# GMC-DRL/MetaBox

Hardware: AMD Instinct MI355X
Metric: env-steps/sec (instances x gens/s), RLEPSO bbob-easy d=10 (higher is better)
Workload: dtype f64

## Files before the change

### include/mbx.h

```cpp
#ifndef MBX_H
#define MBX_H

#include <stddef.h>
#include <stdint.h>

#ifdef __cplusplus
extern "C" {
#endif

#define MBX_OK            0
#define MBX_E_ARG        -1
#define MBX_E_HIP        -2
#define MBX_E_UNSUPPORTED -3
#define MBX_E_NOMEM      -4

#define MBX_KIND_PROTEIN 100

#define MBX_NOISE_NONE    0
#define MBX_NOISE_GAUSS   1
#define MBX_NOISE_UNIFORM 2
#define MBX_NOISE_CAUCHY  3

typedef struct mbx_problem_desc {
    int32_t func_id;
    int32_t kind;
    int32_t dim;
    int32_t n_peaks;
    int32_t noise_kind;
    int32_t reserved;
    double  bias, lb, ub;
    double  pen_coef;
    double  s[4];
    double  noise_a, noise_b;
    const double* dshift;
    const double* m1;
    const double* m2;
    const double* v0;
    const double* v1;
    const double* v2;
    const double* py;
    const double* pc;
    const double* pw;
} mbx_problem_desc;

typedef struct mbx_suite mbx_suite;
typedef struct mbx_batch mbx_batch;

int mbx_suite_create(const mbx_problem_desc* descs, int n_problems, const double* opt, mbx_suite** out);
int mbx_suite_destroy(mbx_suite* s);
int mbx_suite_size(const mbx_suite* s);
int mbx_suite_optimum(const mbx_suite* s, double* optimum_out );
int mbx_suite_close_pairs(const mbx_suite* s, int problem);

int mbx_eval(mbx_suite* s, int problem, const double* d_x, int n, double* d_f,
             int noisy, uint64_t seed, const double* d_noise_draws, void* stream);

#define MBX_ALGO_RLEPSO 1
#define MBX_ALGO_LDE    2
#define MBX_ALGO_DEDDQN 3
#define MBX_ALGO_RANDOM_SEARCH 4
#define MBX_ALGO_RLPSO  5
#define MBX_ALGO_GLEET  6
#define MBX_ALGO_QLPSO  7
#define MBX_ALGO_DE     8
#define MBX_ALGO_PSO    9
#define MBX_ALGO_CMAES  10
#define MBX_ALGO_GLPSO  11
#define MBX_ALGO_JDE21  13
#define MBX_ALGO_MADDE  15

typedef struct mbx_algo_cfg {
    int32_t algo;
    int32_t np;
    int32_t dim;
    int32_t max_fes;
    int32_t log_interval;
    int32_t n_logpoint;
    int32_t early_stop;
    int32_t n_group;
    uint32_t flags;
} mbx_algo_cfg;

#define MBX_F_FDR_FAST               1u
#define MBX_F_GENERIC_GEOMETRY       2u
#define MBX_F_ROLLOUT_PER_GENERATION 4u
int mbx_batch_flags(const mbx_batch* b);

int mbx_state_dim(const mbx_algo_cfg* cfg);
int mbx_action_dim(const mbx_algo_cfg* cfg);
int64_t mbx_tape_stride(const mbx_algo_cfg* cfg);

int mbx_batch_create(mbx_suite* s, const mbx_algo_cfg* cfg, const int32_t* problem_idx,
                     const uint64_t* seeds, int n_instances, mbx_batch** out);
int mbx_batch_destroy(mbx_batch* b);

int mbx_set_tape(mbx_batch* b, const double* d_tape);

int mbx_reset(mbx_batch* b, double* d_state_out, void* stream);

int mbx_step(mbx_batch* b, const void* d_actions, double* d_state_out, double* d_reward_out,
             uint8_t* d_done_out, void* stream);

int mbx_results(mbx_batch* b, double* d_cost_curves , double* d_fes ,
                double* d_return , int32_t* d_steps , int32_t* d_cost_len ,
                void* stream);

int mbx_batch_rebind(mbx_batch* b, const int32_t* problem_idx , const uint64_t* seeds );

int mbx_read_public(mbx_batch* b, int instance, double* host_out , void* stream);

int64_t mbx_instance_state_doubles(const mbx_batch* b);
int mbx_debug_read_state(mbx_batch* b, int instance, double* host_out);
int mbx_debug_write_state(mbx_batch* b, int instance, const double* host_in);

#define MBX_POLICY_RLEPSO 0
#define MBX_POLICY_RLPSO  1
typedef struct mbx_gauss_mlp {
    const float* d_weights;
    int32_t in_dim, h1, h2, out_dim;
    float min_sigma, max_sigma;
    int32_t variant;
} mbx_gauss_mlp;

int mbx_gauss_policy(mbx_batch* b, const mbx_gauss_mlp* net, const double* d_state, float* d_actions, float* d_mu_sigma,
                      void* stream);

typedef struct mbx_lstm_policy {
    const float* d_weights;
    int32_t in_dim, hidden, out_dim;
} mbx_lstm_policy;
int mbx_lde_policy(mbx_batch* b, const mbx_lstm_policy* net, const double* d_state, float* d_h, float* d_c, float* d_actions,
                   float* d_mu_sigma, void* stream);

typedef struct mbx_qnet {
    const float* d_weights;
    int32_t in_dim, width, depth, n_act;
} mbx_qnet;
int mbx_ddqn_qnet(mbx_batch* b, const mbx_qnet* net, const double* d_state, int32_t* d_actions, float* d_q, void* stream);

int mbx_rlepso_policy_table_rows(const mbx_batch* b);
int mbx_rlepso_policy_table(mbx_batch* b, const mbx_gauss_mlp* net, float* d_table, void* stream);
int mbx_rlepso_act_step(mbx_batch* b, const float* d_table, float* d_actions_out, double* d_state_out,
                        double* d_reward_out, uint8_t* d_done_out, void* stream);

int mbx_rlepso_rollout_resident(const mbx_batch* b);
int mbx_rlepso_rollout(mbx_batch* b, const float* d_table, int n_gens, float* d_traj_actions, double* d_traj_state,
                       double* d_traj_reward, uint8_t* d_traj_done, double* d_state_out, double* d_reward_out,
                       uint8_t* d_done_out, void* stream);

int mbx_lde_rollout_resident(const mbx_batch* b);
int mbx_lde_rollout(mbx_batch* b, const mbx_lstm_policy* net, const double* d_state_in, float* d_h, float* d_c, int n_gens,
                    float* d_traj_actions, double* d_traj_state, double* d_traj_reward, uint8_t* d_traj_done, double* d_state_out,
                    double* d_reward_out, uint8_t* d_done_out, void* stream);

int mbx_rlpso_rollout(mbx_batch* b, const mbx_gauss_mlp* net, int n_steps, float* d_actions_out, double* d_state_out,
                      double* d_reward_out, uint8_t* d_done_out, void* stream);

typedef struct mbx_gleet_actor {
    const float* d_weights;
    int32_t n_floats;
    float min_sigma, max_sigma;
} mbx_gleet_actor;
int mbx_gleet_policy(mbx_batch* b, const mbx_gleet_actor* net, const double* d_state, float* d_actions, float* d_mu_sigma, void* stream);

int mbx_qlpso_rollout(mbx_batch* b, const double* d_q_table, int n_steps, int32_t* d_actions_out, double* d_state_out,
                      double* d_reward_out, uint8_t* d_done_out, void* stream);

int mbx_debug_math(int op, const double* d_x, const double* d_y, double* d_out, int n, void* stream);

int mbx_debug_rlepso_draws(uint64_t seed, int gen, int episode, int np, int dim, double* d_out, void* stream);

int mbx_batch_launch_info(const mbx_batch* b, int32_t out[4]);

int mbx_debug_clock_probe(uint64_t* d_out, int n_samples, int sleep_units, void* stream);
int mbx_debug_clock_mark(uint64_t* d_out2, void* stream);
int mbx_debug_clock_slots(mbx_batch* b, uint64_t* d_slots2);

const char* mbx_last_error(void);
const char* mbx_version(void);

#ifdef __cplusplus
}
#endif
#endif
```

### metabox_amd/_abi.py

```python
import ctypes as C
import os

import numpy as np

_HERE = os.path.dirname(os.path.abspath(__file__))
LIB_PATH = os.environ.get('MBX_LIB') or os.path.join(_HERE, 'csrc', 'libmbx.so')

c_double_p = C.POINTER(C.c_double)


class ProblemDesc(C.Structure):
    _fields_ = [('func_id', C.c_int32), ('kind', C.c_int32), ('dim', C.c_int32), ('n_peaks', C.c_int32),
                ('noise_kind', C.c_int32), ('reserved', C.c_int32),
                ('bias', C.c_double), ('lb', C.c_double), ('ub', C.c_double), ('pen_coef', C.c_double),
                ('s', C.c_double * 4), ('noise_a', C.c_double), ('noise_b', C.c_double),
                ('dshift', c_double_p), ('m1', c_double_p), ('m2', c_double_p),
                ('v0', c_double_p), ('v1', c_double_p), ('v2', c_double_p),
                ('py', c_double_p), ('pc', c_double_p), ('pw', c_double_p)]


class AlgoCfg(C.Structure):
    _fields_ = [('algo', C.c_int32), ('np', C.c_int32), ('dim', C.c_int32), ('max_fes', C.c_int32),
                ('log_interval', C.c_int32), ('n_logpoint', C.c_int32), ('early_stop', C.c_int32),
                ('n_group', C.c_int32), ('flags', C.c_uint32)]


F_FDR_FAST, F_GENERIC_GEOMETRY, F_ROLLOUT_PER_GENERATION = 1, 2, 4


class GaussMlp(C.Structure):
    _fields_ = [('d_weights', C.c_void_p), ('in_dim', C.c_int32), ('h1', C.c_int32), ('h2', C.c_int32), ('out_dim', C.c_int32),
                ('min_sigma', C.c_float), ('max_sigma', C.c_float), ('variant', C.c_int32)]


class LstmPolicy(C.Structure):
    _fields_ = [('d_weights', C.c_void_p), ('in_dim', C.c_int32), ('hidden', C.c_int32), ('out_dim', C.c_int32)]


class QNet(C.Structure):
    _fields_ = [('d_weights', C.c_void_p), ('in_dim', C.c_int32), ('width', C.c_int32), ('depth', C.c_int32), ('n_act', C.c_int32)]


class GleetActor(C.Structure):
    _fields_ = [('d_weights', C.c_void_p), ('n_floats', C.c_int32), ('min_sigma', C.c_float), ('max_sigma', C.c_float)]


ALGO_RLEPSO, ALGO_LDE, ALGO_DEDDQN, ALGO_RANDOM_SEARCH, ALGO_RLPSO, ALGO_GLEET, ALGO_QLPSO, ALGO_DE, ALGO_PSO, ALGO_CMAES = 1, 2, 3, 4, 5, 6, 7, 8, 9, 10
ALGO_GLPSO = 11
ALGO_JDE21 = 13
ALGO_MADDE = 15
POLICY_RLEPSO, POLICY_RLPSO = 0, 1
_ARRAY_FIELDS = ('dshift', 'm1', 'm2', 'v0', 'v1', 'v2', 'py', 'pc', 'pw')


def pack_desc(d):
    st = ProblemDesc()
    keep = []
    for k in ('func_id', 'kind', 'dim', 'n_peaks', 'noise_kind'):
        setattr(st, k, int(d[k]))
    for k in ('bias', 'lb', 'ub', 'pen_coef', 'noise_a', 'noise_b'):
        setattr(st, k, float(d[k]))
    for i in range(4):
        st.s[i] = float(d['s'][i])
    for k in _ARRAY_FIELDS:
        a = d.get(k)
        if a is None:
            setattr(st, k, c_double_p())
        else:
            a = np.ascontiguousarray(a, dtype=np.float64)
            keep.append(a)
            setattr(st, k, a.ctypes.data_as(c_double_p))
    return st, keep


def pack_descs(descs):
    arr = (ProblemDesc * len(descs))()
    keep = []
    for i, d in enumerate(descs):
        st, k = pack_desc(d)
        arr[i] = st
        keep.extend(k)
    return arr, keep


_lib = None


class MbxError(RuntimeError):
    pass


def load_lib():
    global _lib
    if _lib is not None:
        return _lib
    if not os.path.exists(LIB_PATH) and not os.environ.get('MBX_LIB'):
        import shutil
        import subprocess
        if shutil.which('hipcc') or os.path.exists('/opt/rocm/bin/hipcc'):
            subprocess.call(['make', '-C', os.path.join(_HERE, 'csrc'), '-s'])
    if not os.path.exists(LIB_PATH):
        raise MbxError(f'{LIB_PATH} is missing: build it with `python -c "import __graft_entry__ as g; g.build()"` '
                       f'(hipcc --offload-arch=gfx950). metabox_amd has no CPU fallback.')
    lib = C.CDLL(LIB_PATH)
    vp, i32, u64, i64 = C.c_void_p, C.c_int32, C.c_uint64, C.c_int64
    proto = {
        'mbx_suite_create': (C.c_int, [C.POINTER(ProblemDesc), C.c_int, c_double_p, C.POINTER(vp)]),
        'mbx_suite_destroy': (C.c_int, [vp]),
        'mbx_suite_size': (C.c_int, [vp]),
        'mbx_suite_optimum': (C.c_int, [vp, c_double_p]),
        'mbx_suite_close_pairs': (C.c_int, [vp, C.c_int]),
        'mbx_eval': (C.c_int, [vp, C.c_int, vp, C.c_int, vp, C.c_int, u64, vp, vp]),
        'mbx_state_dim': (C.c_int, [C.POINTER(AlgoCfg)]),
        'mbx_action_dim': (C.c_int, [C.POINTER(AlgoCfg)]),
        'mbx_tape_stride': (i64, [C.POINTER(AlgoCfg)]),
        'mbx_batch_create': (C.c_int, [vp, C.POINTER(AlgoCfg), C.POINTER(i32), C.POINTER(u64), C.c_int,
                                       C.POINTER(vp)]),
        'mbx_batch_destroy': (C.c_int, [vp]),
        'mbx_batch_flags': (C.c_int, [vp]),
        'mbx_set_tape': (C.c_int, [vp, vp]),
        'mbx_reset': (C.c_int, [vp, vp, vp]),
        'mbx_step': (C.c_int, [vp, vp, vp, vp, vp, vp]),
        'mbx_results': (C.c_int, [vp, vp, vp, vp, vp, vp, vp]),
        'mbx_gauss_policy': (C.c_int, [vp, C.POINTER(GaussMlp), vp, vp, vp, vp]),
        'mbx_lde_policy': (C.c_int, [vp, C.POINTER(LstmPolicy), vp, vp, vp, vp, vp, vp]),
        'mbx_ddqn_qnet': (C.c_int, [vp, C.POINTER(QNet), vp, vp, vp, vp]),
        'mbx_rlepso_policy_table_rows': (C.c_int, [vp]),
        'mbx_rlepso_policy_table': (C.c_int, [vp, C.POINTER(GaussMlp), vp, vp]),
        'mbx_rlepso_act_step': (C.c_int, [vp, vp, vp, vp, vp, vp, vp]),
        'mbx_rlepso_rollout_resident': (C.c_int, [vp]),
        'mbx_rlepso_rollout': (C.c_int, [vp, vp, C.c_int, vp, vp, vp, vp, vp, vp, vp, vp]),
        'mbx_lde_rollout_resident': (C.c_int, [vp]),
        'mbx_lde_rollout': (C.c_int, [vp, C.POINTER(LstmPolicy), vp, vp, vp, C.c_int, vp, vp, vp, vp, vp, vp, vp, vp]),
        'mbx_rlpso_rollout': (C.c_int, [vp, C.POINTER(GaussMlp), C.c_int, vp, vp, vp, vp, vp]),
        'mbx_qlpso_rollout': (C.c_int, [vp, vp, C.c_int, vp, vp, vp, vp, vp]),
        'mbx_gleet_policy': (C.c_int, [vp, C.POINTER(GleetActor), vp, vp, vp, vp]),
        'mbx_debug_math': (C.c_int, [C.c_int, vp, vp, vp, C.c_int, vp]),
        'mbx_debug_rlepso_draws': (C.c_int, [C.c_uint64, C.c_int, C.c_int, C.c_int, C.c_int, vp, vp]),
        'mbx_batch_launch_info': (C.c_int, [vp, C.POINTER(C.c_int32)]),
        'mbx_instance_state_doubles': (i64, [vp]),
        'mbx_debug_read_state': (C.c_int, [vp, C.c_int, c_double_p]),
        'mbx_debug_write_state': (C.c_int, [vp, C.c_int, c_double_p]),
        'mbx_debug_clock_probe': (C.c_int, [vp, C.c_int, C.c_int, vp]),
        'mbx_debug_clock_mark': (C.c_int, [vp, vp]),
        'mbx_debug_clock_slots': (C.c_int, [vp, vp]),
        'mbx_batch_rebind': (C.c_int, [vp, vp, vp]),
        'mbx_read_public': (C.c_int, [vp, C.c_int, c_double_p, vp]),
        'mbx_last_error': (C.c_char_p, []),
        'mbx_version': (C.c_char_p, []),
    }
    for name, (res, args) in proto.items():
        fn = getattr(lib, name)
        fn.restype = res
        fn.argtypes = args
    _lib = lib
    return lib


EXPORTED_SYMBOLS = ('mbx_suite_create', 'mbx_suite_destroy', 'mbx_suite_size', 'mbx_suite_optimum', 'mbx_suite_close_pairs', 'mbx_eval', 'mbx_state_dim', 'mbx_action_dim',
                    'mbx_tape_stride', 'mbx_batch_create', 'mbx_batch_destroy', 'mbx_batch_flags', 'mbx_set_tape', 'mbx_reset', 'mbx_step', 'mbx_results',
                    'mbx_gauss_policy', 'mbx_lde_policy', 'mbx_ddqn_qnet', 'mbx_rlepso_policy_table_rows', 'mbx_rlepso_policy_table', 'mbx_rlepso_act_step',
                    'mbx_rlepso_rollout_resident', 'mbx_rlepso_rollout', 'mbx_lde_rollout_resident', 'mbx_lde_rollout', 'mbx_rlpso_rollout',
                    'mbx_qlpso_rollout', 'mbx_gleet_policy', 'mbx_debug_math', 'mbx_debug_rlepso_draws', 'mbx_batch_launch_info', 'mbx_instance_state_doubles',
                    'mbx_debug_read_state', 'mbx_debug_write_state', 'mbx_debug_clock_probe', 'mbx_debug_clock_mark', 'mbx_debug_clock_slots',
                    'mbx_batch_rebind', 'mbx_read_public', 'mbx_last_error', 'mbx_version')


def check(rc):
    if rc != 0:
        msg = load_lib().mbx_last_error()
        raise MbxError(f'mbx error {rc}: {msg.decode() if msg else "?"}')
```

### metabox_amd/csrc/mbx.hip

```cpp
#include <hip/hip_runtime.h>

#include <cmath>
#include <cstdarg>
#include <cstdio>
#include <cstring>
#include <algorithm>
#include <memory>
#include <string>
#include <vector>

#include "mbx_device.hpp"
#include "mbx_rlepso.hpp"
#include "mbx_lde.hpp"
#ifndef MBX_LDE100_STEP_THREADS
#define MBX_LDE100_STEP_THREADS 512
#endif
#ifndef MBX_LDE50_STEP_THREADS
#define MBX_LDE50_STEP_THREADS 256
#endif
#include "mbx_ddqn.hpp"
#include "mbx_rs.hpp"
#include "mbx_policy.hpp"
#include "mbx_lstm_policy.hpp"
#include "mbx_lde_run.hpp"
#include "mbx_qnet.hpp"
#include "mbx_rlpso.hpp"
#include "mbx_gleet.hpp"
#include "mbx_qlpso.hpp"
#include "mbx_gleet_policy.hpp"
#include "mbx_classic.hpp"
#include "mbx_glpso.hpp"
#include "mbx_jde21.hpp"
#include "mbx_madde.hpp"
#ifndef MBX_SINGLE_TU
#define MBX_RUN_KERNELS_EXTERN
#endif
#include "mbx_run_kernels.hpp"

using namespace mbx;

static thread_local std::string g_err;

static int fail(int code, const char* fmt, ...)
{
    char buf[512];
    va_list ap;
    va_start(ap, fmt);
    vsnprintf(buf, sizeof(buf), fmt, ap);
    va_end(ap);
    g_err = buf;
    return code;
}

#define HIP_TRY(expr)                                                                             \
    do {                                                                                          \
        hipError_t _e = (expr);                                                                   \
        if (_e != hipSuccess) return fail(MBX_E_HIP, "%s failed: %s", #expr, hipGetErrorString(_e)); \
    } while (0)

struct mbx_suite {
    int n = 0, dim = 0;
    double* d_pool = nullptr;
    DevProblem* d_problems = nullptr;
    std::vector<DevProblem> h_problems;
    std::vector<double> optimum;
};

struct mbx_batch {
    mbx_suite* suite = nullptr;
    mbx_algo_cfg cfg{};
    int B = 0;
    int32_t* d_problem_idx = nullptr;
    std::vector<int32_t> h_problem_idx;
    uint64_t* d_seeds = nullptr;
    double* d_state = nullptr;
    int32_t* d_order = nullptr;
    double* d_pci = nullptr;
    unsigned long long* d_clk = nullptr;
    double* d_scratch = nullptr;
    float* d_lstm_pack = nullptr;
    bool fdr_fast = false;
    bool rl_run_kinds_ok = false;
    bool lde_run_kinds_ok = false;
    bool lde_run_kinds_two = false;
    bool rollout_per_generation = false;
    int64_t state_stride = 0;
    const double* d_tape = nullptr;
    size_t lds_bytes = 0;
    int64_t sc_off = 0;
    int64_t tape_stride = 0;
    int state_dim = 0, action_dim = 0;
    int threads = kThreads;
    int fixed_geometry = 0;
};

struct AlgoGeom { int64_t state_doubles, sc_off, tape_stride, lds_doubles; int state_dim, action_dim; };

static AlgoGeom geom_of(const mbx_algo_cfg& c)
{
    AlgoGeom g{};
    if (c.algo == MBX_ALGO_RLEPSO) {
        g.state_doubles = MBX_RLEPSO_STATE_DOUBLES(c.np, c.dim, c.n_logpoint);
        g.sc_off = MBX_RLEPSO_ST_SCALARS(c.np, c.dim);
        g.tape_stride = MBX_RLEPSO_TAPE_STRIDE(c.np, c.dim);
        g.lds_doubles = rl_lds_doubles(c.np, c.dim, (c.flags & MBX_F_GENERIC_GEOMETRY) || c.n_group != 5 || rl_maps_in_lds(c.np, c.dim));
        g.state_dim = 1; g.action_dim = 7 * c.n_group;
    } else if (c.algo == MBX_ALGO_LDE) {
        g.state_doubles = MBX_LDE_STATE_DOUBLES(c.np, c.dim, c.n_logpoint);
        g.sc_off = MBX_LDE_ST_SCALARS(c.np, c.dim);
        g.tape_stride = MBX_LDE_TAPE_STRIDE(c.np, c.dim);
        g.lds_doubles = lde_lds_doubles(c.np, c.dim, lde_maps_in_lds(c.np, c.dim) || (c.flags & MBX_F_GENERIC_GEOMETRY));
        g.state_dim = c.np + 2 * MBX_LDE_BINS; g.action_dim = 2 * c.np;
    } else if (c.algo == MBX_ALGO_DEDDQN) {
        g.state_doubles = MBX_DQ_STATE_DOUBLES(c.np, c.dim, c.n_logpoint);
        g.sc_off = MBX_DQ_ST_SCALARS(c.np, c.dim);
        g.tape_stride = MBX_DQ_TAPE_STRIDE(c.np, c.dim);
        g.lds_doubles = dq_lds_doubles(c.np, c.np, c.dim);
        g.state_dim = MBX_DQ_NFEAT; g.action_dim = 1;
    } else if (c.algo == MBX_ALGO_RANDOM_SEARCH) {
        g.state_doubles = MBX_RS_STATE_DOUBLES(c.np, c.dim, c.n_logpoint);
        g.sc_off = MBX_RS_ST_SCALARS(c.np, c.dim);
        g.tape_stride = MBX_RS_TAPE_STRIDE(c.np, c.dim);
        g.lds_doubles = rs_lds_doubles(c.np, c.dim);
        g.state_dim = 1; g.action_dim = 0;
    } else if (c.algo == MBX_ALGO_RLPSO) {
        g.state_doubles = MBX_RLPSO_STATE_DOUBLES(c.np, c.dim, c.n_logpoint);
        g.sc_off = MBX_RLPSO_ST_SCALARS(c.np, c.dim);
        g.tape_stride = MBX_RLPSO_TAPE_STRIDE(c.np, c.dim);
        g.lds_doubles = rp_lds_doubles(c.np, c.dim, 0);
        g.state_dim = 2 * c.dim; g.action_dim = 1;
    } else if (c.algo == MBX_ALGO_GLEET) {
        g.state_doubles = MBX_GLEET_STATE_DOUBLES(c.np, c.dim, c.n_logpoint);
        g.sc_off = MBX_GLEET_ST_SCALARS(c.np, c.dim);
        g.tape_stride = MBX_GLEET_TAPE_STRIDE(c.np, c.dim);
        g.lds_doubles = gl_lds_doubles(c.np, c.dim);
        g.state_dim = 27 * c.np; g.action_dim = c.np;
    } else if (c.algo == MBX_ALGO_QLPSO) {
        g.state_doubles = MBX_QLPSO_STATE_DOUBLES(c.np, c.dim, c.n_logpoint);
        g.sc_off = MBX_QLPSO_ST_SCALARS(c.np, c.dim);
        g.tape_stride = MBX_QLPSO_TAPE_STRIDE(c.np, c.dim);
        g.lds_doubles = ql_lds_doubles(c.np, c.np, c.dim);
        g.state_dim = 1; g.action_dim = 1;
    } else if (c.algo == MBX_ALGO_DE || c.algo == MBX_ALGO_PSO || c.algo == MBX_ALGO_CMAES) {
        g.state_doubles = c.algo == MBX_ALGO_DE ? MBX_DE_STATE_DOUBLES(c.np, c.dim, c.n_logpoint)
                        : c.algo == MBX_ALGO_PSO ? MBX_PSO_STATE_DOUBLES(c.np, c.dim, c.n_logpoint) : MBX_CMA_STATE_DOUBLES(c.np, c.dim, c.n_logpoint);
        g.sc_off = c.algo == MBX_ALGO_DE ? MBX_DE_ST_SCALARS(c.np, c.dim) : c.algo == MBX_ALGO_PSO ? MBX_PSO_ST_SCALARS(c.np, c.dim) : MBX_CMA_ST_SCALARS(c.np, c.dim);
        g.tape_stride = 0;
        g.lds_doubles = cl_lds_doubles(c.np, c.np, c.dim, 0, c.algo == MBX_ALGO_CMAES);
        g.state_dim = 1; g.action_dim = 0;
    } else if (c.algo == MBX_ALGO_GLPSO) {
        g.state_doubles = MBX_GLPSO_STATE_DOUBLES(c.np, c.dim, c.n_logpoint);
        g.sc_off = MBX_GLPSO_ST_SCALARS(c.np, c.dim);
        g.tape_stride = MBX_GLPSO_TAPE_STRIDE(c.np, c.dim);
        g.lds_doubles = gp_lds_doubles(c.np, c.dim);
        g.state_dim = 1; g.action_dim = 0;
    } else if (c.algo == MBX_ALGO_JDE21) {
        g.state_doubles = MBX_JDE21_STATE_DOUBLES(c.np, c.dim, c.n_logpoint);
        g.sc_off = MBX_JDE21_ST_SCALARS(c.np, c.dim);
        g.tape_stride = MBX_JDE21_TAPE_STRIDE(c.np, c.dim);
        g.lds_doubles = jd_lds_doubles(c.np, c.dim);
        g.state_dim = 1; g.action_dim = 0;
    } else if (c.algo == MBX_ALGO_MADDE) {
        g.state_doubles = MBX_MADDE_STATE_DOUBLES(c.np, c.dim, c.n_logpoint);
        g.sc_off = MBX_MADDE_ST_SCALARS(c.np, c.dim);
        g.tape_stride = MBX_MADDE_TAPE_STRIDE(c.np, c.dim);
        g.lds_doubles = md_lds_doubles(c.np, c.dim);
        g.state_dim = 1; g.action_dim = 0;
    }
    return g;
}

extern "C" int mbx_suite_destroy(mbx_suite* s);
extern "C" int mbx_batch_destroy(mbx_batch* b);

__global__ __launch_bounds__(kThreads) void k_eval(const DevProblem* problems, int problem, const double* __restrict__ x, int n,
                                                   int rows, double* __restrict__ f, int noisy, uint64_t seed,
                                                   const double* __restrict__ draws)
{
    extern __shared__ __attribute__((aligned(16))) double smem[];
    const DevProblem P = problems[problem];
    const int D = P.dim, tid = threadIdx.x;
    const int row0 = blockIdx.x * rows;
    const int m = min(rows, n - row0);
    const int64_t NE = align2((int64_t)rows * D), SC = align2(NE > 2 * kThreads ? NE : 2 * kThreads), DD = align2((int64_t)D * D);
    const int64_t DV = align2(D);
    double* X = smem;
    double* T = X + NE;
    double* Z = T + eval_t_doubles(rows, D);
    double* M1T = Z + SC;
    double* M2T = M1T + DD;
    double* VEC = M2T + DD;
    double* F = VEC + 4 * DV;
    const EvalLds L{X, Z, T, M1T, M2T, VEC, VEC + DV, VEC + 2 * DV, VEC + 3 * DV, F};
    stage_problem(P, L);
    for (int e = tid; e < m * D; e += kThreads) X[e] = x[(int64_t)row0 * D + e];
    __syncthreads();
    eval_rows(P, L, m);
    for (int i = tid; i < m; i += kThreads) {
        double v = F[i];
        if (noisy && P.noise_kind != MBX_NOISE_NONE) {
            double a, b, c;
            const int r = row0 + i;
            if (draws) { a = draws[r]; b = draws[n + r]; c = draws[2 * (int64_t)n + r]; }
            else {
                const Rng rng{(uint32_t)seed, (uint32_t)(seed >> 32), 0u, 0u};
                philox_noise(rng, (uint32_t)r, MBX_SITE_EVAL_A, MBX_SITE_EVAL_B, P.noise_kind, a, b, c);
            }
            v = apply_noise(P, v, a, b, c);
        }
        f[row0 + i] = v;
    }
}

static size_t eval_lds_bytes(int rows, int D)
{
    const int64_t NE = align2((int64_t)rows * D), SC = align2(NE > 2 * kThreads ? NE : 2 * kThreads), DD = align2((int64_t)D * D);
    return (size_t)(NE + eval_t_doubles(rows, D) + SC + 2 * DD + 4 * align2(D) + align2(rows)) * sizeof(double);
}

__global__ void k_init_state(double* state, int64_t stride, int64_t sc_off, int B)
{
    const int b = blockIdx.x * blockDim.x + threadIdx.x;
    if (b < B) state[(int64_t)b * stride + sc_off + MBX_SC_EPISODE] = -1.;
}

__global__ void k_set_optimum(DevProblem* problems, const double* opt, int n)
{
    const int i = blockIdx.x * blockDim.x + threadIdx.x;
    if (i < n) problems[i].optimum = opt[i];
}

__global__ void k_results(const double* state, int64_t stride, int64_t sc_off, int B, int nlog, double* cost, double* fes,
                          double* ret, int32_t* steps, int32_t* cost_len)
{
    const int b = blockIdx.x * blockDim.x + threadIdx.x;
    if (b >= B) return;
    const double* sc = state + (int64_t)b * stride + sc_off;
    const int len = (int)sc[MBX_SC_COST_LEN];
    if (cost)
        for (int k = 0; k <= nlog; ++k) cost[(int64_t)b * (nlog + 1) + k] = sc[MBX_NSCALAR + (k < len ? k : len - 1)];
    if (fes) fes[b] = sc[MBX_SC_FES];
    if (ret) ret[b] = sc[MBX_SC_RETURN];
    if (steps) steps[b] = (int32_t)sc[MBX_SC_GEN];
    if (cost_len) cost_len[b] = len;
}

static int max_lds_bytes()
{
    int v = 0, dev = 0;
    (void)hipGetDevice(&dev);
    if (hipDeviceGetAttribute(&v, hipDeviceAttributeMaxSharedMemoryPerBlock, dev) != hipSuccess || v <= 0) v = 64 * 1024;
    return v;
}

static int launch_eval(mbx_suite* s, int problem, const double* d_x, int n, double* d_f, int noisy, uint64_t seed,
                       const double* d_draws, hipStream_t st)
{
    if (n <= 0) return MBX_OK;
    const int D = s->dim;
    int rows = n < 128 ? n : 128;
    const int cap = max_lds_bytes();
    while (rows > 1 && eval_lds_bytes(rows, D) > (size_t)cap) rows /= 2;
    const size_t lds = eval_lds_bytes(rows, D);
    if (lds > (size_t)cap) return fail(MBX_E_UNSUPPORTED, "dim %d needs %zu B of LDS (> %d)", D, lds, cap);
    HIP_TRY(hipFuncSetAttribute((const void*)k_eval, hipFuncAttributeMaxDynamicSharedMemorySize, (int)lds));
    const int grid = (n + rows - 1) / rows;
    hipLaunchKernelGGL(k_eval, dim3(grid), dim3(kThreads), lds, st, s->d_problems, problem, d_x, n, rows, d_f, noisy, seed,
                       d_draws);
    HIP_TRY(hipGetLastError());
    return MBX_OK;
}

extern "C" int mbx_suite_create(const mbx_problem_desc* descs, int n_problems, const double* opt, mbx_suite** out)
{
    if (!descs || n_problems <= 0 || !out) return fail(MBX_E_ARG, "mbx_suite_create: bad arguments");
    const int D = descs[0].dim;
    if (D < 2 || D > 64) return fail(MBX_E_ARG, "dim %d outside [2, 64]", D);
    std::vector<double> pool;
    std::vector<DevProblem> hp(n_problems);
    struct Off { int64_t o[11]; };
    std::vector<Off> offs(n_problems);
    auto push = [&](const double* p, size_t n) -> int64_t {
        if (!p) return -1;
        while (pool.size() % 2) pool.push_back(0.);
        const int64_t o = (int64_t)pool.size();
        pool.insert(pool.end(), p, p + n);
        return o;
    };
    for (int i = 0; i < n_problems; ++i) {
        const mbx_problem_desc& d = descs[i];
        if (d.dim != D) return fail(MBX_E_ARG, "problem %d has dim %d, suite dim is %d", i, d.dim, D);
        const bool bbob = d.kind >= 1 && d.kind <= 24, protein = d.kind == MBX_KIND_PROTEIN;
        if (!bbob && !protein) return fail(MBX_E_UNSUPPORTED, "problem %d: objective kind %d is not implemented", i, d.kind);
        if (bbob && (!d.dshift || !d.m1)) return fail(MBX_E_ARG, "problem %d: dshift/m1 missing", i);
        if (protein && (!d.v0 || !d.py || !d.pc || !d.pw || d.n_peaks < 2 || d.n_peaks > 160))
            return fail(MBX_E_ARG, "problem %d: protein tables missing (v0, py, pc, pw) or n_atoms outside [2,160]", i);
        if ((d.kind == 21 || d.kind == 22) && (!d.py || !d.pc || !d.pw || d.n_peaks <= 0))
            return fail(MBX_E_ARG, "problem %d: Gallagher tables missing", i);
        DevProblem& p = hp[i];
        memset(&p, 0, sizeof(p));
        p.func_id = d.func_id; p.kind = d.kind; p.dim = d.dim; p.n_peaks = d.n_peaks; p.noise_kind = d.noise_kind;
        p.bias = d.bias; p.lb = d.lb; p.ub = d.ub; p.pen_coef = d.pen_coef;
        for (int k = 0; k < 4; ++k) p.s[k] = d.s[k];
        p.noise_a = d.noise_a; p.noise_b = d.noise_b; p.optimum = NAN;
        const size_t DD = (size_t)D * D, NA = (size_t)d.n_peaks;
        const size_t PK = protein ? 3 * NA * D : NA * D;
        const size_t PC = protein ? 3 * NA : NA * D;
        const size_t PW = protein ? 3 * NA * NA : NA;
        Off& o = offs[i];
        o.o[0] = push(d.dshift, D); o.o[1] = push(d.m1, DD); o.o[2] = push(d.m2, DD);
        o.o[3] = push(d.v0, D); o.o[4] = push(d.v1, D); o.o[5] = push(d.v2, D);
        o.o[6] = push(d.py, PK); o.o[7] = push(d.pc, PC); o.o[8] = push(d.pw, PW);
        o.o[9] = -1; o.o[10] = -1;
        if (d.kind == 21 || d.kind == 22) {
            std::vector<double> lw(NA);
            for (size_t k = 0; k < NA; ++k) lw[k] = std::log(d.pw[k]);
            o.o[10] = push(lw.data(), NA);
            std::vector<double> ry(NA * D);
            for (int k = 0; k < d.n_peaks; ++k)
                for (int r = 0; r < D; ++r) {
                    double acc = 0.;
                    for (int j = 0; j < D; ++j) acc = std::fma(d.m1[(size_t)r * D + j], d.py[(size_t)k * D + j], acc);
                    ry[(size_t)k * D + r] = acc;
                }
            o.o[9] = push(ry.data(), NA * D);
        }
        if (protein) {
            const int n = d.n_peaks, W = n - 1, n_pairs = ((n + 1) / 2) * W;
            const double *se = d.pw, *qm = d.pw + NA * NA, *rm = d.pw + 2 * NA * NA;
            for (int a = 0; a < n; ++a)
                for (int c = a + 1; c < n; ++c)
                    if (se[a * n + c] != se[c * n + a] || qm[a * n + c] != qm[c * n + a] || rm[a * n + c] != rm[c * n + a])
                        return fail(MBX_E_ARG, "problem %d: the protein tables sqrt(e) | q | r must be symmetric (atoms %d, %d)", i, a, c);
            std::vector<int> pi_(n_pairs), pj_(n_pairs), order;
            std::vector<double> d0(n_pairs, INFINITY);
            std::vector<double> bd(n, 0.);
            for (int m = 0; m < n; ++m) {
                double q2 = 0.;
                for (int c = 0; c < 3; ++c) {
                    double bsum = 0.;
                    for (int k = 0; k < D; ++k) bsum += std::fabs(d.v0[k] * d.py[(size_t)k * 3 * n + 3 * m + c]);
                    bsum *= std::fmax(std::fabs(d.ub), std::fabs(d.lb));
                    q2 += bsum * bsum;
                }
                bd[m] = std::sqrt(q2) * (1. + 1e-12);
            }
            for (int t = 0; t < n_pairs; ++t) {
                const int a = t / W, b = t - a * W, La = W - a;
                const bool lower = b >= La;
                pi_[t] = lower ? W - a : a; pj_[t] = pi_[t] + 1 + (lower ? b - La : b);
                if (lower && pi_[t] == a) { pi_[t] = -1; continue; }
                double q2 = 0.;
                for (int c = 0; c < 3; ++c) { const double dd = d.pc[3 * pi_[t] + c] - d.pc[3 * pj_[t] + c]; q2 += dd * dd; }
                d0[t] = std::sqrt(q2) - bd[pi_[t]] - bd[pj_[t]];
            }
            int n_close = 0;
            for (int t = 0; t < n_pairs; ++t) n_close += pi_[t] >= 0 && d0[t] <= 9.0 + 1e-6;
            hp[i].n_close = n_close;
            order.resize(n_pairs);
            for (int t = 0; t < n_pairs; ++t) order[t] = t;
            std::stable_sort(order.begin(), order.end(), [&](int x, int y) { return d0[x] < d0[y]; });
            std::vector<double> rec((size_t)n_pairs * 4, 0.);
            std::vector<double> ij((size_t)(n_pairs + 1) / 2, 0.);
            int32_t* ijw = reinterpret_cast<int32_t*>(ij.data());
            for (int t = 0; t < n_pairs; ++t) {
                const int pi = pi_[order[t]], pj = pj_[order[t]];
                if (pi < 0) { ijw[t] = -1; continue; }
                ijw[t] = pi | (pj << 16);
                rec[(size_t)t * 4] = se[pi * n + pj]; rec[(size_t)t * 4 + 1] = qm[pi * n + pj]; rec[(size_t)t * 4 + 2] = rm[pi * n + pj];
            }
            o.o[9] = push(rec.data(), rec.size());
            o.o[10] = push(ij.data(), ij.size());
        }
    }
    std::unique_ptr<mbx_suite, int (*)(mbx_suite*)> guard(new mbx_suite(), mbx_suite_destroy);
    mbx_suite* s = guard.get();
    s->n = n_problems; s->dim = D;
    HIP_TRY(hipMalloc(&s->d_pool, pool.size() * sizeof(double)));
    HIP_TRY(hipMemcpy(s->d_pool, pool.data(), pool.size() * sizeof(double), hipMemcpyHostToDevice));
    for (int i = 0; i < n_problems; ++i) {
        const double** ptrs[11] = {&hp[i].dshift, &hp[i].m1, &hp[i].m2, &hp[i].v0, &hp[i].v1,
                                   &hp[i].v2, &hp[i].py, &hp[i].pc, &hp[i].pw, &hp[i].pyr, &hp[i].plogw};
        for (int k = 0; k < 11; ++k) *ptrs[k] = offs[i].o[k] < 0 ? nullptr : s->d_pool + offs[i].o[k];
    }
    HIP_TRY(hipMalloc(&s->d_problems, n_problems * sizeof(DevProblem)));
    HIP_TRY(hipMemcpy(s->d_problems, hp.data(), n_problems * sizeof(DevProblem), hipMemcpyHostToDevice));
    s->h_problems = hp;
    s->optimum.assign(n_problems, NAN);
    if (opt) {
        double *d_x = nullptr, *d_f = nullptr;
        HIP_TRY(hipMalloc(&d_x, (size_t)n_problems * D * sizeof(double)));
        HIP_TRY(hipMalloc(&d_f, (size_t)n_problems * sizeof(double)));
        HIP_TRY(hipMemcpy(d_x, opt, (size_t)n_problems * D * sizeof(double), hipMemcpyHostToDevice));
        for (int i = 0; i < n_problems; ++i) {
            int rc = launch_eval(s, i, d_x + (size_t)i * D, 1, d_f + i, 0, 0, nullptr, nullptr);
            if (rc) return rc;
        }
        hipLaunchKernelGGL(k_set_optimum, dim3((n_problems + 63) / 64), dim3(64), 0, nullptr, s->d_problems, d_f, n_problems);
        HIP_TRY(hipDeviceSynchronize());
        HIP_TRY(hipMemcpy(s->optimum.data(), d_f, n_problems * sizeof(double), hipMemcpyDeviceToHost));
        for (int i = 0; i < n_problems; ++i) s->h_problems[i].optimum = s->optimum[i];
        (void)hipFree(d_x); (void)hipFree(d_f);
    }
    *out = guard.release();
    return MBX_OK;
}

extern "C" int mbx_suite_destroy(mbx_suite* s)
{
    if (!s) return MBX_OK;
    (void)hipFree(s->d_pool); (void)hipFree(s->d_problems);
    delete s;
    return MBX_OK;
}

extern "C" int mbx_suite_size(const mbx_suite* s) { return s ? s->n : fail(MBX_E_ARG, "null suite"); }

extern "C" int mbx_suite_optimum(const mbx_suite* s, double* optimum_out)
{
    if (!s || !optimum_out) return fail(MBX_E_ARG, "mbx_suite_optimum: bad arguments");
    memcpy(optimum_out, s->optimum.data(), s->n * sizeof(double));
    return MBX_OK;
}

extern "C" int mbx_suite_close_pairs(const mbx_suite* s, int problem)
{
    if (!s || problem < 0 || problem >= s->n) return fail(MBX_E_ARG, "mbx_suite_close_pairs: bad arguments");
    return s->h_problems[problem].kind == MBX_KIND_PROTEIN ? s->h_problems[problem].n_close : -1;
}

extern "C" int mbx_eval(mbx_suite* s, int problem, const double* d_x, int n, double* d_f, int noisy, uint64_t seed,
                        const double* d_noise_draws, void* stream)
{
    if (!s || problem < 0 || problem >= s->n || n < 0 || (n > 0 && (!d_x || !d_f)))
        return fail(MBX_E_ARG, "mbx_eval: bad arguments");
    return launch_eval(s, problem, d_x, n, d_f, noisy, seed, d_noise_draws, (hipStream_t)stream);
}

static int check_cfg(const mbx_algo_cfg* c)
{
    if (!c) return fail(MBX_E_ARG, "null cfg");
    if (!((c->algo >= MBX_ALGO_RLEPSO && c->algo <= MBX_ALGO_GLPSO) || c->algo == MBX_ALGO_JDE21 || c->algo == MBX_ALGO_MADDE))
        return fail(MBX_E_UNSUPPORTED, "algo %d is not implemented in this build", c->algo);
    if (c->algo == MBX_ALGO_JDE21 && c->np != MBX_JDE21_NP) return fail(MBX_E_ARG, "JDE21 runs np = %d (160 + 10 rows), not %d", MBX_JDE21_NP, c->np);
    if (c->algo == MBX_ALGO_MADDE) {
        if (c->dim < 2 || c->dim > MBX_MADDE_DIM_MAX) return fail(MBX_E_ARG, "MadDE runs dim in [2, %d], not %d", MBX_MADDE_DIM_MAX, c->dim);
        if (c->np != MBX_MADDE_NP(c->dim)) return fail(MBX_E_ARG, "MadDE runs np = 2 dim^2 = %d, not %d", MBX_MADDE_NP(c->dim), c->np);
    } else if (c->np < 4 || c->np > kThreads) return fail(MBX_E_ARG, "np %d outside [4, %d]", c->np, kThreads);
    if (c->dim < 2 || c->dim > 64) return fail(MBX_E_ARG, "dim %d outside [2, 64]", c->dim);
    if (c->algo == MBX_ALGO_RLEPSO && (c->n_group < 1 || c->n_group > 16 || c->np / c->n_group < 1))
        return fail(MBX_E_ARG, "bad n_group %d", c->n_group);
    if (c->max_fes <= 0 || c->log_interval <= 0 || c->n_logpoint <= 0) return fail(MBX_E_ARG, "bad budget/log settings");
    if (c->flags & ~(MBX_F_FDR_FAST | MBX_F_GENERIC_GEOMETRY | MBX_F_ROLLOUT_PER_GENERATION)) return fail(MBX_E_ARG, "unknown bits in cfg.flags 0x%x", c->flags);
    return MBX_OK;
}

extern "C" int mbx_state_dim(const mbx_algo_cfg* c)
{
    if (int rc = check_cfg(c)) return rc;
    return geom_of(*c).state_dim;
}

extern "C" int mbx_action_dim(const mbx_algo_cfg* c)
{
    if (int rc = check_cfg(c)) return rc;
    return geom_of(*c).action_dim;
}

extern "C" int64_t mbx_tape_stride(const mbx_algo_cfg* c)
{
    if (int rc = check_cfg(c)) return rc;
    return geom_of(*c).tape_stride;
}

static int upload_launch_order(mbx_batch* b, const int32_t* problem_idx)
{
    const mbx_suite* s = b->suite;
    const int n_instances = b->B;
    auto weight = [&](int pi) -> int {
        const int k = s->h_problems[pi].kind;
        if (b->cfg.algo == MBX_ALGO_LDE && s->dim >= 16 && k != MBX_KIND_PROTEIN) {
            switch (k) {
            case 21: case 22: return 155; case 17: case 18: return 121; case 16: case 23: return 110; case 15: case 3: case 4: return 100; case 2: case 10: case 11: return 92;
            case 14: case 12: return 81; case 7: return 78; case 19: case 24: case 20: return 77; case 8: case 9: case 6: return 66; default: return 62;
            }
        }
        if (s->dim >= 16 && k != MBX_KIND_PROTEIN) {
            switch (k) {
            case 21: return 3016; case 22: return 2378; case 16: return 2342; case 15: return 2285; case 18: return 2283; case 17: return 2255;
            case 3: return 2077; case 23: return 2049; case 4: return 1980; case 7: return 1885; case 12: return 1840; case 2: return 1787;
            case 11: return 1784; case 10: return 1783; case 24: return 1682; case 14: return 1656; case 19: return 1607; case 1: return 1588;
            case 6: return 1566; case 8: return 1533; case 9: return 1528; case 20: return 1526; case 13: return 1499; case 5: return 1334;
            default: return 1886;
            }
        }
        switch (k) {
        case MBX_KIND_PROTEIN: return 30000 + s->h_problems[pi].n_close;
        case 21: return 416; case 3: return 332; case 15: return 326; case 16: return 325; case 22: return 323; case 23: return 316;
        case 18: return 310; case 17: return 310; case 4: return 309; case 2: return 282; case 12: return 282; case 11: return 275;
        case 10: return 270; case 6: return 254; case 14: return 252; case 1: return 251; case 20: return 250; case 19: return 247;
        case 24: return 246; case 8: return 244; case 13: return 239; case 7: return 237; case 9: return 233; case 5: return 153;
        default: return 276;
        }
    };
    b->lde_run_kinds_ok = true;
    b->rl_run_kinds_ok = true;
    for (int i = 0; i < n_instances; ++i) b->rl_run_kinds_ok = b->rl_run_kinds_ok && rl_run_kind_ok(s->h_problems[problem_idx[i]].kind, s->h_problems[problem_idx[i]].noise_kind);
    b->lde_run_kinds_two = true;
    for (int i = 0; i < n_instances; ++i) {
        b->lde_run_kinds_ok = b->lde_run_kinds_ok && lde_run_kind_ok(s->h_problems[problem_idx[i]].kind, s->dim, false);
        b->lde_run_kinds_two = b->lde_run_kinds_two && lde_run_kind_ok(s->h_problems[problem_idx[i]].kind, s->dim, true);
    }
    std::vector<int32_t> order(n_instances);
    for (int i = 0; i < n_instances; ++i) order[i] = i;
    std::stable_sort(order.begin(), order.end(), [&](int a, int c) {
        const int wa = weight(problem_idx[a]), wc = weight(problem_idx[c]);
        return wa != wc ? wa > wc : s->h_problems[problem_idx[a]].kind < s->h_problems[problem_idx[c]].kind;
    });
    if (!b->d_order) HIP_TRY(hipMalloc(&b->d_order, n_instances * sizeof(int32_t)));
    HIP_TRY(hipMemcpy(b->d_order, order.data(), n_instances * sizeof(int32_t), hipMemcpyHostToDevice));
    return MBX_OK;
}

static uint32_t env_flags()
{
    auto on = [](const char* name) { const char* v = getenv(name); return v && v[0] == '1'; };
    return (on("MBX_FDR_FAST") ? MBX_F_FDR_FAST : 0u) | (on("MBX_GENERIC_GEOMETRY") ? MBX_F_GENERIC_GEOMETRY : 0u) |
           (on("MBX_ROLLOUT_PER_GENERATION") ? MBX_F_ROLLOUT_PER_GENERATION : 0u);
}

extern "C" int mbx_batch_create(mbx_suite* s, const mbx_algo_cfg* cfg_in, const int32_t* problem_idx, const uint64_t* seeds,
                                int n_instances, mbx_batch** out)
{
    if (!s || !problem_idx || !seeds || n_instances <= 0 || !out) return fail(MBX_E_ARG, "mbx_batch_create: bad arguments");
    if (int rc = check_cfg(cfg_in)) return rc;
    mbx_algo_cfg effective = *cfg_in;
    effective.flags |= env_flags();
    const mbx_algo_cfg* cfg = &effective;
    if (cfg->dim != s->dim) return fail(MBX_E_ARG, "cfg.dim %d != suite dim %d", cfg->dim, s->dim);
    for (int i = 0; i < n_instances; ++i)
        if (problem_idx[i] < 0 || problem_idx[i] >= s->n) return fail(MBX_E_ARG, "problem_idx[%d]=%d out of range", i, problem_idx[i]);
    const AlgoGeom g = geom_of(*cfg);
    const size_t lds = (size_t)g.lds_doubles * sizeof(double);
    if (lds > (size_t)max_lds_bytes())
        return fail(MBX_E_UNSUPPORTED, "np=%d dim=%d needs %zu B of LDS per workgroup (> %d)", cfg->np, cfg->dim, lds, max_lds_bytes());
    std::unique_ptr<mbx_batch, int (*)(mbx_batch*)> guard(new mbx_batch(), mbx_batch_destroy);
    mbx_batch* b = guard.get();
    b->suite = s; b->cfg = *cfg; b->B = n_instances; b->lds_bytes = lds;
    if (cfg->algo == MBX_ALGO_LDE && (size_t)lde_lds_doubles(cfg->np, cfg->dim, true) * sizeof(double) > 40 * 1024 && cfg->dim >= 16) b->threads = 512;
    if (cfg->algo == MBX_ALGO_RLEPSO && (size_t)rl_lds_doubles(cfg->np, cfg->dim, true) * sizeof(double) > 80 * 1024 && cfg->dim >= 16) b->threads = cfg->dim >= 32 ? 1024 : 512;
    {
        const bool generic = (cfg->flags & MBX_F_GENERIC_GEOMETRY) != 0;
        if (cfg->algo == MBX_ALGO_RLEPSO && cfg->n_group == 5 && !generic) {
            if (b->threads == kThreads && cfg->np == 100 && cfg->dim == 10) b->fixed_geometry = 1;
            if (b->threads == 1024 && cfg->np == 128 && cfg->dim == 40) b->fixed_geometry = 2;
            if (b->threads == 512 && cfg->np == 100 && cfg->dim == 30) b->fixed_geometry = 7;
            if (b->threads == kThreads && cfg->np == 100 && cfg->dim == 12) b->fixed_geometry = 8;
            if (b->threads == 1024 && cfg->np == 100 && cfg->dim == 40) b->fixed_geometry = 10;
        }
        if (cfg->algo != MBX_ALGO_RLEPSO || b->fixed_geometry == 7 || b->fixed_geometry == 8 || b->fixed_geometry == 10) b->cfg.flags &= ~MBX_F_FDR_FAST;
        b->fdr_fast = (b->cfg.flags & MBX_F_FDR_FAST) != 0;
        if (cfg->algo == MBX_ALGO_LDE && b->threads == 512 && cfg->np == 50 && cfg->dim == 30 && !generic) b->fixed_geometry = 3;
        if (cfg->algo == MBX_ALGO_LDE && b->threads == 512 && cfg->np == 100 && cfg->dim == 30 && !generic) b->fixed_geometry = 6;
        if (cfg->algo == MBX_ALGO_LDE && b->threads == kThreads && cfg->np == 50 && cfg->dim == 10 && !generic) b->fixed_geometry = 9;
        if (cfg->algo == MBX_ALGO_DEDDQN && cfg->np == 100 && cfg->dim == 12 && !generic) b->fixed_geometry = 4;
        if (cfg->algo == MBX_ALGO_GLEET && cfg->np == 100 && cfg->dim == 10 && !generic) b->fixed_geometry = 5;
        b->rollout_per_generation = (cfg->flags & MBX_F_ROLLOUT_PER_GENERATION) != 0;
    }
#ifdef MBX_LDS_PAD_EXPERIMENT
    if (const char* e = getenv("MBX_LDS_PAD")) b->lds_bytes += (size_t)atoi(e);
#endif
    b->state_stride = (g.state_doubles + 1) & ~(int64_t)1;
    b->sc_off = g.sc_off; b->tape_stride = g.tape_stride; b->state_dim = g.state_dim; b->action_dim = g.action_dim;
    HIP_TRY(hipMalloc(&b->d_problem_idx, n_instances * sizeof(int32_t)));
    HIP_TRY(hipMalloc(&b->d_seeds, n_instances * sizeof(uint64_t)));
    HIP_TRY(hipMalloc(&b->d_state, (size_t)n_instances * b->state_stride * sizeof(double)));
    HIP_TRY(hipMemcpy(b->d_problem_idx, problem_idx, n_instances * sizeof(int32_t), hipMemcpyHostToDevice));
    b->h_problem_idx.assign(problem_idx, problem_idx + n_instances);
    HIP_TRY(hipMemcpy(b->d_seeds, seeds, n_instances * sizeof(uint64_t), hipMemcpyHostToDevice));
    HIP_TRY(hipMemset(b->d_state, 0, (size_t)n_instances * b->state_stride * sizeof(double)));
    if (int rc = upload_launch_order(b, problem_idx)) return rc;
    hipLaunchKernelGGL(k_init_state, dim3((n_instances + 255) / 256), dim3(256), 0, nullptr, b->d_state, b->state_stride,
                       g.sc_off, n_instances);
    HIP_TRY(hipDeviceSynchronize());
    if (cfg->algo == MBX_ALGO_RLEPSO) {
        {
        std::vector<double> pci(cfg->np);
        for (int i = 0; i < cfg->np; ++i) pci[i] = 0.05 + 0.45 * std::exp(10. * i / (cfg->np - 1)) / (std::exp(10.) - 1);
        HIP_TRY(hipMalloc(&b->d_pci, cfg->np * sizeof(double)));
        HIP_TRY(hipMemcpy(b->d_pci, pci.data(), cfg->np * sizeof(double), hipMemcpyHostToDevice));
        HIP_TRY(hipMalloc(&b->d_scratch, (size_t)n_instances * sizeof(double)));
    }
#define MBX_RL_LDS(...) HIP_TRY(hipFuncSetAttribute((const void*)(__VA_ARGS__), hipFuncAttributeMaxDynamicSharedMemorySize, (int)lds))
        MBX_RL_LDS(k_rlepso_reset<kThreads>); MBX_RL_LDS(k_rlepso_reset<512>); MBX_RL_LDS(k_rlepso_reset<1024>); MBX_RL_LDS(k_rlepso_reset<512, 100, 30>);
        MBX_RL_LDS(k_rlepso_step<kThreads, 0, 0, 0, true>); MBX_RL_LDS(k_rlepso_step<512, 0, 0, 0, true>); MBX_RL_LDS(k_rlepso_step<1024, 0, 0, 0, true>);
        MBX_RL_LDS(k_rlepso_step<kThreads, 0, 0, 0, false>); MBX_RL_LDS(k_rlepso_step<512, 0, 0, 0, false>); MBX_RL_LDS(k_rlepso_step<1024, 0, 0, 0, false>);
        MBX_RL_LDS(k_rlepso_step<kThreads, 100, 10, 5, true>); MBX_RL_LDS(k_rlepso_step<kThreads, 100, 10, 5, false>);
        MBX_RL_LDS(k_rlepso_step<1024, 128, 40, 5, true>); MBX_RL_LDS(k_rlepso_step<1024, 128, 40, 5, false>);
        MBX_RL_LDS(k_rlepso_step<512, 100, 30, 5, true>);
        MBX_RL_LDS(k_rlepso_run<MBX_RUN10_THREADS, 100, 10, 5, true>); MBX_RL_LDS(k_rlepso_run<MBX_RUN10_THREADS, 100, 10, 5, false>);
        MBX_RL_LDS(k_rlepso_run<1024, 128, 40, 5, true>); MBX_RL_LDS(k_rlepso_run<1024, 128, 40, 5, false>);
        MBX_RL_LDS(k_rlepso_run<512, 100, 30, 5, true>); MBX_RL_LDS(k_rlepso_run<256, 100, 12, 5, true>); MBX_RL_LDS(k_rlepso_run<1024, 100, 40, 5, true>);
#undef MBX_RL_LDS
    } else if (cfg->algo == MBX_ALGO_LDE) {
        {
            HIP_TRY(hipMalloc(&b->d_scratch, (size_t)n_instances * (sizeof(double) + (size_t)g.action_dim * sizeof(float))));
            HIP_TRY(hipMalloc(&b->d_lstm_pack, (size_t)lde_run_pack_floats(g.state_dim, 64, g.action_dim) * sizeof(float)));
            HIP_TRY(hipFuncSetAttribute((const void*)k_lde_run<100, 30>, hipFuncAttributeMaxDynamicSharedMemorySize, (int)(lde_run_lds_doubles(100, 30, 50, false) * sizeof(double))));
            HIP_TRY(hipFuncSetAttribute((const void*)k_lde_run<50, 30>, hipFuncAttributeMaxDynamicSharedMemorySize, (int)(lde_run_lds_doubles(50, 30, 50, false) * sizeof(double))));
            HIP_TRY(hipFuncSetAttribute((const void*)k_lde_run<50, 30, 50, true>, hipFuncAttributeMaxDynamicSharedMemorySize, (int)(lde_run_lds_doubles(50, 30, 50, true) * sizeof(double))));
            HIP_TRY(hipFuncSetAttribute((const void*)k_lde_run<50, 10>, hipFuncAttributeMaxDynamicSharedMemorySize, (int)(lde_run_lds_doubles(50, 10, 50, true) * sizeof(double))));
        }
        HIP_TRY(hipFuncSetAttribute((const void*)k_lde_reset<kThreads>, hipFuncAttributeMaxDynamicSharedMemorySize, (int)lds));
        HIP_TRY(hipFuncSetAttribute((const void*)k_lde_step<kThreads>, hipFuncAttributeMaxDynamicSharedMemorySize, (int)lds));
        HIP_TRY(hipFuncSetAttribute((const void*)k_lde_reset<512>, hipFuncAttributeMaxDynamicSharedMemorySize, (int)lds));
        HIP_TRY(hipFuncSetAttribute((const void*)k_lde_step<512>, hipFuncAttributeMaxDynamicSharedMemorySize, (int)lds));
        HIP_TRY(hipFuncSetAttribute((const void*)k_lde_step<MBX_LDE50_STEP_THREADS, 50, 30>, hipFuncAttributeMaxDynamicSharedMemorySize, (int)lds));
        HIP_TRY(hipFuncSetAttribute((const void*)k_lde_step<MBX_LDE100_STEP_THREADS, 100, 30>, hipFuncAttributeMaxDynamicSharedMemorySize, (int)lds));
        HIP_TRY(hipFuncSetAttribute((const void*)k_lde_reset<512, 100, 30>, hipFuncAttributeMaxDynamicSharedMemorySize, (int)lds));
        HIP_TRY(hipFuncSetAttribute((const void*)k_lde_reset<512, 50, 30>, hipFuncAttributeMaxDynamicSharedMemorySize, (int)lds));
    } else if (cfg->algo == MBX_ALGO_DEDDQN) {
        HIP_TRY(hipFuncSetAttribute((const void*)k_dq_reset, hipFuncAttributeMaxDynamicSharedMemorySize, (int)lds));
        HIP_TRY(hipFuncSetAttribute((const void*)k_dq_step<>, hipFuncAttributeMaxDynamicSharedMemorySize, (int)lds));
        HIP_TRY(hipFuncSetAttribute((const void*)k_dq_step<100, 12>, hipFuncAttributeMaxDynamicSharedMemorySize, (int)lds));
    } else if (cfg->algo == MBX_ALGO_DE || cfg->algo == MBX_ALGO_PSO || cfg->algo == MBX_ALGO_CMAES) {
        HIP_TRY(hipFuncSetAttribute((const void*)k_classic_reset, hipFuncAttributeMaxDynamicSharedMemorySize, (int)lds));
        HIP_TRY(hipFuncSetAttribute((const void*)k_de_sweep, hipFuncAttributeMaxDynamicSharedMemorySize, (int)lds));
        HIP_TRY(hipFuncSetAttribute((const void*)k_pso_sweep, hipFuncAttributeMaxDynamicSharedMemorySize, (int)lds));
        HIP_TRY(hipFuncSetAttribute((const void*)k_cmaes_generation, hipFuncAttributeMaxDynamicSharedMemorySize, (int)lds));
    } else if (cfg->algo == MBX_ALGO_GLPSO) {
        HIP_TRY(hipFuncSetAttribute((const void*)k_glpso_reset, hipFuncAttributeMaxDynamicSharedMemorySize, (int)lds));
        HIP_TRY(hipFuncSetAttribute((const void*)k_glpso_generation, hipFuncAttributeMaxDynamicSharedMemorySize, (int)lds));
    } else if (cfg->algo == MBX_ALGO_JDE21) {
        HIP_TRY(hipFuncSetAttribute((const void*)k_jde21_reset, hipFuncAttributeMaxDynamicSharedMemorySize, (int)lds));
        HIP_TRY(hipFuncSetAttribute((const void*)k_jde21_generation<2>, hipFuncAttributeMaxDynamicSharedMemorySize, (int)lds));
        HIP_TRY(hipFuncSetAttribute((const void*)k_jde21_generation<3>, hipFuncAttributeMaxDynamicSharedMemorySize, (int)lds));
    } else if (cfg->algo == MBX_ALGO_MADDE) {
        HIP_TRY(hipFuncSetAttribute((const void*)k_madde_reset, hipFuncAttributeMaxDynamicSharedMemorySize, (int)lds));
        HIP_TRY(hipFuncSetAttribute((const void*)k_madde_generation, hipFuncAttributeMaxDynamicSharedMemorySize, (int)lds));
    } else if (cfg->algo == MBX_ALGO_QLPSO) {
        HIP_TRY(hipFuncSetAttribute((const void*)k_qlpso_reset, hipFuncAttributeMaxDynamicSharedMemorySize, (int)lds));
        HIP_TRY(hipFuncSetAttribute((const void*)k_qlpso_step<false>, hipFuncAttributeMaxDynamicSharedMemorySize, (int)lds));
        HIP_TRY(hipFuncSetAttribute((const void*)k_qlpso_step<true>, hipFuncAttributeMaxDynamicSharedMemorySize, (int)lds));
    } else if (cfg->algo == MBX_ALGO_GLEET) {
        HIP_TRY(hipFuncSetAttribute((const void*)k_gleet_reset, hipFuncAttributeMaxDynamicSharedMemorySize, (int)lds));
        HIP_TRY(hipFuncSetAttribute((const void*)k_gleet_step<>, hipFuncAttributeMaxDynamicSharedMemorySize, (int)lds));
        HIP_TRY(hipFuncSetAttribute((const void*)k_gleet_step<100, 10>, hipFuncAttributeMaxDynamicSharedMemorySize, (int)lds));
    } else if (cfg->algo == MBX_ALGO_RLPSO) {
        HIP_TRY(hipFuncSetAttribute((const void*)k_rlpso_reset, hipFuncAttributeMaxDynamicSharedMemorySize, (int)lds));
        HIP_TRY(hipFuncSetAttribute((const void*)k_rlpso_step<false>, hipFuncAttributeMaxDynamicSharedMemorySize, (int)lds));
        HIP_TRY(hipFuncSetAttribute((const void*)k_rlpso_step<true>, hipFuncAttributeMaxDynamicSharedMemorySize, (int)lds));
    } else {
        HIP_TRY(hipFuncSetAttribute((const void*)k_rs_population, hipFuncAttributeMaxDynamicSharedMemorySize, (int)lds));
    }
    *out = guard.release();
    return MBX_OK;
}

extern "C" int mbx_batch_destroy(mbx_batch* b)
{
    if (!b) return MBX_OK;
    (void)hipFree(b->d_problem_idx); (void)hipFree(b->d_seeds); (void)hipFree(b->d_state); (void)hipFree(b->d_order); (void)hipFree(b->d_pci); (void)hipFree(b->d_scratch); (void)hipFree(b->d_lstm_pack);
    delete b;
    return MBX_OK;
}

extern "C" int mbx_batch_rebind(mbx_batch* b, const int32_t* problem_idx, const uint64_t* seeds)
{
    if (!b || !problem_idx || !seeds) return fail(MBX_E_ARG, "mbx_batch_rebind: bad arguments");
    for (int i = 0; i < b->B; ++i)
        if (problem_idx[i] < 0 || problem_idx[i] >= b->suite->n) return fail(MBX_E_ARG, "problem_idx[%d]=%d out of range", i, problem_idx[i]);
    HIP_TRY(hipDeviceSynchronize());
    HIP_TRY(hipMemcpy(b->d_problem_idx, problem_idx, b->B * sizeof(int32_t), hipMemcpyHostToDevice));
    b->h_problem_idx.assign(problem_idx, problem_idx + b->B);
    HIP_TRY(hipMemcpy(b->d_seeds, seeds, b->B * sizeof(uint64_t), hipMemcpyHostToDevice));
    if (int rc = upload_launch_order(b, problem_idx)) return rc;
    hipLaunchKernelGGL(k_init_state, dim3((b->B + 255) / 256), dim3(256), 0, nullptr, b->d_state, b->state_stride, b->sc_off, b->B);
    HIP_TRY(hipDeviceSynchronize());
    return MBX_OK;
}

extern "C" int mbx_read_public(mbx_batch* b, int instance, double* host_out, void* stream)
{
    if (!b || instance < 0 || instance >= b->B || !host_out) return fail(MBX_E_ARG, "mbx_read_public: bad arguments");
    const size_t n = (size_t)(MBX_NSCALAR + b->cfg.n_logpoint + 1) * sizeof(double);
    HIP_TRY(hipMemcpyAsync(host_out, b->d_state + (int64_t)instance * b->state_stride + b->sc_off, n, hipMemcpyDeviceToHost, (hipStream_t)stream));
    HIP_TRY(hipStreamSynchronize((hipStream_t)stream));
    return MBX_OK;
}

extern "C" int mbx_set_tape(mbx_batch* b, const double* d_tape)
{
    if (!b) return fail(MBX_E_ARG, "null batch");
    b->d_tape = d_tape;
    return MBX_OK;
}

static BatchParams make_params(const mbx_batch* b)
{
    BatchParams p;
    p.problems = b->suite->d_problems; p.problem_idx = b->d_problem_idx; p.seeds = b->d_seeds;
    p.state = b->d_state; p.state_stride = b->state_stride;
    p.tape = b->d_tape; p.tape_stride = b->tape_stride; p.order = b->d_order; p.pci = b->d_pci;
    p.NP = b->cfg.np; p.D = b->cfg.dim; p.max_fes = b->cfg.max_fes; p.log_interval = b->cfg.log_interval;
    p.n_logpoint = b->cfg.n_logpoint; p.early_stop = b->cfg.early_stop; p.n_group = b->cfg.n_group; p.B = b->B;
    p.sc_off = b->sc_off;
    p.clk = b->d_clk;
    return p;
}

static void launch_rlepso_step(mbx_batch* b, hipStream_t stream, const float* d_actions, double* d_state_out, double* d_reward_out,
                               uint8_t* d_done_out, const float* d_table, int table_rows, float* d_actions_out)
{
#define MBX_RLEPSO_LAUNCH(...)                                                                                                   \
    hipLaunchKernelGGL((k_rlepso_step<__VA_ARGS__>), dim3(b->B), dim3(b->threads), b->lds_bytes, stream, make_params(b), d_actions, \
                       d_state_out, d_reward_out, d_done_out, d_table, table_rows, d_actions_out)
    const bool fast = b->fdr_fast;
    if (b->fixed_geometry == 1) { if (fast) MBX_RLEPSO_LAUNCH(kThreads, 100, 10, 5, false); else MBX_RLEPSO_LAUNCH(kThreads, 100, 10, 5, true); }
    else if (b->fixed_geometry == 2) { if (fast) MBX_RLEPSO_LAUNCH(1024, 128, 40, 5, false); else MBX_RLEPSO_LAUNCH(1024, 128, 40, 5, true); }
    else if (b->fixed_geometry == 7) MBX_RLEPSO_LAUNCH(512, 100, 30, 5, true);
    else if (b->threads == 1024) { if (fast) MBX_RLEPSO_LAUNCH(1024, 0, 0, 0, false); else MBX_RLEPSO_LAUNCH(1024, 0, 0, 0, true); }
    else if (b->threads == 512) { if (fast) MBX_RLEPSO_LAUNCH(512, 0, 0, 0, false); else MBX_RLEPSO_LAUNCH(512, 0, 0, 0, true); }
    else { if (fast) MBX_RLEPSO_LAUNCH(kThreads, 0, 0, 0, false); else MBX_RLEPSO_LAUNCH(kThreads, 0, 0, 0, true); }
#undef MBX_RLEPSO_LAUNCH
}

extern "C" int mbx_reset(mbx_batch* b, double* d_state_out, void* stream)
{
    if (!b) return fail(MBX_E_ARG, "null batch");
    if (b->cfg.algo == MBX_ALGO_RANDOM_SEARCH)
        hipLaunchKernelGGL(k_rs_population, dim3(b->B), dim3(kThreads), b->lds_bytes, (hipStream_t)stream, make_params(b), 1, d_state_out,
                           (double*)nullptr, (uint8_t*)nullptr);
    else if (b->cfg.algo == MBX_ALGO_RLEPSO && b->fixed_geometry == 7)
        hipLaunchKernelGGL((k_rlepso_reset<512, 100, 30>), dim3(b->B), dim3(512), b->lds_bytes, (hipStream_t)stream, make_params(b), d_state_out);
    else if (b->cfg.algo == MBX_ALGO_RLEPSO && b->threads == 1024)
        hipLaunchKernelGGL(k_rlepso_reset<1024>, dim3(b->B), dim3(1024), b->lds_bytes, (hipStream_t)stream, make_params(b), d_state_out);
    else if (b->cfg.algo == MBX_ALGO_RLEPSO && b->threads == 512)
        hipLaunchKernelGGL(k_rlepso_reset<512>, dim3(b->B), dim3(512), b->lds_bytes, (hipStream_t)stream, make_params(b), d_state_out);
    else if (b->cfg.algo == MBX_ALGO_RLEPSO)
        hipLaunchKernelGGL(k_rlepso_reset<kThreads>, dim3(b->B), dim3(kThreads), b->lds_bytes, (hipStream_t)stream, make_params(b), d_state_out);
    else if (b->cfg.algo == MBX_ALGO_RLPSO)
        hipLaunchKernelGGL(k_rlpso_reset, dim3(b->B), dim3(kThreads), b->lds_bytes, (hipStream_t)stream, make_params(b), d_state_out);
    else if (b->cfg.algo == MBX_ALGO_DE || b->cfg.algo == MBX_ALGO_PSO || b->cfg.algo == MBX_ALGO_CMAES)
        hipLaunchKernelGGL(k_classic_reset, dim3(b->B), dim3(kThreads), (size_t)cl_lds_doubles(b->cfg.np, b->cfg.np, b->cfg.dim, 0, 0) * sizeof(double),
                           (hipStream_t)stream, make_params(b), (int)b->cfg.algo, d_state_out);
    else if (b->cfg.algo == MBX_ALGO_GLPSO)
        hipLaunchKernelGGL(k_glpso_reset, dim3(b->B), dim3(kThreads), b->lds_bytes, (hipStream_t)stream, make_params(b), d_state_out);
    else if (b->cfg.algo == MBX_ALGO_JDE21)
        hipLaunchKernelGGL(k_jde21_reset, dim3(b->B), dim3(kThreads), b->lds_bytes, (hipStream_t)stream, make_params(b), d_state_out);
    else if (b->cfg.algo == MBX_ALGO_MADDE)
        hipLaunchKernelGGL(k_madde_reset, dim3(b->B), dim3(kThreads), b->lds_bytes, (hipStream_t)stream, make_params(b), d_state_out);
    else if (b->cfg.algo == MBX_ALGO_QLPSO)
        hipLaunchKernelGGL(k_qlpso_reset, dim3(b->B), dim3(kThreads), b->lds_bytes, (hipStream_t)stream, make_params(b), d_state_out);
    else if (b->cfg.algo == MBX_ALGO_GLEET)
        hipLaunchKernelGGL(k_gleet_reset, dim3(b->B), dim3(kThreads), b->lds_bytes, (hipStream_t)stream, make_params(b), d_state_out);
    else {
        if (!d_state_out) return fail(MBX_E_ARG, "mbx_reset: this algorithm needs d_state_out");
        if (b->cfg.algo == MBX_ALGO_LDE && b->fixed_geometry == 6)
            hipLaunchKernelGGL((k_lde_reset<512, 100, 30>), dim3(b->B), dim3(512), b->lds_bytes, (hipStream_t)stream, make_params(b), d_state_out);
        else if (b->cfg.algo == MBX_ALGO_LDE && b->fixed_geometry == 3)
            hipLaunchKernelGGL((k_lde_reset<512, 50, 30>), dim3(b->B), dim3(512), b->lds_bytes, (hipStream_t)stream, make_params(b), d_state_out);
        else if (b->cfg.algo == MBX_ALGO_LDE && b->threads == 512)
            hipLaunchKernelGGL(k_lde_reset<512>, dim3(b->B), dim3(512), b->lds_bytes, (hipStream_t)stream, make_params(b), d_state_out);
        else if (b->cfg.algo == MBX_ALGO_LDE)
            hipLaunchKernelGGL(k_lde_reset<kThreads>, dim3(b->B), dim3(kThreads), b->lds_bytes, (hipStream_t)stream, make_params(b), d_state_out);
        else
            hipLaunchKernelGGL(k_dq_reset, dim3(b->B), dim3(kThreads), b->lds_bytes, (hipStream_t)stream, make_params(b), d_state_out);
    }
    HIP_TRY(hipGetLastError());
    return MBX_OK;
}

extern "C" int mbx_step(mbx_batch* b, const void* d_actions, double* d_state_out, double* d_reward_out, uint8_t* d_done_out,
                        void* stream)
{
    const bool no_agent = b && (b->cfg.algo == MBX_ALGO_RANDOM_SEARCH || b->cfg.algo == MBX_ALGO_DE || b->cfg.algo == MBX_ALGO_PSO ||
                                b->cfg.algo == MBX_ALGO_CMAES || b->cfg.algo == MBX_ALGO_GLPSO || b->cfg.algo == MBX_ALGO_JDE21 ||
                                b->cfg.algo == MBX_ALGO_MADDE);
    if (!b || (!d_actions && !no_agent)) return fail(MBX_E_ARG, "mbx_step: bad arguments");
    if (b->cfg.algo == MBX_ALGO_RANDOM_SEARCH)
        hipLaunchKernelGGL(k_rs_population, dim3(b->B), dim3(kThreads), b->lds_bytes, (hipStream_t)stream, make_params(b), 0, d_state_out,
                           d_reward_out, d_done_out);
    else if (b->cfg.algo == MBX_ALGO_RLEPSO)
        launch_rlepso_step(b, (hipStream_t)stream, (const float*)d_actions, d_state_out, d_reward_out, d_done_out, nullptr, 0, nullptr);
    else if (b->cfg.algo == MBX_ALGO_DE)
        hipLaunchKernelGGL(k_de_sweep, dim3(b->B), dim3(kThreads), (size_t)cl_lds_doubles(1, b->cfg.np, b->cfg.dim, 1, 0) * sizeof(double),
                           (hipStream_t)stream, make_params(b), d_state_out, d_reward_out, d_done_out);
    else if (b->cfg.algo == MBX_ALGO_PSO)
        hipLaunchKernelGGL(k_pso_sweep, dim3(b->B), dim3(kThreads), (size_t)cl_lds_doubles(1, b->cfg.np, b->cfg.dim, 0, 0) * sizeof(double),
                           (hipStream_t)stream, make_params(b), d_state_out, d_reward_out, d_done_out);
    else if (b->cfg.algo == MBX_ALGO_CMAES)
        hipLaunchKernelGGL(k_cmaes_generation, dim3(b->B), dim3(kThreads), (size_t)cl_lds_doubles(b->cfg.np, b->cfg.np, b->cfg.dim, 0, 1) * sizeof(double),
                           (hipStream_t)stream, make_params(b), d_state_out, d_reward_out, d_done_out);
    else if (b->cfg.algo == MBX_ALGO_GLPSO)
        hipLaunchKernelGGL(k_glpso_generation, dim3(b->B), dim3(kThreads), b->lds_bytes, (hipStream_t)stream, make_params(b), d_state_out,
                           d_reward_out, d_done_out);
    else if (b->cfg.algo == MBX_ALGO_JDE21 && jd_waves((int64_t)b->lds_bytes) == 3)
        hipLaunchKernelGGL(k_jde21_generation<3>, dim3(b->B), dim3(kThreads), b->lds_bytes, (hipStream_t)stream, make_params(b), d_state_out,
                           d_reward_out, d_done_out);
    else if (b->cfg.algo == MBX_ALGO_JDE21)
        hipLaunchKernelGGL(k_jde21_generation<2>, dim3(b->B), dim3(kThreads), b->lds_bytes, (hipStream_t)stream, make_params(b), d_state_out,
                           d_reward_out, d_done_out);
    else if (b->cfg.algo == MBX_ALGO_MADDE)
        hipLaunchKernelGGL(k_madde_generation, dim3(b->B), dim3(kThreads), b->lds_bytes, (hipStream_t)stream, make_params(b), d_state_out,
                           d_reward_out, d_done_out);
    else if (b->cfg.algo == MBX_ALGO_QLPSO)
        hipLaunchKernelGGL(k_qlpso_step<false>, dim3(b->B), dim3(kThreads), (size_t)ql_lds_doubles(1, b->cfg.np, b->cfg.dim) * sizeof(double),
                           (hipStream_t)stream, make_params(b), (const int32_t*)d_actions, (const double*)nullptr, 1, d_state_out,
                           d_reward_out, d_done_out, (int32_t*)nullptr);
    else if (b->cfg.algo == MBX_ALGO_GLEET && b->fixed_geometry == 5)
        hipLaunchKernelGGL((k_gleet_step<100, 10>), dim3(b->B), dim3(kThreads), b->lds_bytes, (hipStream_t)stream, make_params(b),
                           (const float*)d_actions, d_state_out, d_reward_out, d_done_out);
    else if (b->cfg.algo == MBX_ALGO_GLEET)
        hipLaunchKernelGGL(k_gleet_step<>, dim3(b->B), dim3(kThreads), b->lds_bytes, (hipStream_t)stream, make_params(b),
                           (const float*)d_actions, d_state_out, d_reward_out, d_done_out);
    else if (b->cfg.algo == MBX_ALGO_RLPSO)
        hipLaunchKernelGGL(k_rlpso_step<false>, dim3(b->B), dim3(kThreads), (size_t)rp_lds_doubles(1, b->cfg.dim, 0) * sizeof(double),
                           (hipStream_t)stream, make_params(b), (const float*)d_actions, GaussMlp{}, 1, d_state_out, d_reward_out,
                           d_done_out, (float*)nullptr);
    else {
        if (!d_state_out) return fail(MBX_E_ARG, "mbx_step: this algorithm needs d_state_out");
        if (b->cfg.algo == MBX_ALGO_LDE && b->fixed_geometry == 3)
            hipLaunchKernelGGL((k_lde_step<MBX_LDE50_STEP_THREADS, 50, 30>), dim3(b->B), dim3(MBX_LDE50_STEP_THREADS), b->lds_bytes, (hipStream_t)stream, make_params(b),
                               (const float*)d_actions, d_state_out, d_reward_out, d_done_out);
        else if (b->cfg.algo == MBX_ALGO_LDE && b->fixed_geometry == 6)
            hipLaunchKernelGGL((k_lde_step<MBX_LDE100_STEP_THREADS, 100, 30>), dim3(b->B), dim3(MBX_LDE100_STEP_THREADS), b->lds_bytes, (hipStream_t)stream, make_params(b),
                               (const float*)d_actions, d_state_out, d_reward_out, d_done_out);
        else if (b->cfg.algo == MBX_ALGO_LDE && b->threads == 512)
            hipLaunchKernelGGL(k_lde_step<512>, dim3(b->B), dim3(512), b->lds_bytes, (hipStream_t)stream, make_params(b),
                               (const float*)d_actions, d_state_out, d_reward_out, d_done_out);
        else if (b->cfg.algo == MBX_ALGO_LDE)
            hipLaunchKernelGGL(k_lde_step<kThreads>, dim3(b->B), dim3(kThreads), b->lds_bytes, (hipStream_t)stream, make_params(b),
                               (const float*)d_actions, d_state_out, d_reward_out, d_done_out);
        else if (b->fixed_geometry == 4)
            hipLaunchKernelGGL((k_dq_step<100, 12>), dim3(b->B), dim3(kDqStepThreads), (size_t)dq_lds_doubles(1, b->cfg.np, b->cfg.dim) * sizeof(double), (hipStream_t)stream, make_params(b),
                               (const int32_t*)d_actions, d_state_out, d_reward_out, d_done_out);
        else
            hipLaunchKernelGGL(k_dq_step<>, dim3(b->B), dim3(kDqStepThreads), (size_t)dq_lds_doubles(1, b->cfg.np, b->cfg.dim) * sizeof(double), (hipStream_t)stream, make_params(b),
                               (const int32_t*)d_actions, d_state_out, d_reward_out, d_done_out);
    }
    HIP_TRY(hipGetLastError());
    return MBX_OK;
}

static int check_gauss_mlp(const mbx_batch* b, const mbx_gauss_mlp* net, const char* who, size_t* lds)
{
    if (!b || !net || !net->d_weights) return fail(MBX_E_ARG, "%s: bad arguments", who);
    if (b->cfg.algo != MBX_ALGO_RLEPSO && b->cfg.algo != MBX_ALGO_RLPSO)
        return fail(MBX_E_UNSUPPORTED, "%s: the batch is neither an RLEPSO nor an RL-PSO batch", who);
    if (net->variant != (b->cfg.algo == MBX_ALGO_RLPSO ? MBX_POLICY_RLPSO : MBX_POLICY_RLEPSO))
        return fail(MBX_E_ARG, "%s: net.variant does not match the batch's algorithm", who);
    if (net->in_dim != b->state_dim || net->out_dim != b->action_dim || net->h1 < 1 || net->h2 < 1)
        return fail(MBX_E_ARG, "%s: network dimensions do not match the batch (state_dim -> h1 -> h2 -> action_dim)", who);
    *lds = gauss_mlp_lds_bytes(net->in_dim, net->h1, net->h2, net->out_dim);
    if (*lds > 64 * 1024) return fail(MBX_E_UNSUPPORTED, "%s: the weights do not fit the 64 KB LDS budget of this kernel", who);
    return MBX_OK;
}

static int policy_blocks(int rows)
{
    const int blocks = (rows + 2 * kPolicyWaves - 1) / (2 * kPolicyWaves);
    return blocks < 1 ? 1 : (blocks > 2048 ? 2048 : blocks);
}

extern "C" int mbx_gauss_policy(mbx_batch* b, const mbx_gauss_mlp* net, const double* d_state, float* d_actions, float* d_mu_sigma,
                                 void* stream)
{
    size_t lds = 0;
    if (const int rc = check_gauss_mlp(b, net, "mbx_gauss_policy", &lds)) return rc;
    if (!d_state || !d_actions) return fail(MBX_E_ARG, "mbx_gauss_policy: bad arguments");
    const GaussMlp g{net->d_weights, net->in_dim, net->h1, net->h2, net->out_dim, net->min_sigma, net->max_sigma, net->variant};
    hipLaunchKernelGGL(k_gauss_mlp_policy, dim3(policy_blocks(b->B)), dim3(kThreads), lds, (hipStream_t)stream, make_params(b), g,
                       d_state, d_actions, d_mu_sigma, 0);
    HIP_TRY(hipGetLastError());
    return MBX_OK;
}

static int lde_policy_launch(mbx_batch* b, const mbx_lstm_policy* net, const double* d_state, float* d_h, float* d_c, float* d_actions,
                             float* d_mu_sigma, void* stream, int skip_done)
{
    if (!b || !net || !net->d_weights || !d_state || !d_h || !d_c) return fail(MBX_E_ARG, "mbx_lde_policy: bad arguments");
    if (b->cfg.algo != MBX_ALGO_LDE) return fail(MBX_E_UNSUPPORTED, "mbx_lde_policy: the batch is not an LDE batch");
    if (net->in_dim != b->state_dim || net->out_dim != b->action_dim || net->hidden < 1 || net->hidden > 64 || net->out_dim > 512)
        return fail(MBX_E_ARG, "mbx_lde_policy: network %d -> %d -> %d does not fit the batch (state %d, action %d; hidden <= 64)",
                    net->in_dim, net->hidden, net->out_dim, b->state_dim, b->action_dim);
    const LstmPolicy g{net->d_weights, net->in_dim, net->hidden, net->out_dim};
    {
        const size_t lds = lstm_policy_lds_bytes(net->in_dim, net->hidden);
        if (lds > (size_t)max_lds_bytes()) return fail(MBX_E_UNSUPPORTED, "mbx_lde_policy: %zu B of LDS needed", lds);
#define MBX_LSTM_LAUNCH(...)                                                                                                                          \
        do {                                                                                                                                          \
            HIP_TRY(hipFuncSetAttribute((const void*)k_lstm_policy<__VA_ARGS__>, hipFuncAttributeMaxDynamicSharedMemorySize, (int)lds));              \
            hipLaunchKernelGGL((k_lstm_policy<__VA_ARGS__>), dim3((b->B + kLstmTile - 1) / kLstmTile), dim3(kThreads), lds, (hipStream_t)stream,      \
                               make_params(b), g, d_state, d_h, d_c, d_actions, d_mu_sigma, skip_done);                                               \
        } while (0)
        if (net->in_dim == 60 && net->hidden == 50 && net->out_dim == 100) MBX_LSTM_LAUNCH(kLstmTile, 60, 50, 100);
        else if (net->in_dim == 110 && net->hidden == 50 && net->out_dim == 200) MBX_LSTM_LAUNCH(kLstmTile, 110, 50, 200);
        else MBX_LSTM_LAUNCH(kLstmTile);
#undef MBX_LSTM_LAUNCH
    }
    HIP_TRY(hipGetLastError());
    return MBX_OK;
}

extern "C" int mbx_lde_policy(mbx_batch* b, const mbx_lstm_policy* net, const double* d_state, float* d_h, float* d_c, float* d_actions,
                              float* d_mu_sigma, void* stream)
{
    return lde_policy_launch(b, net, d_state, d_h, d_c, d_actions, d_mu_sigma, stream, 0);
}

extern "C" int mbx_ddqn_qnet(mbx_batch* b, const mbx_qnet* net, const double* d_state, int32_t* d_actions, float* d_q, void* stream)
{
    if (!b || !net || !net->d_weights || !d_state || !d_actions) return fail(MBX_E_ARG, "mbx_ddqn_qnet: bad arguments");
    if (b->cfg.algo != MBX_ALGO_DEDDQN) return fail(MBX_E_UNSUPPORTED, "mbx_ddqn_qnet: the batch is not a DE-DDQN batch");
    if (net->in_dim != b->state_dim) return fail(MBX_E_ARG, "mbx_ddqn_qnet: the network reads %d features, the batch writes %d", net->in_dim, b->state_dim);
    if (net->in_dim != 99 || net->width != 100 || net->depth != 4 || net->n_act != 4)
        return fail(MBX_E_UNSUPPORTED, "mbx_ddqn_qnet: only the reference architecture 99 -> 100 x 4 -> 4 is built (got %d -> %d x %d -> %d)",
                    net->in_dim, net->width, net->depth, net->n_act);
    const QNet g{net->d_weights, net->in_dim, net->width, net->depth, net->n_act};
    hipLaunchKernelGGL((k_qnet_argmax<99, 100, 4>), dim3((b->B + kQTile - 1) / kQTile), dim3(kQThreads), 0, (hipStream_t)stream, g, d_state, d_actions,
                       d_q, b->B);
    HIP_TRY(hipGetLastError());
    return MBX_OK;
}

extern "C" int mbx_rlepso_policy_table_rows(const mbx_batch* b)
{
    if (!b || b->cfg.algo != MBX_ALGO_RLEPSO) return fail(MBX_E_ARG, "mbx_rlepso_policy_table_rows: not an RLEPSO batch");
    return b->cfg.max_fes + 2 * b->cfg.np + 1;
}

extern "C" int mbx_rlepso_policy_table(mbx_batch* b, const mbx_gauss_mlp* net, float* d_table, void* stream)
{
    size_t lds = 0;
    if (const int rc = check_gauss_mlp(b, net, "mbx_rlepso_policy_table", &lds)) return rc;
    if (!d_table || net->in_dim != 1 || b->cfg.algo != MBX_ALGO_RLEPSO) return fail(MBX_E_ARG, "mbx_rlepso_policy_table: bad arguments");
    const int rows = mbx_rlepso_policy_table_rows(b);
    const GaussMlp g{net->d_weights, net->in_dim, net->h1, net->h2, net->out_dim, net->min_sigma, net->max_sigma, net->variant};
    hipLaunchKernelGGL(k_gauss_mlp_policy, dim3(policy_blocks(rows)), dim3(kThreads), lds, (hipStream_t)stream, make_params(b), g,
                       (const double*)nullptr, (float*)nullptr, d_table, rows);
    HIP_TRY(hipGetLastError());
    return MBX_OK;
}

extern "C" int mbx_rlepso_act_step(mbx_batch* b, const float* d_table, float* d_actions_out, double* d_state_out,
                                   double* d_reward_out, uint8_t* d_done_out, void* stream)
{
    if (!b || !d_table) return fail(MBX_E_ARG, "mbx_rlepso_act_step: bad arguments");
    if (b->cfg.algo != MBX_ALGO_RLEPSO) return fail(MBX_E_UNSUPPORTED, "mbx_rlepso_act_step: the batch is not an RLEPSO batch");
    if (b->d_tape) return fail(MBX_E_ARG, "mbx_rlepso_act_step: a replay tape carries no policy draws; use mbx_step with recorded actions");
    launch_rlepso_step(b, (hipStream_t)stream, nullptr, d_state_out, d_reward_out, d_done_out, d_table, mbx_rlepso_policy_table_rows(b), d_actions_out);
    HIP_TRY(hipGetLastError());
    return MBX_OK;
}

extern "C" int mbx_batch_flags(const mbx_batch* b)
{
    if (!b) return fail(MBX_E_ARG, "mbx_batch_flags: null batch");
    return (int)b->cfg.flags;
}

extern "C" int mbx_rlepso_rollout_resident(const mbx_batch* b)
{
    if (!b) return fail(MBX_E_ARG, "mbx_rlepso_rollout_resident: null batch");
    if (b->cfg.algo != MBX_ALGO_RLEPSO) return 0;
    return (b->fixed_geometry == 1 || b->fixed_geometry == 2 || b->fixed_geometry == 7 || b->fixed_geometry == 8 || b->fixed_geometry == 10) && !b->rollout_per_generation ? 1 : 0;
}

__global__ void k_sum_rewards(double* __restrict__ acc, const double* __restrict__ r, int n, int first)
{
    const int i = blockIdx.x * blockDim.x + threadIdx.x;
    if (i < n) acc[i] = first ? r[i] : acc[i] + r[i];
}

static int launch_rlepso_run(mbx_batch* b, const float* d_table, int rows, int n_gens, const RunOut& out, hipStream_t stream)
{
#define MBX_RUN_LAUNCH(T, ...) hipLaunchKernelGGL((k_rlepso_run<T, __VA_ARGS__>), dim3(b->B), dim3(T), b->lds_bytes, stream, make_params(b), d_table, rows, n_gens, out)
    if (b->fixed_geometry == 1) { if (b->fdr_fast) MBX_RUN_LAUNCH(MBX_RUN10_THREADS, 100, 10, 5, false); else MBX_RUN_LAUNCH(MBX_RUN10_THREADS, 100, 10, 5, true); }
    else if (b->fixed_geometry == 2) { if (b->fdr_fast) MBX_RUN_LAUNCH(1024, 128, 40, 5, false); else MBX_RUN_LAUNCH(1024, 128, 40, 5, true); }
    else if (b->fixed_geometry == 7) MBX_RUN_LAUNCH(512, 100, 30, 5, true);
    else if (b->fixed_geometry == 8) MBX_RUN_LAUNCH(256, 100, 12, 5, true);
    else if (b->fixed_geometry == 10) MBX_RUN_LAUNCH(1024, 100, 40, 5, true);
    else return fail(MBX_E_UNSUPPORTED, "k_rlepso_run: no instantiation for this geometry");
#undef MBX_RUN_LAUNCH
    HIP_TRY(hipGetLastError());
    return MBX_OK;
}

extern "C" int mbx_rlepso_rollout(mbx_batch* b, const float* d_table, int n_gens, float* d_traj_actions, double* d_traj_state,
                                  double* d_traj_reward, uint8_t* d_traj_done, double* d_state_out, double* d_reward_out,
                                  uint8_t* d_done_out, void* stream)
{
    if (!b || !d_table) return fail(MBX_E_ARG, "mbx_rlepso_rollout: bad arguments");
    if (b->cfg.algo != MBX_ALGO_RLEPSO) return fail(MBX_E_UNSUPPORTED, "mbx_rlepso_rollout: the batch is not an RLEPSO batch");
    if (n_gens < 1) return fail(MBX_E_ARG, "mbx_rlepso_rollout: n_gens must be >= 1");
    if (b->d_tape) return fail(MBX_E_ARG, "mbx_rlepso_rollout: a replay tape holds one generation and no policy draws; use mbx_step with recorded actions");
    const int rows = mbx_rlepso_policy_table_rows(b);
    if (mbx_rlepso_rollout_resident(b) == 1)
        return launch_rlepso_run(b, d_table, rows, n_gens, RunOut{d_traj_actions, d_traj_state, d_traj_reward, d_traj_done, d_state_out, d_reward_out, d_done_out},
                                 (hipStream_t)stream);
    const int64_t B = b->B, A = b->action_dim;
    for (int g = 0; g < n_gens; ++g) {
        double* r = d_traj_reward ? d_traj_reward + g * B : (d_reward_out ? b->d_scratch : nullptr);
        double* st = d_traj_state ? d_traj_state + g * B : d_state_out;
        uint8_t* dn = d_traj_done ? d_traj_done + g * B : d_done_out;
        launch_rlepso_step(b, (hipStream_t)stream, nullptr, st, r, dn, d_table, rows, d_traj_actions ? d_traj_actions + g * B * A : nullptr);
        if (d_reward_out)
            hipLaunchKernelGGL(k_sum_rewards, dim3((b->B + 255) / 256), dim3(256), 0, (hipStream_t)stream, d_reward_out, r, b->B, g == 0);
    }
    if (d_traj_state && d_state_out)
        HIP_TRY(hipMemcpyAsync(d_state_out, d_traj_state + (n_gens - 1) * B, B * sizeof(double), hipMemcpyDeviceToDevice, (hipStream_t)stream));
    if (d_traj_done && d_done_out)
        HIP_TRY(hipMemcpyAsync(d_done_out, d_traj_done + (n_gens - 1) * B, B, hipMemcpyDeviceToDevice, (hipStream_t)stream));
    HIP_TRY(hipGetLastError());
    return MBX_OK;
}

extern "C" int mbx_lde_rollout_resident(const mbx_batch* b)
{
    if (!b) return fail(MBX_E_ARG, "mbx_lde_rollout_resident: null batch");
    if (b->cfg.algo != MBX_ALGO_LDE) return 0;
    if (b->rollout_per_generation) return 0;
    if (b->fixed_geometry == 9 || b->fixed_geometry == 3) return (b->lde_run_kinds_ok || b->lde_run_kinds_two) ? 1 : 0;
    return b->fixed_geometry == 6 && b->lde_run_kinds_ok ? 1 : 0;
}

extern "C" int mbx_lde_rollout(mbx_batch* b, const mbx_lstm_policy* net, const double* d_state_in, float* d_h, float* d_c, int n_gens,
                               float* d_traj_actions, double* d_traj_state, double* d_traj_reward, uint8_t* d_traj_done,
                               double* d_state_out, double* d_reward_out, uint8_t* d_done_out, void* stream)
{
    if (!b || !net || !net->d_weights || !d_state_in || !d_h || !d_c || !d_state_out) return fail(MBX_E_ARG, "mbx_lde_rollout: bad arguments");
    if (b->cfg.algo != MBX_ALGO_LDE) return fail(MBX_E_UNSUPPORTED, "mbx_lde_rollout: the batch is not an LDE batch");
    if (n_gens < 1) return fail(MBX_E_ARG, "mbx_lde_rollout: n_gens must be >= 1");
    if (b->d_tape) return fail(MBX_E_ARG, "mbx_lde_rollout: a replay tape holds one generation and no policy draws; use mbx_step with recorded actions");
    if (net->in_dim != b->state_dim || net->out_dim != b->action_dim || net->hidden < 1 || net->hidden > 64)
        return fail(MBX_E_ARG, "mbx_lde_rollout: network %d -> %d -> %d does not fit the batch (state %d, action %d; hidden <= 64)",
                    net->in_dim, net->hidden, net->out_dim, b->state_dim, b->action_dim);
    const int64_t B = b->B, A = b->action_dim, NF = b->state_dim;
    if (mbx_lde_rollout_resident(b) == 1 && net->hidden == 50) {
        LdeRunArgs ka{};
        ka.bp = make_params(b);
        {
            const LstmPolicy src{net->d_weights, net->in_dim, net->hidden, net->out_dim};
            hipLaunchKernelGGL(k_lde_repack<0>, dim3(64), dim3(256), 0, (hipStream_t)stream, src, b->d_lstm_pack);
        }
        ka.net = LstmPolicy{b->d_lstm_pack, net->in_dim, net->hidden, net->out_dim};
        ka.state_in = d_state_in; ka.hbuf = d_h; ka.cbuf = d_c; ka.n_gens = n_gens;
        ka.out = LdeRunOut{d_traj_actions, d_traj_state, d_traj_reward, d_traj_done, d_state_out, d_reward_out, d_done_out};
        if (b->fixed_geometry == 6)
            hipLaunchKernelGGL((k_lde_run<100, 30>), dim3(b->B), dim3(lde_run_threads(100)), (size_t)lde_run_lds_doubles(100, 30, 50, false) * sizeof(double),
                               (hipStream_t)stream, ka);
        else if (b->fixed_geometry == 9)
            hipLaunchKernelGGL((k_lde_run<50, 10>), dim3(b->B), dim3(lde_run_threads(50)), (size_t)lde_run_lds_doubles(50, 10, 50, true) * sizeof(double),
                               (hipStream_t)stream, ka);
        else if (b->lde_run_kinds_ok)
            hipLaunchKernelGGL((k_lde_run<50, 30>), dim3(b->B), dim3(lde_run_threads(50)), (size_t)lde_run_lds_doubles(50, 30, 50, false) * sizeof(double),
                               (hipStream_t)stream, ka);
        else
            hipLaunchKernelGGL((k_lde_run<50, 30, 50, true>), dim3(b->B), dim3(lde_run_threads(50)), (size_t)lde_run_lds_doubles(50, 30, 50, true) * sizeof(double),
                               (hipStream_t)stream, ka);
        HIP_TRY(hipGetLastError());
        return MBX_OK;
    }
    if (d_state_in != d_state_out)
        HIP_TRY(hipMemcpyAsync(d_state_out, d_state_in, (size_t)B * NF * sizeof(double), hipMemcpyDeviceToDevice, (hipStream_t)stream));
    double* r_scratch = b->d_scratch;
    float* a_scratch = (float*)(b->d_scratch + B);
    for (int g = 0; g < n_gens; ++g) {
        float* acts = d_traj_actions ? d_traj_actions + g * B * A : a_scratch;
        if (const int rc = lde_policy_launch(b, net, d_state_out, d_h, d_c, acts, nullptr, stream, 1)) return rc;
        double* r = d_traj_reward ? d_traj_reward + g * B : (d_reward_out ? r_scratch : nullptr);
        uint8_t* dn = d_traj_done ? d_traj_done + g * B : d_done_out;
        if (const int rc = mbx_step(b, acts, d_state_out, r, dn, stream)) return rc;
        if (d_traj_state)
            HIP_TRY(hipMemcpyAsync(d_traj_state + g * B * NF, d_state_out, (size_t)B * NF * sizeof(double), hipMemcpyDeviceToDevice, (hipStream_t)stream));
        if (d_reward_out)
            hipLaunchKernelGGL(k_sum_rewards, dim3((b->B + 255) / 256), dim3(256), 0, (hipStream_t)stream, d_reward_out, r, b->B, g == 0);
    }
    if (d_traj_done && d_done_out)
        HIP_TRY(hipMemcpyAsync(d_done_out, d_traj_done + (n_gens - 1) * B, B, hipMemcpyDeviceToDevice, (hipStream_t)stream));
    HIP_TRY(hipGetLastError());
    return MBX_OK;
}

extern "C" int mbx_rlpso_rollout(mbx_batch* b, const mbx_gauss_mlp* net, int n_steps, float* d_actions_out, double* d_state_out,
                                 double* d_reward_out, uint8_t* d_done_out, void* stream)
{
    size_t lds = 0;
    if (const int rc = check_gauss_mlp(b, net, "mbx_rlpso_rollout", &lds)) return rc;
    if (b->cfg.algo != MBX_ALGO_RLPSO) return fail(MBX_E_UNSUPPORTED, "mbx_rlpso_rollout: the batch is not an RL-PSO batch");
    if (n_steps < 1) return fail(MBX_E_ARG, "mbx_rlpso_rollout: n_steps must be >= 1");
    if (b->d_tape) return fail(MBX_E_ARG, "mbx_rlpso_rollout: a replay tape holds one step; use mbx_step with recorded actions");
    if ((size_t)(net->in_dim + 2 * net->h1 + 2 * net->h2 + 2) * sizeof(float) > (size_t)kRpActDoubles * sizeof(double))
        return fail(MBX_E_UNSUPPORTED, "mbx_rlpso_rollout: hidden layers too wide for the in-kernel actor");
    const GaussMlp g{net->d_weights, net->in_dim, net->h1, net->h2, net->out_dim, net->min_sigma, net->max_sigma, net->variant};
    const size_t step_lds = (size_t)rp_lds_doubles(1, b->cfg.dim, 2 * gauss_mlp_net_floats(net->in_dim, net->h1, net->h2, 1)) * sizeof(double);
    if (step_lds > 64 * 1024) return fail(MBX_E_UNSUPPORTED, "mbx_rlpso_rollout: the actor does not fit the LDS budget of the step kernel");
    if (n_steps == 1)
        hipLaunchKernelGGL(k_rlpso_step<false>, dim3(b->B), dim3(kThreads), step_lds, (hipStream_t)stream, make_params(b),
                           (const float*)nullptr, g, 1, d_state_out, d_reward_out, d_done_out, d_actions_out);
    else
        hipLaunchKernelGGL(k_rlpso_step<true>, dim3(b->B), dim3(kThreads), step_lds, (hipStream_t)stream, make_params(b),
                           (const float*)nullptr, g, n_steps, d_state_out, d_reward_out, d_done_out, d_actions_out);
    HIP_TRY(hipGetLastError());
    return MBX_OK;
}

extern "C" int mbx_gleet_policy(mbx_batch* b, const mbx_gleet_actor* net, const double* d_state, float* d_actions, float* d_mu_sigma,
                                void* stream)
{
    if (!b || !net || !net->d_weights || !d_state || !d_actions) return fail(MBX_E_ARG, "mbx_gleet_policy: bad arguments");
    if (b->cfg.algo != MBX_ALGO_GLEET) return fail(MBX_E_UNSUPPORTED, "mbx_gleet_policy: the batch is not a GLEET batch");
    if (net->n_floats != GpOff::total) return fail(MBX_E_ARG, "mbx_gleet_policy: expected %d weights, got %d", GpOff::total, net->n_floats);
    if (b->cfg.np > kGpThreads) return fail(MBX_E_UNSUPPORTED, "mbx_gleet_policy: np %d > %d", b->cfg.np, kGpThreads);
    const GleetActor g{net->d_weights, net->min_sigma, net->max_sigma};
    hipLaunchKernelGGL(k_gleet_policy, dim3(b->B), dim3(kGpThreads), gleet_policy_lds_bytes(b->cfg.np), (hipStream_t)stream, make_params(b),
                       g, d_state, d_actions, d_mu_sigma);
    HIP_TRY(hipGetLastError());
    return MBX_OK;
}

extern "C" int mbx_qlpso_rollout(mbx_batch* b, const double* d_q_table, int n_steps, int32_t* d_actions_out, double* d_state_out,
                                 double* d_reward_out, uint8_t* d_done_out, void* stream)
{
    if (!b || !d_q_table) return fail(MBX_E_ARG, "mbx_qlpso_rollout: bad arguments");
    if (b->cfg.algo != MBX_ALGO_QLPSO) return fail(MBX_E_UNSUPPORTED, "mbx_qlpso_rollout: the batch is not a QLPSO batch");
    if (n_steps < 1) return fail(MBX_E_ARG, "mbx_qlpso_rollout: n_steps must be >= 1");
    if (b->d_tape && n_steps != 1) return fail(MBX_E_ARG, "mbx_qlpso_rollout: a replay tape holds one step");
    const size_t lds = (size_t)ql_lds_doubles(1, b->cfg.np, b->cfg.dim) * sizeof(double);
    if (n_steps == 1)
        hipLaunchKernelGGL(k_qlpso_step<false>, dim3(b->B), dim3(kThreads), lds, (hipStream_t)stream, make_params(b), (const int32_t*)nullptr,
                           d_q_table, 1, d_state_out, d_reward_out, d_done_out, d_actions_out);
    else
        hipLaunchKernelGGL(k_qlpso_step<true>, dim3(b->B), dim3(kThreads), lds, (hipStream_t)stream, make_params(b), (const int32_t*)nullptr,
                           d_q_table, n_steps, d_state_out, d_reward_out, d_done_out, d_actions_out);
    HIP_TRY(hipGetLastError());
    return MBX_OK;
}

extern "C" int mbx_results(mbx_batch* b, double* d_cost_curves, double* d_fes, double* d_return, int32_t* d_steps,
                           int32_t* d_cost_len, void* stream)
{
    if (!b) return fail(MBX_E_ARG, "null batch");
    hipLaunchKernelGGL(k_results, dim3((b->B + 255) / 256), dim3(256), 0, (hipStream_t)stream, b->d_state, b->state_stride,
                       b->sc_off, b->B, b->cfg.n_logpoint, d_cost_curves, d_fes, d_return,
                       d_steps, d_cost_len);
    HIP_TRY(hipGetLastError());
    return MBX_OK;
}

__global__ void k_debug_math(int op, const double* __restrict__ x, const double* __restrict__ y, double* __restrict__ out, int n)
{
    const int i = blockIdx.x * blockDim.x + threadIdx.x;
    if (i >= n) return;
    const double a = x[i], b = y ? y[i] : 0.;
    double r;
    switch (op) {
    case 0: r = m_log(a); break;
    case 1: r = m_exp(a); break;
    case 2: r = m_sin(a); break;
    case 3: r = m_cos(a); break;
    case 4: r = m_pow(a, b); break;
    case 5: r = osc1(a); break;
    default: r = asy1(a, b); break;
    }
    out[i] = r;
}

__global__ void k_debug_rlepso_draws(uint64_t seed, uint32_t gen, uint32_t episode, int NP, int D, double* __restrict__ out)
{
    const int it = blockIdx.x * blockDim.x + threadIdx.x;
    if (2 * it >= NP * D) return;
    const Rng rng{(uint32_t)seed, (uint32_t)(seed >> 32), gen, episode};
    const U4 wa = rng.draw((uint32_t)it, MBX_SITE_ELEM_A), wt = rng.draw((uint32_t)it, MBX_SITE_TOURN);
    double* o = out + (int64_t)it * 8;
    o[0] = u32d(wa.x); o[1] = u32d(wa.z); o[2] = (double)__umulhi(wt.x, (uint32_t)NP); o[3] = (double)__umulhi(wt.y, (uint32_t)NP);
    if (2 * it + 1 < NP * D) { o[4] = u32d(wa.y); o[5] = u32d(wa.w); o[6] = (double)__umulhi(wt.z, (uint32_t)NP); o[7] = (double)__umulhi(wt.w, (uint32_t)NP); }
}

extern "C" int mbx_debug_rlepso_draws(uint64_t seed, int gen, int episode, int np, int dim, double* d_out, void* stream)
{
    if (np < 1 || dim < 1 || !d_out) return fail(MBX_E_ARG, "mbx_debug_rlepso_draws: bad arguments");
    const int pairs = (np * dim + 1) / 2;
    hipLaunchKernelGGL(k_debug_rlepso_draws, dim3((pairs + 255) / 256), dim3(256), 0, (hipStream_t)stream, seed, (uint32_t)gen, (uint32_t)episode, np, dim, d_out);
    HIP_TRY(hipGetLastError());
    return MBX_OK;
}

__global__ void k_clock_probe(uint64_t* __restrict__ out, int n, int sleep_units)
{
    if (threadIdx.x != 0) return;
    for (int i = 0; i < n; ++i) {
        const uint64_t t = __builtin_amdgcn_s_memtime(), r = __builtin_amdgcn_s_memrealtime();
        out[2 * i] = t; out[2 * i + 1] = r;
        for (int k = 0; k < sleep_units; k += 127) __builtin_amdgcn_s_sleep(127);
    }
}

__global__ void k_clock_mark(uint64_t* __restrict__ out)
{
    if (threadIdx.x == 0) { out[0] = __builtin_amdgcn_s_memtime(); out[1] = __builtin_amdgcn_s_memrealtime(); }
}

extern "C" int mbx_debug_clock_probe(uint64_t* d_out, int n_samples, int sleep_units, void* stream)
{
    if (!d_out || n_samples < 2 || sleep_units < 1) return fail(MBX_E_ARG, "mbx_debug_clock_probe: bad arguments");
    hipLaunchKernelGGL(k_clock_probe, dim3(1), dim3(64), 0, (hipStream_t)stream, d_out, n_samples, sleep_units);
    HIP_TRY(hipGetLastError());
    return MBX_OK;
}

extern "C" int mbx_debug_clock_mark(uint64_t* d_out2, void* stream)
{
    if (!d_out2) return fail(MBX_E_ARG, "mbx_debug_clock_mark: bad arguments");
    hipLaunchKernelGGL(k_clock_mark, dim3(1), dim3(64), 0, (hipStream_t)stream, d_out2);
    HIP_TRY(hipGetLastError());
    return MBX_OK;
}

extern "C" int mbx_debug_clock_slots(mbx_batch* b, uint64_t* d_slots2)
{
    if (!b) return fail(MBX_E_ARG, "mbx_debug_clock_slots: null batch");
    b->d_clk = (unsigned long long*)d_slots2;
    return MBX_OK;
}

extern "C" int mbx_batch_launch_info(const mbx_batch* b, int32_t out[4])
{
    if (!b || !out) return fail(MBX_E_ARG, "mbx_batch_launch_info: bad arguments");
    out[0] = b->threads; out[1] = (int32_t)b->lds_bytes; out[2] = b->fixed_geometry; out[3] = (int32_t)b->state_stride;
    if (b->cfg.algo == MBX_ALGO_LDE && b->fixed_geometry == 3) out[0] = MBX_LDE50_STEP_THREADS;
    if (b->cfg.algo == MBX_ALGO_DEDDQN) {
        out[0] = kDqStepThreads; out[1] = (int32_t)(dq_lds_doubles(1, b->cfg.np, b->cfg.dim) * sizeof(double));
    }
    return MBX_OK;
}

extern "C" int mbx_debug_math(int op, const double* d_x, const double* d_y, double* d_out, int n, void* stream)
{
    if (op < 0 || op > 6 || !d_x || !d_out || n < 0 || ((op == 4 || op == 6) && !d_y)) return fail(MBX_E_ARG, "mbx_debug_math: bad arguments");
    if (n) hipLaunchKernelGGL(k_debug_math, dim3((n + 255) / 256), dim3(256), 0, (hipStream_t)stream, op, d_x, d_y, d_out, n);
    HIP_TRY(hipGetLastError());
    return MBX_OK;
}

extern "C" int64_t mbx_instance_state_doubles(const mbx_batch* b)
{
    if (!b) return fail(MBX_E_ARG, "null batch");
    return geom_of(b->cfg).state_doubles;
}

extern "C" int mbx_debug_read_state(mbx_batch* b, int instance, double* host_out)
{
    if (!b || instance < 0 || instance >= b->B || !host_out) return fail(MBX_E_ARG, "mbx_debug_read_state: bad arguments");
    HIP_TRY(hipDeviceSynchronize());
    const int64_t n = mbx_instance_state_doubles(b);
    HIP_TRY(hipMemcpy(host_out, b->d_state + (int64_t)instance * b->state_stride, n * sizeof(double), hipMemcpyDeviceToHost));
    double* sc = host_out + b->sc_off;
    const int len = (int)sc[MBX_SC_COST_LEN];
    for (int k = len; k <= b->cfg.n_logpoint && len > 0; ++k) sc[MBX_NSCALAR + k] = sc[MBX_NSCALAR + len - 1];
    return MBX_OK;
}

extern "C" int mbx_debug_write_state(mbx_batch* b, int instance, const double* host_in)
{
    if (!b || instance < 0 || instance >= b->B || !host_in) return fail(MBX_E_ARG, "mbx_debug_write_state: bad arguments");
    if (b->cfg.algo == MBX_ALGO_RLEPSO) {
        const DevProblem& P = b->suite->h_problems[b->h_problem_idx[instance]];
        const double* pb = host_in + MBX_RLEPSO_ST_PBPOS(b->cfg.np, b->cfg.dim);
        for (int e = 0; e < b->cfg.np * b->cfg.dim; ++e)
            if (!(pb[e] >= P.lb && pb[e] <= P.ub))
                return fail(MBX_E_ARG, "mbx_debug_write_state: pbest position %d (%g) lies outside the problem's box [%g, %g]", e, pb[e], P.lb, P.ub);
    }
    HIP_TRY(hipDeviceSynchronize());
    const int64_t n = mbx_instance_state_doubles(b);
    HIP_TRY(hipMemcpy(b->d_state + (int64_t)instance * b->state_stride, host_in, n * sizeof(double), hipMemcpyHostToDevice));
    return MBX_OK;
}

extern "C" const char* mbx_last_error(void) { return g_err.c_str(); }
extern "C" const char* mbx_version(void) { return "metabox_amd libmbx 0.4 (gfx950; Philox stream layout 2: include/mbx_layout.h section 3; linear maps as fma chains)"; }

#ifdef MBX_PHASE_TIMING
extern "C" int mbx_debug_phase_cycles(unsigned long long* out, int n, int reset)
{
    std::vector<unsigned long long> h(8192 * 16);
    if (hipMemcpyFromSymbol(h.data(), HIP_SYMBOL(mbx::g_phase_cycles), h.size() * 8) != hipSuccess) return -1;
    for (int i = 0; i < n && i < 16; ++i) { out[i] = 0; for (int b = 0; b < 8192; ++b) out[i] += h[b * 16 + i]; }
// ... 8 lines not shown
```

### metabox_amd/csrc/mbx_rlepso.hpp

```cpp
#pragma once
#include "mbx_device.hpp"

namespace mbx {

struct BatchParams {
    const DevProblem* problems;
    const int32_t* problem_idx;
    const uint64_t* seeds;
    double* state;
    int64_t state_stride;
    const double* tape;
    int64_t tape_stride;
    const int32_t* order;
    const double* pci;
    int32_t NP, D, max_fes, log_interval, n_logpoint, early_stop, n_group, B;
    int64_t sc_off;
    unsigned long long* clk;
};

template <class PT>
__device__ __forceinline__ bool log_and_terminate(const BatchParams& bp, const PT& P, double fes, double gbest, int& log_index,
                                                  int& cost_len, double* __restrict__ cost)
{
    if (fes >= (double)log_index * bp.log_interval) { log_index += 1; cost[cost_len++] = gbest; }
    bool done = fes >= bp.max_fes;
    if (!isnan(P.optimum) && bp.early_stop) done = done || gbest <= 1e-8;
    if (done) {
        if (cost_len >= bp.n_logpoint + 1) cost[cost_len - 1] = gbest;
        else cost[cost_len++] = gbest;
    }
    return done;
}

struct RlLds {
    double *PB, *X, *Z, *T, *M1T, *M2T, *DSH, *V0, *V1, *V2, *PBC, *NC, *PNI, *CMUT, *R1, *R2, *GB, *COEF, *RED;
    int *IMPR, *MASK, *RANK;
    uint8_t* KB;
    uint16_t* FL;
    int* FLN;
    double* NCS;
    int zd;
    __device__ __forceinline__ EvalLds eval() const { return EvalLds{X, Z, T, M1T, M2T, DSH, V0, V1, V2, NC, zd}; }
};

__host__ __device__ inline int64_t align2(int64_t n) { return (n + 1) & ~(int64_t)1; }

__host__ __device__ inline int64_t rl_aux_doubles(int NP, int D) { const int64_t NE = (int64_t)NP * D; return ((NE + 15) / 16 * 16 + 16 + 2 * NE + 7) / 8; }

__host__ __device__ inline int64_t rl_z_doubles(int NP, int D)
{
    const int64_t NE = align2((int64_t)NP * D);
    int64_t need = 3 * align2(NP) + 96 + rl_aux_doubles(NP, D);
    if (need < 2 * kThreads) need = 2 * kThreads;
    if (D == 12 && need < 4 * 4 * 100) need = 4 * 4 * 100;
    return align2(NE > need ? NE : need);
}

#ifndef MBX_RUN_KC40
#define MBX_RUN_KC40 8
#endif
#ifndef MBX_RUN_KC30
#define MBX_RUN_KC30 0
#endif
__host__ __device__ constexpr int rl_run_matvec_chunk(int D) { return D == 40 ? MBX_RUN_KC40 : D == 30 ? MBX_RUN_KC30 : 0; }

__host__ __device__ constexpr bool rl_maps_in_lds(int NP, int D) { return !(NP == 100 && D == 30); }

__host__ __device__ inline int64_t rl_lds_doubles(int NP, int D, bool maps = true)
{
    const int64_t NE = align2((int64_t)NP * D), SC = rl_z_doubles(NP, D), DD = maps ? align2((int64_t)D * D) : 0,
                  P = align2(NP), TS = eval_t_doubles(NP, D);
    return TS + NE + SC + 2 * DD + 4 * P + 5 * align2(D) + 16 + 3 * align2((P + 1) / 2);
}

__device__ __forceinline__ RlLds rl_carve(double* base, int NP, int D, bool maps = true)
{
    const int64_t NE = align2((int64_t)NP * D), SC = rl_z_doubles(NP, D), DD = maps ? align2((int64_t)D * D) : 0,
                  P = align2(NP), TS = eval_t_doubles(NP, D);
    RlLds L;
    double* p = base;
    L.PB = p; L.T = p; p += TS;
    L.X = p; p += NE;
    L.Z = p; L.zd = (int)SC;
    L.R1 = p; L.R2 = p + P; L.COEF = p + 2 * P;
    L.NCS = p + 2 * P + 96;
    L.KB = (uint8_t*)(p + 3 * P + 96);
    L.FLN = (int*)(L.KB + ((int64_t)NP * D + 15) / 16 * 16);
    L.FL = (uint16_t*)(L.FLN + 4);
    p += SC;
    L.M1T = p; p += DD;
    L.M2T = p; p += DD;
    L.DSH = p; p += align2(D);
    L.V0 = p; p += align2(D);
    L.V1 = p; p += align2(D);
    L.V2 = p; p += align2(D);
    L.PBC = p; p += P;
    L.NC = p; p += P;
    L.PNI = p; p += P;
    L.CMUT = p; p += P;
    L.GB = p; p += align2(D);
    L.RED = p; p += 16;
    L.IMPR = (int*)p; p += align2((P + 1) / 2);
    L.MASK = (int*)p; p += align2((P + 1) / 2);
    L.RANK = (int*)p;
    return L;
}

__device__ __forceinline__ void rl_commit(const RlLds& L, int NP, int D, bool stagnation, double& gbest, int& gbest_idx,
                                          double* __restrict__ gPB, double* __restrict__ gCC)
{
    const int tid = threadIdx.x;
    for (int i = tid; i < NP; i += MBX_NT) {
        const double nc = L.NC[i];
        if (stagnation) L.PNI[i] = nc < gCC[i] ? 0. : L.PNI[i] + 1;
        const int impr = nc < L.PBC[i];
        if (impr) L.PBC[i] = nc;
        L.IMPR[i] = impr;
        gCC[i] = nc;
    }
    double cbv; int cb;
    block_argmin(L.NC, NP, L.RED, cbv, cb);
    const bool better = cbv < gbest;
    if (better) { gbest = cbv; gbest_idx = cb; }
    const int NE = NP * D;
    const FastDiv fd(D);
    for (int e = tid; e < NE; e += MBX_NT) {
        const int i = fd.div(e);
        if (L.IMPR[i]) gPB[e] = L.X[e];
    }
    if (better && tid < D) L.GB[tid] = L.X[cb * D + tid];
    __syncthreads();
}

struct MoveCtx {
    const RlLds& L; const double* pci; const double* tape; const Rng& rng; double* gPos; double* gVel;
    const int* ORDER; const int* NLESS; const int* RANK; int NP, D, G; double lb, ub, vmax; const FastDiv& fg;
};

struct GaussMlp {
    const float* w;
    int32_t in_dim, h1, h2, out_dim;
    float min_sigma, max_sigma;
    int32_t variant;
};

__host__ __device__ inline int gauss_mlp_net_floats(int in, int h1, int h2, int A) { return in * h1 + h1 + h1 * h2 + h2 + h2 * A + A; }

__device__ __forceinline__ void gauss_head(const GaussMlp& net, float am, float as, float& mu, float& sigma)
{
    mu = (tanhf(am) + 1.f) / 2.f;
    if (net.variant == MBX_POLICY_RLPSO) sigma = fminf(fmaxf((tanhf(as) + 1.f) / 2.f, net.min_sigma), net.max_sigma);
    else sigma = (tanhf(as) + 1.f) / 2.f * (net.max_sigma - net.min_sigma) + net.min_sigma;
}

__device__ __forceinline__ float sample_action(const Rng& rng, int j, float mu, float sigma, int variant)
{
    const U4 w = rng.draw((uint32_t)j, MBX_SITE_POLICY);
    const float u1 = (float)((w.x >> 8) + 1u) * 5.9604644775390625e-8f;
    const float u2 = (float)(w.y >> 8) * 5.9604644775390625e-8f;
    const float r = __builtin_sqrtf(-1.3862943611198906f * __builtin_amdgcn_logf(u1));
    const float a = mu + sigma * (r * __builtin_amdgcn_cosf(u2));
    if (variant == MBX_POLICY_RLPSO) return fabsf(a - 0.5f) >= 0.5f ? (a + 3.f * sigma - mu) * ((1.f / 6.f) * sigma) : a;
    return fminf(fmaxf(a, 0.f), 1.f);
}

#ifdef MBX_PHASE_TIMING
__device__ unsigned long long g_phase_cycles[8192 * 16];
#define MBX_PHASE_BEGIN unsigned long long ph_t = clock64();
#define MBX_PHASE(k) do { if (threadIdx.x == 0) { const unsigned long long t_ = clock64(); g_phase_cycles[(blockIdx.x & 8191) * 16 + (k)] += t_ - ph_t; ph_t = t_; } } while (0)
#else
#define MBX_PHASE_BEGIN
#define MBX_PHASE(k)
#endif

#ifndef MBX_RL_WAVES
#define MBX_RL_WAVES __attribute__((amdgpu_waves_per_eu(THREADS == 256 ? 5 : 4)))
#endif
#ifndef MBX_FDR_UNROLL
#define MBX_FDR_UNROLL 4
#endif
#ifndef MBX_FDR_OWN_AT
#define MBX_FDR_OWN_AT 64
#endif

__device__ __forceinline__ void fdr_take(double lhs, double rhs, double& ab, double& bb, int& kb, double a, double b, int k)
{
#ifdef MBX_FDR_BRANCH
    if (__builtin_amdgcn_ballot_w64(lhs < rhs) == 0ull) return;
#endif
#ifdef MBX_FDR_SELECT
    if (lhs < rhs) { ab = a; bb = b; kb = k; }
#else
    unsigned long long saved;
    asm("s_mov_b64 %[sv], exec\n\t"
                 "v_cmpx_lt_f64_e32 %[l], %[r]\n\t"
                 "v_mov_b64 %[ab], %[a]\n\t"
                 "v_mov_b64 %[bb], %[b]\n\t"
                 "v_mov_b32 %[kb], %[k]\n\t"
                 "s_mov_b64 exec, %[sv]"
                 : [ab] "+v"(ab), [bb] "+v"(bb), [kb] "+v"(kb), [sv] "=&s"(saved)
                 : [l] "v"(lhs), [r] "v"(rhs), [a] "v"(a), [b] "v"(b), [k] "s"(k)
                 : "vcc");
#endif
}

__device__ __forceinline__ void fdr_take_neg(double dif, double& ab, double& bb, int& kb, double a, double b, int k)
{
    unsigned long long saved;
    asm("s_mov_b64 %[sv], exec\n\t"
        "v_cmpx_gt_f64_e32 0, %[d]\n\t"
        "v_mov_b64 %[ab], %[a]\n\t"
        "v_mov_b64 %[bb], %[b]\n\t"
        "v_mov_b32 %[kb], %[k]\n\t"
        "s_mov_b64 exec, %[sv]"
        : [ab] "+v"(ab), [bb] "+v"(bb), [kb] "+v"(kb), [sv] "=&s"(saved)
        : [d] "v"(dif), [a] "v"(a), [b] "v"(b), [k] "s"(k)
        : "vcc");
}
__device__ __forceinline__ void fdr_take_neg2(double dif0, double dif1, double& ab0, double& bb0, int& kb0, double& ab1, double& bb1, int& kb1,
                                              double a, double b0, double b1, int k)
{
    unsigned long long saved;
    asm("s_mov_b64 %[sv], exec\n\t"
        "v_cmpx_gt_f64_e32 0, %[d0]\n\t"
        "v_mov_b64 %[ab0], %[a]\n\t"
        "v_mov_b64 %[bb0], %[b0]\n\t"
        "v_mov_b32 %[kb0], %[k]\n\t"
        "s_mov_b64 exec, %[sv]\n\t"
        "v_cmpx_gt_f64_e32 0, %[d1]\n\t"
        "v_mov_b64 %[ab1], %[a]\n\t"
        "v_mov_b64 %[bb1], %[b1]\n\t"
        "v_mov_b32 %[kb1], %[k]\n\t"
        "s_mov_b64 exec, %[sv]"
        : [ab0] "+v"(ab0), [bb0] "+v"(bb0), [kb0] "+v"(kb0), [ab1] "+v"(ab1), [bb1] "+v"(bb1), [kb1] "+v"(kb1), [sv] "=&s"(saved)
        : [d0] "v"(dif0), [d1] "v"(dif1), [a] "v"(a), [b0] "v"(b0), [b1] "v"(b1), [k] "s"(k)
        : "vcc");
}
__device__ __forceinline__ float f64_hi_as_f32(double v) { return __int_as_float(__double2hiint(v)); }
__device__ __forceinline__ float fdr_min3_abs(float m, float x, float y)
{
    float r;
    asm("v_min3_f32 %[r], %[m], |%[x]|, |%[y]|" : [r] "=v"(r) : [m] "v"(m), [x] "v"(x), [y] "v"(y));
    return r;
}
__device__ __forceinline__ void rl_mark_copies(const RlLds& L, int NP, int D, int r)
{
    if (r > 0 && r < NP && L.NC[r] == L.NC[r - 1]) {
        bool same = true;
        for (int d = 0; d < D && same; ++d) same = L.PB[r * D + d] == L.PB[(r - 1) * D + d];
        if (same) L.NCS[r] = 1e300;
    }
}

__device__ __forceinline__ int fdr_settle(const RlLds& L, const int* __restrict__ ORDER, int D, int rk, int d, int nless, int kw, unsigned long long* cnt = nullptr)
{
    const int lane = threadIdx.x & 63;
    const double fi = L.NC[rk];
    const double pp = L.PB[rk * D + d];
    const double aw = L.NC[kw] - fi, bw = fabs(L.PB[kw * D + d] - pp) + 1e-5;
    int first_copy = 0x7fffffff;
    bool others = false;
    for (int k0 = 0; k0 < nless; k0 += 64) {
        const int k = k0 + lane;
        bool band = false, copy = false;
        if (k < nless && k != kw) {
            const double a = L.NC[k] - fi, b = fabs(L.PB[k * D + d] - pp) + 1e-5, pr = aw * b;
            band = __builtin_fma(a, bw, -pr) <= pr * -0x1p-49;
            copy = band && a == aw && b == bw;
        }
        const unsigned long long mc = __builtin_amdgcn_ballot_w64(copy), mo = __builtin_amdgcn_ballot_w64(band && !copy);
        if (mc != 0ull && first_copy == 0x7fffffff) first_copy = k0 + (int)__builtin_ctzll(mc);
        others = others || mo != 0ull;
    }
    int kbest = kw < first_copy ? kw : first_copy;
#ifdef MBX_FDR_COUNT
    if (cnt && lane == 0) atomicAdd(cnt + (others ? 5 : first_copy != 0x7fffffff ? 4 : 6), 1ull);
#endif
    if (others) {
        double qb = aw / bw;
        int ib = ORDER[kbest];
        for (int k0 = 0; k0 < nless; k0 += 64) {
            const int k = k0 + lane;
            bool cont = false;
            double qk = 0.;
            int ik = 0;
            if (k < nless && k != kw) {
                const double a = L.NC[k] - fi, b = fabs(L.PB[k * D + d] - pp) + 1e-5, pr = aw * b;
                cont = __builtin_fma(a, bw, -pr) <= pr * -0x1p-49 && !(a == aw && b == bw);
                if (cont) { qk = a / b; ik = ORDER[k]; }
            }
            unsigned long long m = __builtin_amdgcn_ballot_w64(cont);
            while (m != 0ull) {
                const int l = (int)__builtin_ctzll(m);
                m &= m - 1ull;
                const double ql = __hiloint2double(__builtin_amdgcn_readlane(__double2hiint(qk), l), __builtin_amdgcn_readlane(__double2loint(qk), l));
                const int il = __builtin_amdgcn_readlane(ik, l);
                if (ql < qb || (ql == qb && il < ib)) { qb = ql; ib = il; kbest = k0 + l; }
            }
        }
    }
    return kbest;
}

template <int W, int UN = MBX_FDR_UNROLL, bool TIE = true>
// ... 209 lines not shown
                const int e = e0 + q;
                if (!(ucs[q] > pci)) {
                    int t1, t2;
                    if (c.tape) { t1 = (int)c.tape[MBX_RLEPSO_TAPE_TOURN(NP, D) + 2 * e]; t2 = (int)c.tape[MBX_RLEPSO_TAPE_TOURN(NP, D) + 2 * e + 1]; }
                    else {
                        const bool odd = W == 2 ? q == 1 : (e & 1);
                        t1 = (int)__umulhi(odd ? wt.z : wt.x, (uint32_t)NP); t2 = (int)__umulhi(odd ? wt.w : wt.y, (uint32_t)NP);
                    }
                    xrs[q] = c.RANK[L.PBC[t2] < L.PBC[t1] ? t2 : t1];
                }
            }
        }
    }
#pragma unroll
    for (int q = 0; q < W; ++q) {
        const int e = e0 + q, d = d0 + q;
        const double pp = L.PB[es0 + q], uc = ucs[q];
        const int xr = xrs[q], kb = L.KB[es0 + q];
        const double ex = L.PB[xr * D + d];
        const double v_fdr = uf[q] * (L.PB[kb * D + d] - pp);
        const double v_pbest = r1 * (pp - cur[q]);
        const double v_gbest = r2 * (L.GB[d] - cur[q]);
        const double v_cl = uc * (ex - cur[q]);
        double nv = cw * vel[q] + c1 * v_cl + c2 * v_fdr + c3 * v_gbest + c4 * v_pbest;
        nv = fmin(fmax(nv, -c.vmax), c.vmax);
        double np_ = cur[q] + nv;
        np_ = fmin(fmax(np_, c.lb), c.ub);
        L.X[e] = np_;
        if (RES) { cur[q] = np_; vel[q] = nv; }
        else { c.gPos[e] = np_; c.gVel[e] = nv; }
    }
}

template <int THREADS, int NPC = 0, int DC = 0>
__global__ __launch_bounds__(THREADS) void k_rlepso_reset(BatchParams bp, double* __restrict__ state_out)
{
    extern __shared__ __attribute__((aligned(16))) double smem[];
    const int b = bp.order[blockIdx.x], tid = threadIdx.x;
    const int NP = NPC ? NPC : bp.NP, D = DC ? DC : bp.D, NE = NP * D;
    constexpr bool MAPS = rl_maps_in_lds(NPC, DC);
    constexpr int MD = MAPS ? 0 : DC;
    const DevProblem P = bp.problems[bp.problem_idx[b]];
    const RlLds L = rl_carve(smem, NP, D, MAPS);
    double* S = bp.state + (int64_t)b * bp.state_stride;
    double* sc = S + MBX_RLEPSO_ST_SCALARS(NP, D);
    const double* tape = bp.tape ? bp.tape + (int64_t)b * bp.tape_stride : nullptr;

    const int episode = (int)sc[MBX_SC_EPISODE] + 1;
    const uint64_t seed = bp.seeds[b];
    const Rng rng{(uint32_t)seed, (uint32_t)(seed >> 32), 0u, (uint32_t)episode};
    const double lb = P.lb, ub = P.ub, vmax = 0.1 * (ub - lb);

    stage_problem<0, MAPS>(P, L.eval());
    for (int e = tid; e < NE; e += MBX_NT) {
        double up, uv;
        if (tape) { up = tape[MBX_RLEPSO_TAPE_REPOS(NP, D) + e]; uv = tape[MBX_RLEPSO_TAPE_REVEL(NP, D) + e]; }
        else { const U4 w = rng.draw((uint32_t)e, MBX_SITE_ELEM_R); up = u53(w.x, w.y); uv = u53(w.z, w.w); }
        const double x = lb + (ub - lb) * up;
        L.X[e] = x;
        S[MBX_RLEPSO_ST_POS(NP, D) + e] = x;
        S[MBX_RLEPSO_ST_PBPOS(NP, D) + e] = x;
        S[MBX_RLEPSO_ST_VEL(NP, D) + e] = -vmax + (vmax - (-vmax)) * uv;
    }
    __syncthreads();
    population_costs<0, MD>(P, L.eval(), NP, rng, tape ? tape + MBX_RLEPSO_TAPE_NOISE1(NP, D) : nullptr, MBX_SITE_NOISE1_A, MBX_SITE_NOISE1_B);
    double gb; int gi;
    block_argmin(L.NC, NP, L.RED, gb, gi);
    for (int i = tid; i < NP; i += MBX_NT) {
        const double c = L.NC[i];
        S[MBX_RLEPSO_ST_CCOST(NP, D) + i] = c;
        S[MBX_RLEPSO_ST_PBEST(NP, D) + i] = c;
        S[MBX_RLEPSO_ST_PNI(NP, D) + i] = 0.;
    }
    if (tid < D) S[MBX_RLEPSO_ST_GBPOS(NP, D) + tid] = L.X[gi * D + tid];
    if (tid == 0) {
        sc[MBX_SC_GBEST] = gb; sc[MBX_SC_FES] = NP; sc[MBX_SC_LOG_INDEX] = 1; sc[MBX_SC_COST_LEN] = 1;
        sc[MBX_SC_DONE] = 0; sc[MBX_SC_RETURN] = 0; sc[MBX_SC_GEN] = 0; sc[MBX_SC_EPISODE] = episode;
        sc[MBX_SC_GBEST_IDX] = gi; sc[MBX_SC_REINIT] = 0;
        sc[MBX_NSCALAR] = gb;
        if (state_out) state_out[b] = (double)NP / bp.max_fes;
    }
}

template <int THREADS, int NPC = 0, int DC = 0, int GC = 0, bool TIE = true>
__global__ __launch_bounds__(THREADS) MBX_RL_WAVES void k_rlepso_step(BatchParams bp, const float* __restrict__ actions,
                                                          double* __restrict__ state_out, double* __restrict__ reward_out,
                                                          uint8_t* __restrict__ done_out, const float* __restrict__ policy_table,
                                                          int table_rows, float* __restrict__ actions_out)
{
    extern __shared__ __attribute__((aligned(16))) double smem[];
    const int b = bp.order[blockIdx.x], tid = threadIdx.x;
    const int NP = NPC ? NPC : bp.NP, D = DC ? DC : bp.D, NE = NP * D, G = GC ? GC : bp.n_group;
    double* S = bp.state + (int64_t)b * bp.state_stride;
    double* sc = S + MBX_RLEPSO_ST_SCALARS(NP, D);

    if (sc[MBX_SC_DONE] != 0.) {
        if (tid == 0) {
            if (state_out) state_out[b] = sc[MBX_SC_FES] / bp.max_fes;
            if (reward_out) reward_out[b] = 0.;
            if (done_out) done_out[b] = 1;
        }
        return;
    }
    MBX_PHASE_BEGIN
    ConstProblem& P = *(ConstProblem*)(bp.problems + bp.problem_idx[b]);
    const RlLds L = rl_carve(smem, NP, D, rl_maps_in_lds(NPC, DC));
    const double* tape = bp.tape ? bp.tape + (int64_t)b * bp.tape_stride : nullptr;
    const float* act = actions + (int64_t)b * (7 * G);

    const int gen = (int)sc[MBX_SC_GEN] + 1;
    const uint64_t seed = bp.seeds[b];
    const Rng rng{(uint32_t)seed, (uint32_t)(seed >> 32), (uint32_t)gen, (uint32_t)(int)sc[MBX_SC_EPISODE], true};
    const double lb = P.lb, ub = P.ub, vmax = 0.1 * (ub - lb);
    double gbest = sc[MBX_SC_GBEST];
    int gbest_idx = (int)sc[MBX_SC_GBEST_IDX];
    const double pre_gbest = gbest;
    double fes = sc[MBX_SC_FES];

    const double* gPB = S + MBX_RLEPSO_ST_PBPOS(NP, D);
    double* gPos = S + MBX_RLEPSO_ST_POS(NP, D);
    double* gVel = S + MBX_RLEPSO_ST_VEL(NP, D);
    float* ACT = (float*)L.R1;
    if (policy_table && tid < 7 * G) {
        const int A = 7 * G;
        int row = (int)fes;
        row = row < table_rows ? row : table_rows - 1;
        const float* ms = policy_table + (int64_t)row * 2 * A;
        const float a = sample_action(rng, tid, ms[tid], ms[A + tid], MBX_POLICY_RLEPSO);
        ACT[tid] = a;
        if (actions_out) actions_out[(int64_t)b * A + tid] = a;
    }
    for (int i = tid; i < NP; i += MBX_NT) {
        L.PBC[i] = S[MBX_RLEPSO_ST_PBEST(NP, D) + i];
        L.RANK[i] = 0; L.MASK[i] = 0;
        L.IMPR[i] = i;
        L.PNI[i] = S[MBX_RLEPSO_ST_PNI(NP, D) + i];
    }
    if (tid < D) L.GB[tid] = S[MBX_RLEPSO_ST_GBPOS(NP, D) + tid];
    if (tid == 0) *L.FLN = 0;
    stage_problem<eval_dc(DC), eval_md(DC) == 0>(P, L.eval());
    auto get_coe = [&](const float* a) {
        const float cm = a[0] * 0.01f;
        const float wv = a[1] * 0.8f + 0.1f;
        float den = a[3] + a[4];
        den = den + a[5]; den = den + a[6]; den = den + 1e-5f;
        float scale = 1.f / den;
        scale = scale * a[2]; scale = scale * 8.f;
        double* c = L.COEF + tid * 6;
        c[0] = (double)cm; c[1] = (double)wv;
        c[2] = (double)(scale * a[3]); c[3] = (double)(scale * a[4]);
        c[4] = (double)(scale * a[5]); c[5] = (double)(scale * a[6]);
    };
    if (!policy_table && tid < G) get_coe(act + tid * G);
    __syncthreads();
    if (policy_table && tid < G) get_coe(ACT + tid * G);
    MBX_PHASE(0);
    const int per_group = NP / G;
    const FastDiv fd(D), fg(per_group);
    int* ORDER = L.IMPR;
    int* NLESS = L.MASK;
    int* RANK = L.RANK;
    {
        const int parts = MBX_NT / NP > 0 ? MBX_NT / NP : 1;
        for (int w = tid; w < parts * NP; w += MBX_NT) {
            const int part = w / NP, i = w - part * NP;
            const int j0 = part * NP / parts, j1 = (part + 1) * NP / parts;
            const double fi = L.PBC[i];
            int nle = 0, nless = 0;
#ifndef MBX_ABLATE_RANK
#pragma unroll 4
            for (int j = j0; j < j1; ++j) {
                const double fj = L.PBC[j];
                nless += fj < fi;
                nle += fj <= fi;
            }
#else
            if (part == 0) { nle = i + 1; nless = i; }
#endif
            atomicAdd(&RANK[i], nle); atomicAdd(&NLESS[i], nless);
        }
    }
    __syncthreads();
    int equal_costs = 0;
    for (int i = tid; i < NP; i += MBX_NT) {
        const int g = fg.div(i);
        L.CMUT[i] = g < G ? L.COEF[g * 6] * L.PNI[i] : 0.;
        if (tape) { L.R1[i] = tape[MBX_RLEPSO_TAPE_RAND1(NP, D) + i]; L.R2[i] = tape[MBX_RLEPSO_TAPE_RAND2(NP, D) + i]; }
        else { const U4 w = rng.draw((uint32_t)i, MBX_SITE_PART); L.R1[i] = u53(w.x, w.y); L.R2[i] = u53(w.z, w.w); }
        const double fi = L.PBC[i];
        int rank = NLESS[i];
        if (RANK[i] - rank > 1) {
            equal_costs = 1;
            for (int j = 0; j < i; ++j) rank += L.PBC[j] == fi;
        }
        RANK[i] = rank;
        ORDER[rank] = i; L.NC[rank] = fi; L.NCS[rank] = fi;
    }
    equal_costs = __syncthreads_or(equal_costs);
    MBX_PHASE(1);
    for (int e = tid; e < NE; e += MBX_NT) { const int i = fd.div(e), d = e - i * D; L.PB[RANK[i] * D + d] = gPB[e]; }
    __syncthreads();
    if (equal_costs) {
        for (int r = tid; r < NP; r += MBX_NT) rl_mark_copies(L, NP, D, r);
        __syncthreads();
    }
    MBX_PHASE(2);

#ifndef MBX_ABLATE_FDR
    if ((D & 1) == 0) fdr_pass<2, MBX_FDR_UNROLL, TIE, THREADS>(L, ORDER, NLESS, NP, D, tid, ub - lb + 1e-5);
    else fdr_pass<1, MBX_FDR_UNROLL, TIE, THREADS>(L, ORDER, NLESS, NP, D, tid, ub - lb + 1e-5);
#else
    for (int e = tid; e < NE; e += MBX_NT) L.KB[e] = 0;
    __syncthreads();
#endif

    const MoveCtx mc{L, bp.pci, tape, rng, gPos, gVel, ORDER, NLESS, RANK, NP, D, G, lb, ub, vmax, fg};
    if ((D & 1) == 0) {
        const int HD = D >> 1, NI = NP * HD;
        const FastDiv fh(HD);
        for (int it = tid; it < NI; it += MBX_NT) {
            const int i = fh.div(it);
            const double2 c2 = *(const double2*)(gPos + 2 * it), v2 = *(const double2*)(gVel + 2 * it);
            double cur[2] = {c2.x, c2.y}, vel[2] = {v2.x, v2.y};
            rl_move<2>(mc, i, 2 * (it - i * HD), cur, vel);
        }
    } else {
        for (int e = tid; e < NE; e += MBX_NT) {
            const int i = fd.div(e);
            double cur[1] = {gPos[e]}, vel[1] = {gVel[e]};
            rl_move<1>(mc, i, e - i * D, cur, vel);
        }
    }
    __syncthreads();
    MBX_PHASE(3);

    population_costs<eval_dc(DC), eval_md(DC)>(P, L.eval(), NP, rng, tape ? tape + MBX_RLEPSO_TAPE_NOISE0(NP, D) : nullptr, MBX_SITE_NOISE0_A, MBX_SITE_NOISE0_B);
    MBX_PHASE(4);
    fes += NP;
    rl_commit(L, NP, D, true, gbest, gbest_idx, S + MBX_RLEPSO_ST_PBPOS(NP, D), S + MBX_RLEPSO_ST_CCOST(NP, D));
    MBX_PHASE(5);

    int mine = 0;
    for (int i = tid; i < NP; i += MBX_NT) {
        double u;
        if (tape) u = tape[MBX_RLEPSO_TAPE_REINIT(NP, D) + i];
        else { const U4 w = rng.draw((uint32_t)i, MBX_SITE_REINIT); u = u53(w.x, w.y); }
        const int m = u < L.CMUT[i] * 0.01 * L.PNI[i];
        L.MASK[i] = m;
        mine += m;
    }
    const int n_reinit = __syncthreads_count(mine);
    MBX_PHASE(6);
    if (n_reinit > 0) {
        for (int e = tid; e < NE; e += MBX_NT) {
            const int i = fd.div(e);
            if (L.MASK[i]) {
                double up, uv;
                if (tape) { up = tape[MBX_RLEPSO_TAPE_REPOS(NP, D) + e]; uv = tape[MBX_RLEPSO_TAPE_REVEL(NP, D) + e]; }
                else { const U4 w = rng.draw((uint32_t)e, MBX_SITE_ELEM_R); up = u53(w.x, w.y); uv = u53(w.z, w.w); }
                const double x = lb + (ub - lb) * up;
                L.X[e] = x;
                gPos[e] = x;
                gVel[e] = -vmax + (vmax - (-vmax)) * uv;
            }
        }
        __syncthreads();
        population_costs<eval_dc(DC), eval_md(DC)>(P, L.eval(), NP, rng, tape ? tape + MBX_RLEPSO_TAPE_NOISE1(NP, D) : nullptr, MBX_SITE_NOISE1_A, MBX_SITE_NOISE1_B);
        fes += n_reinit;
        rl_commit(L, NP, D, false, gbest, gbest_idx, S + MBX_RLEPSO_ST_PBPOS(NP, D), S + MBX_RLEPSO_ST_CCOST(NP, D));
    }

    MBX_PHASE(7);
    for (int i = tid; i < NP; i += MBX_NT) {
        S[MBX_RLEPSO_ST_PBEST(NP, D) + i] = L.PBC[i];
        S[MBX_RLEPSO_ST_PNI(NP, D) + i] = L.PNI[i];
    }
    if (gbest < pre_gbest && tid < D) S[MBX_RLEPSO_ST_GBPOS(NP, D) + tid] = L.GB[tid];

    if (tid == 0) {
        int log_index = (int)sc[MBX_SC_LOG_INDEX], cost_len = (int)sc[MBX_SC_COST_LEN];
        double* cost = sc + MBX_NSCALAR;
        const bool done = log_and_terminate(bp, P, fes, gbest, log_index, cost_len, cost);
        const double reward = gbest < pre_gbest ? 1. : -1.;
        sc[MBX_SC_GBEST] = gbest; sc[MBX_SC_FES] = fes; sc[MBX_SC_LOG_INDEX] = log_index; sc[MBX_SC_COST_LEN] = cost_len;
        sc[MBX_SC_DONE] = done ? 1. : 0.; sc[MBX_SC_RETURN] += reward; sc[MBX_SC_GEN] = gen;
        sc[MBX_SC_GBEST_IDX] = gbest_idx; sc[MBX_SC_REINIT] = n_reinit > 0 ? 1. : 0.;
        if (state_out) state_out[b] = fes / bp.max_fes;
        if (reward_out) reward_out[b] = reward;
        if (done_out) done_out[b] = done ? 1 : 0;
    }
    MBX_PHASE(8);
}

struct RunOut {
    float* traj_actions;
    double* traj_state;
    double* traj_reward;
    uint8_t* traj_done;
    double* state_out;
    double* reward_out;
    uint8_t* done_out;
};

#ifndef MBX_RUN_WAVES
#define MBX_RUN_WAVES MBX_RL_WAVES
#endif
template <int THREADS, int NPC, int DC, int GC, int KIND, int NOISE, bool TIE, class ARGS>
__device__ __forceinline__ void rl_run_body(ARGS ar)
{
    const int n_gens = ar().n_gens;
    static_assert(NPC > 0 && DC > 0 && GC > 0 && (DC & 1) == 0 && NPC <= THREADS, "k_rlepso_run: compile-time geometry, even D, NP <= THREADS");
    constexpr int NP = NPC, D = DC, G = GC, HD = D / 2, NI = NP * HD, IT = (NI + THREADS - 1) / THREADS, A = 7 * G;
    extern __shared__ __attribute__((aligned(16))) double smem[];
    const int b = ar().bp.order[blockIdx.x], tid0 = threadIdx.x, tid = tid0;
    double* S = ar().bp.state + (int64_t)b * ar().bp.state_stride;
    double* sc = S + MBX_RLEPSO_ST_SCALARS(NP, D);
    const int64_t B = ar().bp.B;

    if (sc[MBX_SC_DONE] != 0.) {
        const double st = sc[MBX_SC_FES] / ar().bp.max_fes;
        for (int g = tid; g < n_gens; g += THREADS) {
            if (ar().out.traj_state) ar().out.traj_state[g * B + b] = st;
            if (ar().out.traj_reward) ar().out.traj_reward[g * B + b] = 0.;
            if (ar().out.traj_done) ar().out.traj_done[g * B + b] = 1;
        }
        if (tid == 0) {
            if (ar().out.state_out) ar().out.state_out[b] = st;
            if (ar().out.reward_out) ar().out.reward_out[b] = 0.;
            if (ar().out.done_out) ar().out.done_out[b] = 1;
        }
        return;
    }
    unsigned long long clk_c0 = 0, clk_r0 = 0;
    const bool clocked = ar().bp.clk != nullptr && tid0 == 0;
    if (clocked) { clk_c0 = __builtin_amdgcn_s_memtime(); clk_r0 = __builtin_amdgcn_s_memrealtime(); }
    ConstProblem& P = *(ConstProblem*)(ar().bp.problems + ar().bp.problem_idx[b]);
    const RlLds L = rl_carve(smem, NP, D, rl_maps_in_lds(NPC, DC));
    int gen = (int)sc[MBX_SC_GEN];
    const uint64_t seed = ar().bp.seeds[b];
    const uint32_t episode = (uint32_t)(int)sc[MBX_SC_EPISODE];
    const double lb = P.lb, ub = P.ub, vmax = 0.1 * (ub - lb);
    double gbest = sc[MBX_SC_GBEST];
    int gbest_idx = (int)sc[MBX_SC_GBEST_IDX];
    double fes = sc[MBX_SC_FES];
    int log_index = (int)sc[MBX_SC_LOG_INDEX], cost_len = (int)sc[MBX_SC_COST_LEN];
    double* cost = sc + MBX_NSCALAR;
    double ret = 0.;
    int n_reinit = 0;

    double* gPos = S + MBX_RLEPSO_ST_POS(NP, D);
    double* gVel = S + MBX_RLEPSO_ST_VEL(NP, D);
    double* gPB = S + MBX_RLEPSO_ST_PBPOS(NP, D);
    double vel[IT][2], pbp[IT][2], cc = 0.;
#pragma unroll
    for (int j = 0; j < IT; ++j) {
        const int it = tid + j * THREADS;
        vel[j][0] = vel[j][1] = pbp[j][0] = pbp[j][1] = 0.;
        if (it < NI) {
            const double2 v2 = *(const double2*)(gVel + 2 * it), p2 = *(const double2*)(gPB + 2 * it);
            vel[j][0] = v2.x; vel[j][1] = v2.y; pbp[j][0] = p2.x; pbp[j][1] = p2.y;
            *(double2*)(L.X + 2 * it) = *(const double2*)(gPos + 2 * it);
        }
    }
    if (tid < NP) {
        L.PBC[tid] = S[MBX_RLEPSO_ST_PBEST(NP, D) + tid];
        L.PNI[tid] = S[MBX_RLEPSO_ST_PNI(NP, D) + tid];
        cc = S[MBX_RLEPSO_ST_CCOST(NP, D) + tid];
    }
    if (tid < D) L.GB[tid] = S[MBX_RLEPSO_ST_GBPOS(NP, D) + tid];
    stage_problem<eval_dc(DC), eval_md(DC) == 0, ConstProblem>(P, L.eval());
    constexpr int per_group = NP / G;
    const FastDiv fg(per_group), fh(HD);
    int* ORDER = L.IMPR;
    int* NLESS = L.MASK;
    int* RANK = L.RANK;
    float* ACT = (float*)L.R1;
    int* EQC = (int*)(L.RED + 14);

    auto commit = [&](bool stagnation, int tid) {
        if (tid < NP) {
            const double nc = L.NC[tid];
            if (stagnation) L.PNI[tid] = nc < cc ? 0. : L.PNI[tid] + 1;
            const int impr = nc < L.PBC[tid];
            if (impr) L.PBC[tid] = nc;
            L.IMPR[tid] = impr;
            cc = nc;
        }
        double cbv; int cb;
        block_argmin(L.NC, NP, L.RED, cbv, cb);
        const bool better = cbv < gbest;
        if (better) { gbest = cbv; gbest_idx = cb; }
#pragma unroll
        for (int j = 0; j < IT; ++j) {
            const int it = tid + j * THREADS;
            if (it < NI && L.IMPR[fh.div(it)]) { const double2 x2 = *(const double2*)(L.X + 2 * it); pbp[j][0] = x2.x; pbp[j][1] = x2.y; }
        }
        if (better && tid < D) L.GB[tid] = L.X[cb * D + tid];
        __syncthreads();
    };

    bool done = false;
    int g = 0;
    __syncthreads();
    for (; g < n_gens && !done; ++g) {
        int tid = tid0;
        asm volatile("" : "+v"(tid));
        gen += 1;
        const Rng rng{(uint32_t)seed, (uint32_t)(seed >> 32), (uint32_t)gen, episode, true};
        const double pre_gbest = gbest;
        if (tid < A) {
            int row = (int)fes;
            row = row < ar().table_rows ? row : ar().table_rows - 1;
            const float* ms = ar().policy_table + (int64_t)row * 2 * A;
            const float a = sample_action(rng, tid, ms[tid], ms[A + tid], MBX_POLICY_RLEPSO);
            ACT[tid] = a;
            if (ar().out.traj_actions) ar().out.traj_actions[((int64_t)g * B + b) * A + tid] = a;
        }
        if (tid < NP) { NLESS[tid] = 0; ORDER[tid] = tid; }
        if (tid == 0) { *EQC = 0; *L.FLN = 0; }
        __syncthreads();
        if (tid < G) {
            const float* a = ACT + tid * G;
            const float cm = a[0] * 0.01f;
            const float wv = a[1] * 0.8f + 0.1f;
            float den = a[3] + a[4];
            den = den + a[5]; den = den + a[6]; den = den + 1e-5f;
            float scale = 1.f / den;
            scale = scale * a[2]; scale = scale * 8.f;
            double* c = L.COEF + tid * 6;
            c[0] = (double)cm; c[1] = (double)wv;
            c[2] = (double)(scale * a[3]); c[3] = (double)(scale * a[4]);
            c[4] = (double)(scale * a[5]); c[5] = (double)(scale * a[6]);
        }
        {
            constexpr int parts = THREADS / NP > 0 ? THREADS / NP : 1;
            for (int w = tid; w < parts * NP; w += THREADS) {
                const int part = w / NP, i = w - part * NP;
                const int j0 = part * NP / parts, j1 = (part + 1) * NP / parts;
                const double fi = L.PBC[i];
                int nless = 0;
#ifndef MBX_ABLATE_RANK
#pragma unroll 5
                for (int j = j0; j < j1; ++j) nless += L.PBC[j] < fi;
#else
                if (part == 0) nless = i;
#endif
                atomicAdd(&NLESS[i], nless);
            }
        }
        __syncthreads();
        if (tid < NP) {
            const int i = tid, gi = fg.div(i);
            L.CMUT[i] = gi < G ? L.COEF[gi * 6] * L.PNI[i] : 0.;
            const U4 w = rng.draw((uint32_t)i, MBX_SITE_PART);
            L.R1[i] = u53(w.x, w.y); L.R2[i] = u53(w.z, w.w);
            const int rank = NLESS[i];
            RANK[i] = rank;
            ORDER[rank] = i; L.NC[rank] = L.PBC[i]; L.NCS[rank] = L.PBC[i];
        }
        __syncthreads();
        if (tid < NP && ORDER[RANK[tid]] != tid) *EQC = 1;
        auto stage_pbest = [&](int tid) {
#pragma unroll
            for (int j = 0; j < IT; ++j) {
                const int it = tid + j * THREADS;
                if (it < NI) { const int i = fh.div(it), d0 = 2 * (it - i * HD); *(double2*)(L.PB + RANK[i] * D + d0) = double2{pbp[j][0], pbp[j][1]}; }
            }
        };
        stage_pbest(tid);
        __syncthreads();
        if (*EQC) {
            int rank = 0;
            if (tid < NP) {
                const double fi = L.PBC[tid];
                rank = NLESS[tid];
                for (int j = 0; j < tid; ++j) rank += L.PBC[j] == fi;
            }
            __syncthreads();
            if (tid < NP) { RANK[tid] = rank; ORDER[rank] = tid; L.NC[rank] = L.PBC[tid]; L.NCS[rank] = L.PBC[tid]; }
            __syncthreads();
            stage_pbest(tid);
            __syncthreads();
            rl_mark_copies(L, NP, D, tid);
            __syncthreads();
        }
#ifdef MBX_ABLATE_FDR
        for (int e = tid; e < NP * D; e += THREADS) L.KB[e] = 0;
        __syncthreads();
#else
        fdr_pass<2, (DC == 40 ? 2 : MBX_FDR_UNROLL), TIE, THREADS>(L, ORDER, NLESS, NP, D, tid, ub - lb + 1e-5, ar().bp.clk);
#endif
        {
            const MoveCtx mc{L, ar().bp.pci, nullptr, rng, nullptr, nullptr, ORDER, NLESS, RANK, NP, D, G, lb, ub, vmax, fg};
#pragma unroll
            for (int j = 0; j < IT; ++j) {
                const int it = tid + j * THREADS;
                if (it < NI) {
                    const int i = fh.div(it);
                    const double2 c2 = *(const double2*)(L.X + 2 * it);
                    double cur[2] = {c2.x, c2.y};
                    rl_move<2, true>(mc, i, 2 * (it - i * HD), cur, vel[j]);
                }
            }
        }
        __syncthreads();
        population_costs<eval_dc(DC), eval_md(DC), ConstProblem, rl_run_matvec_chunk(DC), KIND, NOISE>(P, L.eval(), NP, rng, nullptr, MBX_SITE_NOISE0_A, MBX_SITE_NOISE0_B);
        fes += NP;
        commit(true, tid);
        int mine = 0;
        if (tid < NP) {
            const U4 w = rng.draw((uint32_t)tid, MBX_SITE_REINIT);
            const double u = u53(w.x, w.y);
            mine = u < L.CMUT[tid] * 0.01 * L.PNI[tid];
            L.MASK[tid] = mine;
        }
        n_reinit = __syncthreads_count(mine);
        if (n_reinit > 0) {
#pragma unroll
            for (int j = 0; j < IT; ++j) {
                const int it = tid + j * THREADS;
                if (it < NI && L.MASK[fh.div(it)]) {
#pragma unroll
                    for (int q = 0; q < 2; ++q) {
                        const int e = 2 * it + q;
                        const U4 w = rng.draw((uint32_t)e, MBX_SITE_ELEM_R);
                        const double up = u53(w.x, w.y), uv = u53(w.z, w.w);
                        L.X[e] = lb + (ub - lb) * up;
                        vel[j][q] = -vmax + (vmax - (-vmax)) * uv;
                    }
                }
            }
            __syncthreads();
            population_costs<eval_dc(DC), eval_md(DC), ConstProblem, rl_run_matvec_chunk(DC), KIND, NOISE>(P, L.eval(), NP, rng, nullptr, MBX_SITE_NOISE1_A, MBX_SITE_NOISE1_B);
            fes += n_reinit;
            commit(false, tid);
        }
        if (fes >= (double)log_index * ar().bp.log_interval) { log_index += 1; if (tid == 0) cost[cost_len] = gbest; cost_len += 1; }
        done = fes >= ar().bp.max_fes;
        if (!isnan(P.optimum) && ar().bp.early_stop) done = done || gbest <= 1e-8;
        if (done) {
            if (cost_len >= ar().bp.n_logpoint + 1) { if (tid == 0) cost[cost_len - 1] = gbest; }
            else { if (tid == 0) cost[cost_len] = gbest; cost_len += 1; }
        }
        const double reward = gbest < pre_gbest ? 1. : -1.;
        ret += reward;
        if (tid == 0) {
            if (ar().out.traj_state) ar().out.traj_state[g * B + b] = fes / ar().bp.max_fes;
            if (ar().out.traj_reward) ar().out.traj_reward[g * B + b] = reward;
            if (ar().out.traj_done) ar().out.traj_done[g * B + b] = done ? 1 : 0;
        }
    }
#pragma unroll
    for (int j = 0; j < IT; ++j) {
        const int it = tid + j * THREADS;
        if (it < NI) {
            *(double2*)(gPos + 2 * it) = *(const double2*)(L.X + 2 * it);
            *(double2*)(gVel + 2 * it) = double2{vel[j][0], vel[j][1]};
            *(double2*)(gPB + 2 * it) = double2{pbp[j][0], pbp[j][1]};
        }
    }
    if (tid < NP) {
        S[MBX_RLEPSO_ST_PBEST(NP, D) + tid] = L.PBC[tid];
        S[MBX_RLEPSO_ST_PNI(NP, D) + tid] = L.PNI[tid];
        S[MBX_RLEPSO_ST_CCOST(NP, D) + tid] = cc;
    }
    if (tid < D) S[MBX_RLEPSO_ST_GBPOS(NP, D) + tid] = L.GB[tid];
    const double st = fes / ar().bp.max_fes;
    for (int t = g + tid; t < n_gens; t += THREADS) {
        if (ar().out.traj_state) ar().out.traj_state[t * B + b] = st;
        if (ar().out.traj_reward) ar().out.traj_reward[t * B + b] = 0.;
        if (ar().out.traj_done) ar().out.traj_done[t * B + b] = 1;
    }
    if (tid == 0) {
        sc[MBX_SC_GBEST] = gbest; sc[MBX_SC_FES] = fes; sc[MBX_SC_LOG_INDEX] = log_index; sc[MBX_SC_COST_LEN] = cost_len;
        sc[MBX_SC_DONE] = done ? 1. : 0.; sc[MBX_SC_RETURN] += ret; sc[MBX_SC_GEN] = gen;
        sc[MBX_SC_GBEST_IDX] = gbest_idx; sc[MBX_SC_REINIT] = n_reinit > 0 ? 1. : 0.;
        if (ar().out.state_out) ar().out.state_out[b] = st;
        if (ar().out.reward_out) ar().out.reward_out[b] = ret;
        if (ar().out.done_out) ar().out.done_out[b] = done ? 1 : 0;
        if (clocked) {
            atomicAdd(ar().bp.clk, (unsigned long long)__builtin_amdgcn_s_memtime() - clk_c0);
            atomicAdd(ar().bp.clk + 1, (unsigned long long)__builtin_amdgcn_s_memrealtime() - clk_r0);
        }
    }
}


struct RlRunArgs {
    BatchParams bp;
    const float* policy_table;
    int32_t table_rows, n_gens;
    RunOut out;
};

template <int THREADS, int NPC, int DC, int GC, int KIND, int NOISE, bool TIE>
__device__ __noinline__ void rl_run_body_of_kind(uint32_t karg_lo_, uint32_t karg_hi_)
{
    const uint32_t lo = (uint32_t)__builtin_amdgcn_readfirstlane((int)karg_lo_), hi = (uint32_t)__builtin_amdgcn_readfirstlane((int)karg_hi_);
    typedef const RlRunArgs __attribute__((address_space(4))) CArgs;
    auto ar = [&]() -> CArgs& {
        uintptr_t p = (uintptr_t)(((uint64_t)hi << 32) | lo);
        asm volatile("" : "+s"(p));
        return *(CArgs*)p;
    };
    rl_run_body<THREADS, NPC, DC, GC, KIND, NOISE, TIE>(ar);
}

__host__ __device__ constexpr bool rl_run_per_kind(int DC) { return DC == 10 || DC == 40; }
__host__ __device__ constexpr bool rl_run_kind_ok(int kind, int noise_kind)
{
    return noise_kind == MBX_NOISE_NONE ? (kind >= 1 && kind <= 24)
                                        : (kind == 1 || kind == 7 || kind == 8 || kind == 10 || kind == 14 || kind == 17 || kind == 19 || kind == 21);
}

template <int THREADS, int NPC, int DC, int GC, bool TIE = true>
__global__ __launch_bounds__(THREADS) MBX_RUN_WAVES void k_rlepso_run(BatchParams bp, const float* __restrict__ policy_table, int table_rows,
                                                                     int n_gens, RunOut out)
{
    if constexpr (rl_run_per_kind(DC)) {
        static_assert(sizeof(RlRunArgs) == sizeof(BatchParams) + 8 + 8 + sizeof(RunOut), "RlRunArgs mirrors the kernel's parameter list");
        const uint64_t karg = (uint64_t)(uintptr_t)__builtin_amdgcn_kernarg_segment_ptr();
        const uint32_t klo = (uint32_t)karg, khi = (uint32_t)(karg >> 32);
        const DevProblem* pr = bp.problems + bp.problem_idx[bp.order[blockIdx.x]];
        const int kind = __builtin_amdgcn_readfirstlane(pr->kind);
        const bool noisy = __builtin_amdgcn_readfirstlane(pr->noise_kind) != MBX_NOISE_NONE;
#define MBX_RL_KIND(K) case K: rl_run_body_of_kind<THREADS, NPC, DC, GC, K, 0, TIE>(klo, khi); break;
#define MBX_RL_NOISY(K) case K: rl_run_body_of_kind<THREADS, NPC, DC, GC, K, 1, TIE>(klo, khi); break;
        if (noisy) {
            switch (kind) {
            MBX_RL_NOISY(1) MBX_RL_NOISY(7) MBX_RL_NOISY(8) MBX_RL_NOISY(10) MBX_RL_NOISY(14) MBX_RL_NOISY(17) MBX_RL_NOISY(19) MBX_RL_NOISY(21)
            default: rl_run_body_of_kind<THREADS, NPC, DC, GC, 0, -1, TIE>(klo, khi);
            }
        } else {
            switch (kind) {
            MBX_RL_KIND(1) MBX_RL_KIND(2) MBX_RL_KIND(3) MBX_RL_KIND(4) MBX_RL_KIND(5) MBX_RL_KIND(6) MBX_RL_KIND(7) MBX_RL_KIND(8)
            MBX_RL_KIND(9) MBX_RL_KIND(10) MBX_RL_KIND(11) MBX_RL_KIND(12) MBX_RL_KIND(13) MBX_RL_KIND(14) MBX_RL_KIND(15) MBX_RL_KIND(16)
            MBX_RL_KIND(17) MBX_RL_KIND(18) MBX_RL_KIND(19) MBX_RL_KIND(20) MBX_RL_KIND(21) MBX_RL_KIND(22) MBX_RL_KIND(23) MBX_RL_KIND(24)
            default: rl_run_body_of_kind<THREADS, NPC, DC, GC, 0, -1, TIE>(klo, khi);
            }
        }
#undef MBX_RL_NOISY
#undef MBX_RL_KIND
    } else {
        typedef const RlRunArgs __attribute__((address_space(4))) CArgs;
        rl_run_body<THREADS, NPC, DC, GC, 0, -1, TIE>([]() -> CArgs& {
            return *(CArgs*)(uintptr_t)__builtin_amdgcn_kernarg_segment_ptr();
        });
    }
}

}
```

### metabox_amd/csrc/mbx_run_kernels.hpp

```cpp
#pragma once
#ifndef MBX_RUN10_THREADS
#define MBX_RUN10_THREADS 256
#endif
#define MBX_RUN_RLEPSO_EXACT(X)                                                                          \
    X template __global__ void k_rlepso_run<MBX_RUN10_THREADS, 100, 10, 5, true>(BatchParams, const float*, int, int, RunOut); \
    X template __global__ void k_rlepso_run<512, 100, 30, 5, true>(BatchParams, const float*, int, int, RunOut);                \
    X template __global__ void k_rlepso_run<256, 100, 12, 5, true>(BatchParams, const float*, int, int, RunOut);
#define MBX_RUN_RLEPSO_C5(X) X template __global__ void k_rlepso_run<1024, 128, 40, 5, true>(BatchParams, const float*, int, int, RunOut);
#define MBX_RUN_RLEPSO_D40(X) X template __global__ void k_rlepso_run<1024, 100, 40, 5, true>(BatchParams, const float*, int, int, RunOut);
#define MBX_RUN_RLEPSO_FAST(X)                                                                           \
    X template __global__ void k_rlepso_run<MBX_RUN10_THREADS, 100, 10, 5, false>(BatchParams, const float*, int, int, RunOut); \
    X template __global__ void k_rlepso_run<1024, 128, 40, 5, false>(BatchParams, const float*, int, int, RunOut);
#ifdef MBX_RUN_KERNELS_EXTERN
namespace mbx {
MBX_RUN_RLEPSO_EXACT(extern)
MBX_RUN_RLEPSO_C5(extern)
MBX_RUN_RLEPSO_D40(extern)
MBX_RUN_RLEPSO_FAST(extern)
extern template __global__ void k_lde_run<100, 30>(LdeRunArgs);
extern template __global__ void k_lde_run<50, 30>(LdeRunArgs);
extern template __global__ void k_lde_run<50, 10>(LdeRunArgs);
extern template __global__ void k_lde_run<50, 30, 50, true>(LdeRunArgs);
}
#endif
```

### metabox_amd/suite.py

```python
import ctypes as C

import numpy as np
import torch

from . import _abi


def _require_gpu():
    if not torch.cuda.is_available():
        raise _abi.MbxError('metabox_amd needs a ROCm GPU (MI355X); there is no CPU fallback for the hot path.')


def _ptr(t):
    return C.c_void_p(t.data_ptr()) if t is not None else C.c_void_p()


def _stream():
    return C.c_void_p(torch.cuda.current_stream().cuda_stream)


class Suite:

    def __init__(self, problems):
        _require_gpu()
        self.lib = _abi.load_lib()
        self.problems = list(problems)
        self.dim = int(self.problems[0].dim)
        descs = [p.desc() for p in self.problems]
        arr, self._keep = _abi.pack_descs(descs)
        opts = [getattr(p, 'opt', None) for p in self.problems]
        opt_arr = None
        if all(o is not None for o in opts):
            opt_arr = np.ascontiguousarray(np.stack([np.asarray(o, dtype=np.float64) for o in opts]))
        h = C.c_void_p()
        _abi.check(self.lib.mbx_suite_create(arr, len(descs), opt_arr.ctypes.data_as(_abi.c_double_p) if opt_arr is not None
                                             else _abi.c_double_p(), C.byref(h)))
        self._h = h
        out = np.empty(len(descs))
        _abi.check(self.lib.mbx_suite_optimum(self._h, out.ctypes.data_as(_abi.c_double_p)))
        self._optimum = out
        for i, p in enumerate(self.problems):
            p._suite = self
            p._suite_index = i
            p._optimum = None if np.isnan(out[i]) else float(out[i])

    def __len__(self):
        return len(self.problems)

    def optimum(self, i):
        v = self._optimum[i]
        return None if np.isnan(v) else float(v)

    def eval_device(self, i, x_dev, noisy=False, seed=0, noise_draws=None):
        assert x_dev.is_cuda and x_dev.dtype == torch.float64 and x_dev.is_contiguous() and x_dev.shape[1] == self.dim
        n = x_dev.shape[0]
        f = torch.empty(n, dtype=torch.float64, device=x_dev.device)
        _abi.check(self.lib.mbx_eval(self._h, int(i), _ptr(x_dev), n, _ptr(f), int(bool(noisy)), int(seed),
                                     _ptr(noise_draws), _stream()))
        return f

    _eval_calls = 0

    def eval(self, i, x, noisy=False, seed=None, noise_draws=None):
        xd = torch.from_numpy(np.ascontiguousarray(x, dtype=np.float64)).cuda()
        if seed is None:
            Suite._eval_calls += 1
            seed = (int(np.random.randint(0, 2 ** 31 - 1)) << 20) + Suite._eval_calls
        nd = None
        if noise_draws is not None:
            nd = torch.from_numpy(np.ascontiguousarray(noise_draws, dtype=np.float64)).cuda()
        return self.eval_device(i, xd, noisy, seed, nd).cpu().numpy()

    def close(self):
        if getattr(self, '_h', None):
            self.lib.mbx_suite_destroy(self._h)
            self._h = None

    def __del__(self):
        try:
            self.close()
        except Exception:
            pass


class Batch:

    def __init__(self, suite, algo, problem_idx, seeds, np_, max_fes, log_interval, n_logpoint, early_stop=True, n_group=5, flags=0):
        _require_gpu()
        self.lib = suite.lib
        self.suite = suite
        self.cfg = _abi.AlgoCfg(int(algo), int(np_), suite.dim, int(max_fes), int(log_interval), int(n_logpoint),
                                int(bool(early_stop)), int(n_group), int(flags))
        pidx = np.ascontiguousarray(problem_idx, dtype=np.int32)
        sd = np.ascontiguousarray(seeds, dtype=np.uint64)
        assert pidx.shape == sd.shape and pidx.ndim == 1
        self.B = int(pidx.shape[0])
        h = C.c_void_p()
        _abi.check(self.lib.mbx_batch_create(suite._h, C.byref(self.cfg), pidx.ctypes.data_as(C.POINTER(C.c_int32)),
                                             sd.ctypes.data_as(C.POINTER(C.c_uint64)), self.B, C.byref(h)))
        self._h = h
        self.flags = int(self.lib.mbx_batch_flags(h))
        self.cfg.flags = self.flags
        self.state_dim = self.lib.mbx_state_dim(C.byref(self.cfg))
        self.action_dim = self.lib.mbx_action_dim(C.byref(self.cfg))
        self.tape_stride = int(self.lib.mbx_tape_stride(C.byref(self.cfg)))
        dev = torch.device('cuda', torch.cuda.current_device())
        self.device = dev
        self.state = torch.zeros(self.B, self.state_dim, dtype=torch.float64, device=dev)
        self.reward = torch.zeros(self.B, dtype=torch.float64, device=dev)
        self.done = torch.zeros(self.B, dtype=torch.uint8, device=dev)
        self._tape = None

    def set_tape(self, tape):
        if tape is not None:
            assert tape.is_cuda and tape.dtype == torch.float64 and tape.is_contiguous()
            assert tuple(tape.shape) == (self.B, self.tape_stride)
        self._tape = tape
        _abi.check(self.lib.mbx_set_tape(self._h, _ptr(tape)))

    def reset(self):
        _abi.check(self.lib.mbx_reset(self._h, _ptr(self.state), _stream()))
        return self.state

    def step(self, actions):
        if self.action_dim > 0:
            want = torch.int32 if self.cfg.algo in (_abi.ALGO_DEDDQN, _abi.ALGO_QLPSO) else torch.float32
            assert actions.is_cuda and actions.is_contiguous() and actions.dtype == want
            assert actions.numel() == self.B * self.action_dim
        else:
            actions = None
        _abi.check(self.lib.mbx_step(self._h, _ptr(actions), _ptr(self.state), _ptr(self.reward), _ptr(self.done), _stream()))
        return self.state, self.reward, self.done

    def _net(self, weights, h1, h2, min_sigma, max_sigma):
        assert weights.is_cuda and weights.dtype == torch.float32 and weights.is_contiguous()
        variant = _abi.POLICY_RLPSO if self.cfg.algo == _abi.ALGO_RLPSO else _abi.POLICY_RLEPSO
        return _abi.GaussMlp(weights.data_ptr(), self.state_dim, int(h1), int(h2), self.action_dim, float(min_sigma), float(max_sigma), variant)

    def rlpso_rollout(self, weights, h1, h2, min_sigma, max_sigma, n_steps, want_actions=False):
        acts = None
        if want_actions:
            if getattr(self, '_actions', None) is None:
                self._actions = torch.empty(self.B, self.action_dim, dtype=torch.float32, device=self.device)
            acts = self._actions
        net = self._net(weights, h1, h2, min_sigma, max_sigma)
        _abi.check(self.lib.mbx_rlpso_rollout(self._h, C.byref(net), int(n_steps), _ptr(acts), _ptr(self.state), _ptr(self.reward),
                                              _ptr(self.done), _stream()))
        return (self.state, self.reward, self.done, acts) if want_actions else (self.state, self.reward, self.done)

    def gleet_policy(self, weights, min_sigma, max_sigma, want_mu_sigma=False):
        assert weights.is_cuda and weights.dtype == torch.float32 and weights.is_contiguous()
        if getattr(self, '_actions', None) is None:
            self._actions = torch.empty(self.B, self.action_dim, dtype=torch.float32, device=self.device)
        ms = torch.empty(self.B, 2, self.action_dim, dtype=torch.float32, device=self.device) if want_mu_sigma else None
        net = _abi.GleetActor(weights.data_ptr(), int(weights.numel()), float(min_sigma), float(max_sigma))
        _abi.check(self.lib.mbx_gleet_policy(self._h, C.byref(net), _ptr(self.state), _ptr(self._actions), _ptr(ms), _stream()))
        return (self._actions, ms) if want_mu_sigma else self._actions

    def qlpso_rollout(self, q_table, n_steps, want_actions=False):
        assert q_table.is_cuda and q_table.dtype == torch.float64 and q_table.is_contiguous() and tuple(q_table.shape) == (4, 4)
        acts = None
        if want_actions:
            if getattr(self, '_iactions', None) is None:
                self._iactions = torch.empty(self.B, dtype=torch.int32, device=self.device)
            acts = self._iactions
        _abi.check(self.lib.mbx_qlpso_rollout(self._h, _ptr(q_table), int(n_steps), _ptr(acts), _ptr(self.state), _ptr(self.reward),
                                              _ptr(self.done), _stream()))
        return (self.state, self.reward, self.done, acts) if want_actions else (self.state, self.reward, self.done)

    def ddqn_qnet(self, weights, width=100, depth=4, n_act=4, want_q=False):
        assert weights.is_cuda and weights.dtype == torch.float32 and weights.is_contiguous()
        need = self.state_dim * width + width + (depth - 1) * (width * width + width) + width * n_act + n_act
        if weights.numel() != need:
            raise ValueError(f'packed Q-network has {weights.numel()} floats, {self.state_dim} -> {width} x {depth} -> {n_act} needs {need}')
        if getattr(self, '_iactions', None) is None:
            self._iactions = torch.empty(self.B, dtype=torch.int32, device=self.device)
        q = torch.empty(self.B, n_act, dtype=torch.float32, device=self.device) if want_q else None
        net = _abi.QNet(weights.data_ptr(), self.state_dim, int(width), int(depth), int(n_act))
        _abi.check(self.lib.mbx_ddqn_qnet(self._h, C.byref(net), _ptr(self.state), _ptr(self._iactions), _ptr(q), _stream()))
        return (self._iactions, q) if want_q else self._iactions

    def lde_policy(self, weights, hidden, h, c, want_mu_sigma=False, sample=True):
        assert weights.is_cuda and weights.dtype == torch.float32 and weights.is_contiguous()
        assert h.is_cuda and c.is_cuda and h.dtype == c.dtype == torch.float32 and h.is_contiguous() and c.is_contiguous()
        assert h.numel() == c.numel() == self.B * hidden
        need = (self.state_dim + hidden) * 4 * hidden + 4 * hidden + 2 * hidden * self.action_dim + 2 * self.action_dim
        if weights.numel() != need:
            raise ValueError(f'packed LSTM policy has {weights.numel()} floats, in {self.state_dim} / hidden {hidden} / out {self.action_dim} needs {need}')
        if getattr(self, '_actions', None) is None:
            self._actions = torch.empty(self.B, self.action_dim, dtype=torch.float32, device=self.device)
        ms = torch.empty(self.B, 2, self.action_dim, dtype=torch.float32, device=self.device) if want_mu_sigma else None
        net = _abi.LstmPolicy(weights.data_ptr(), self.state_dim, int(hidden), self.action_dim)
        _abi.check(self.lib.mbx_lde_policy(self._h, C.byref(net), _ptr(self.state), _ptr(h), _ptr(c), _ptr(self._actions) if sample else None,
                                           _ptr(ms), _stream()))
        acts = self._actions if sample else None
        return (acts, ms) if want_mu_sigma else acts

    def lde_rollout_is_resident(self):
        return int(self.lib.mbx_lde_rollout_resident(self._h)) == 1

    def lde_rollout(self, weights, hidden, h, c, n_gens, trajectory=False):
        assert weights.is_cuda and weights.dtype == torch.float32 and weights.is_contiguous()
        assert h.is_cuda and c.is_cuda and h.dtype == c.dtype == torch.float32 and h.is_contiguous() and c.is_contiguous()
        assert h.numel() == c.numel() == self.B * hidden
        need = (self.state_dim + hidden) * 4 * hidden + 4 * hidden + 2 * hidden * self.action_dim + 2 * self.action_dim
        if weights.numel() != need:
            raise ValueError(f'packed LSTM policy has {weights.numel()} floats, in {self.state_dim} / hidden {hidden} / out {self.action_dim} needs {need}')
        n_gens = int(n_gens)
        traj = None
        if trajectory:
            traj = {'actions': torch.zeros(n_gens, self.B, self.action_dim, dtype=torch.float32, device=self.device),
                    'state': torch.zeros(n_gens, self.B, self.state_dim, dtype=torch.float64, device=self.device),
                    'reward': torch.empty(n_gens, self.B, dtype=torch.float64, device=self.device),
                    'done': torch.empty(n_gens, self.B, dtype=torch.uint8, device=self.device)}
        t = traj or {}
        net = _abi.LstmPolicy(weights.data_ptr(), self.state_dim, int(hidden), self.action_dim)
        _abi.check(self.lib.mbx_lde_rollout(self._h, C.byref(net), _ptr(self.state), _ptr(h), _ptr(c), n_gens, _ptr(t.get('actions')),
                                            _ptr(t.get('state')), _ptr(t.get('reward')), _ptr(t.get('done')), _ptr(self.state), _ptr(self.reward),
                                            _ptr(self.done), _stream()))
        return (self.state, self.reward, self.done, traj) if trajectory else (self.state, self.reward, self.done)

    def gauss_policy(self, weights, h1, h2, min_sigma, max_sigma, want_mu_sigma=False):
        if getattr(self, '_actions', None) is None:
            self._actions = torch.empty(self.B, self.action_dim, dtype=torch.float32, device=self.device)
        ms = torch.empty(self.B, 2, self.action_dim, dtype=torch.float32, device=self.device) if want_mu_sigma else None
        net = self._net(weights, h1, h2, min_sigma, max_sigma)
        _abi.check(self.lib.mbx_gauss_policy(self._h, C.byref(net), _ptr(self.state), _ptr(self._actions), _ptr(ms), _stream()))
        return (self._actions, ms) if want_mu_sigma else self._actions

    def policy_table(self, weights, h1, h2, min_sigma, max_sigma):
        rows = int(self.lib.mbx_rlepso_policy_table_rows(self._h))
        table = torch.empty(rows, 2, self.action_dim, dtype=torch.float32, device=self.device)
        net = self._net(weights, h1, h2, min_sigma, max_sigma)
        _abi.check(self.lib.mbx_rlepso_policy_table(self._h, C.byref(net), _ptr(table), _stream()))
        return table

    def _check_table(self, table):
        assert table.is_cuda and table.dtype == torch.float32 and table.is_contiguous()
        rows = int(self.lib.mbx_rlepso_policy_table_rows(self._h))
        if tuple(table.shape) != (rows, 2, self.action_dim):
            raise ValueError(f'actor table has shape {tuple(table.shape)}, this batch needs ({rows}, 2, {self.action_dim}) '
                             f'(mbx_rlepso_policy_table_rows x (mu, sigma) x action_dim)')

    def rollout_is_resident(self):
        return int(self.lib.mbx_rlepso_rollout_resident(self._h)) == 1

    def act_step(self, table, want_actions=False):
        self._check_table(table)
        acts = None
        if want_actions:
            if getattr(self, '_actions', None) is None:
                self._actions = torch.empty(self.B, self.action_dim, dtype=torch.float32, device=self.device)
            acts = self._actions
        _abi.check(self.lib.mbx_rlepso_act_step(self._h, _ptr(table), _ptr(acts), _ptr(self.state), _ptr(self.reward), _ptr(self.done),
                                                _stream()))
        return (self.state, self.reward, self.done, acts) if want_actions else (self.state, self.reward, self.done)

    def rlepso_rollout(self, table, n_gens, trajectory=False):
        self._check_table(table)
        n_gens = int(n_gens)
        traj = None
        if trajectory:
            traj = {'actions': torch.zeros(n_gens, self.B, self.action_dim, dtype=torch.float32, device=self.device),
                    'state': torch.empty(n_gens, self.B, dtype=torch.float64, device=self.device),
                    'reward': torch.empty(n_gens, self.B, dtype=torch.float64, device=self.device),
                    'done': torch.empty(n_gens, self.B, dtype=torch.uint8, device=self.device)}
        t = traj or {}
        _abi.check(self.lib.mbx_rlepso_rollout(self._h, _ptr(table), n_gens, _ptr(t.get('actions')), _ptr(t.get('state')),
                                               _ptr(t.get('reward')), _ptr(t.get('done')), _ptr(self.state), _ptr(self.reward),
                                               _ptr(self.done), _stream()))
        return (self.state, self.reward, self.done, traj) if trajectory else (self.state, self.reward, self.done)

    def results(self):
        n = self.cfg.n_logpoint + 1
        cost = torch.empty(self.B, n, dtype=torch.float64, device=self.device)
        fes = torch.empty(self.B, dtype=torch.float64, device=self.device)
        ret = torch.empty(self.B, dtype=torch.float64, device=self.device)
        steps = torch.empty(self.B, dtype=torch.int32, device=self.device)
        clen = torch.empty(self.B, dtype=torch.int32, device=self.device)
        _abi.check(self.lib.mbx_results(self._h, _ptr(cost), _ptr(fes), _ptr(ret), _ptr(steps), _ptr(clen), _stream()))
        return {'cost': cost, 'fes': fes, 'return': ret, 'steps': steps, 'cost_len': clen}

    def rebind(self, problem_idx, seeds):
        pidx = np.ascontiguousarray(problem_idx, dtype=np.int32)
        sd = np.ascontiguousarray(seeds, dtype=np.uint64)
        assert pidx.shape == sd.shape == (self.B,)
        _abi.check(self.lib.mbx_batch_rebind(self._h, pidx.ctypes.data_as(C.c_void_p), sd.ctypes.data_as(C.c_void_p)))

    def read_public(self, instance=0):
        if getattr(self, '_pub', None) is None:
            self._pub = np.empty(16 + self.cfg.n_logpoint + 1)
        _abi.check(self.lib.mbx_read_public(self._h, int(instance), self._pub.ctypes.data_as(_abi.c_double_p), _stream()))
        return self._pub

    def read_state(self, instance):
        n = int(self.lib.mbx_instance_state_doubles(self._h))
        out = np.empty(n)
        _abi.check(self.lib.mbx_debug_read_state(self._h, int(instance), out.ctypes.data_as(_abi.c_double_p)))
        return out

    def write_state(self, instance, block):
        n = int(self.lib.mbx_instance_state_doubles(self._h))
        block = np.ascontiguousarray(block, dtype=np.float64)
        assert block.shape == (n,)
        _abi.check(self.lib.mbx_debug_write_state(self._h, int(instance), block.ctypes.data_as(_abi.c_double_p)))

    def launch_info(self):
        import ctypes as C
        out = (C.c_int32 * 4)()
        _abi.check(self.lib.mbx_batch_launch_info(self._h, out))
        return {'threads': out[0], 'lds_bytes': out[1], 'fixed_geometry': out[2], 'state_doubles': out[3]}

    def close(self):
        if getattr(self, '_h', None):
            self.lib.mbx_batch_destroy(self._h)
            self._h = None

    def __del__(self):
        try:
            self.close()
        except Exception:
            pass
```

Measured before the change: 35.81 million.

## Split rollout runs into head/tail units to balance the final wave across CUs

For the d=10 RLEPSO resident rollout, a fraction of instances is split into a head unit (early generations) and a tail unit (last generations). Each head publishes a per-instance epoch flag, and tails either run opportunistically in the first launch once the flag is seen or in a second launch. The aim is to fill idle compute slots during the tail wave where few long blocks would otherwise run alone. In exchange it adds a second kernel launch, atomic flag polling, extra state writes and reads between units, and a risk of redundant or serialized work. It is skipped during graph capture.

Result: slower. 35.41 million (-1.1%).

```diff
diff --git a/include/mbx.h b/include/mbx.h
--- a/include/mbx.h
+++ b/include/mbx.h
@@ -84,6 +84,7 @@
 #define MBX_F_FDR_FAST               1u
 #define MBX_F_GENERIC_GEOMETRY       2u
 #define MBX_F_ROLLOUT_PER_GENERATION 4u
+#define MBX_F_ROLLOUT_NO_SPLIT       8u
 int mbx_batch_flags(const mbx_batch* b);
 
 int mbx_state_dim(const mbx_algo_cfg* cfg);
@@ -176,6 +177,10 @@
 int mbx_debug_clock_mark(uint64_t* d_out2, void* stream);
 int mbx_debug_clock_slots(mbx_batch* b, uint64_t* d_slots2);
 
+int mbx_batch_run_plan(const mbx_batch* b, int n_gens, int32_t out[6]);
+int mbx_debug_run_split(mbx_batch* b, int S, int tail_max, int tail_min, int defer_all);
+int mbx_debug_run_plan(int n_instances, int n_gens, int slots, const int32_t* forced3, int32_t plan_out[4], int32_t* units_out);
+
 const char* mbx_last_error(void);
 const char* mbx_version(void);
 
diff --git a/metabox_amd/_abi.py b/metabox_amd/_abi.py
--- a/metabox_amd/_abi.py
+++ b/metabox_amd/_abi.py
@@ -25,7 +25,7 @@
                 ('n_group', C.c_int32), ('flags', C.c_uint32)]
 
 
-F_FDR_FAST, F_GENERIC_GEOMETRY, F_ROLLOUT_PER_GENERATION = 1, 2, 4
+F_FDR_FAST, F_GENERIC_GEOMETRY, F_ROLLOUT_PER_GENERATION, F_ROLLOUT_NO_SPLIT = 1, 2, 4, 8
 
 
 class GaussMlp(C.Structure):
@@ -144,6 +144,9 @@
         'mbx_debug_clock_probe': (C.c_int, [vp, C.c_int, C.c_int, vp]),
         'mbx_debug_clock_mark': (C.c_int, [vp, vp]),
         'mbx_debug_clock_slots': (C.c_int, [vp, vp]),
+        'mbx_batch_run_plan': (C.c_int, [vp, C.c_int, C.POINTER(C.c_int32)]),
+        'mbx_debug_run_split': (C.c_int, [vp, C.c_int, C.c_int, C.c_int, C.c_int]),
+        'mbx_debug_run_plan': (C.c_int, [C.c_int, C.c_int, C.c_int, C.POINTER(C.c_int32), C.POINTER(C.c_int32), C.POINTER(C.c_int32)]),
         'mbx_batch_rebind': (C.c_int, [vp, vp, vp]),
         'mbx_read_public': (C.c_int, [vp, C.c_int, c_double_p, vp]),
         'mbx_last_error': (C.c_char_p, []),
@@ -163,7 +166,7 @@
                     'mbx_rlepso_rollout_resident', 'mbx_rlepso_rollout', 'mbx_lde_rollout_resident', 'mbx_lde_rollout', 'mbx_rlpso_rollout',
                     'mbx_qlpso_rollout', 'mbx_gleet_policy', 'mbx_debug_math', 'mbx_debug_rlepso_draws', 'mbx_batch_launch_info', 'mbx_instance_state_doubles',
                     'mbx_debug_read_state', 'mbx_debug_write_state', 'mbx_debug_clock_probe', 'mbx_debug_clock_mark', 'mbx_debug_clock_slots',
-                    'mbx_batch_rebind', 'mbx_read_public', 'mbx_last_error', 'mbx_version')
+                    'mbx_batch_run_plan', 'mbx_debug_run_split', 'mbx_debug_run_plan', 'mbx_batch_rebind', 'mbx_read_public', 'mbx_last_error', 'mbx_version')
 
 
 def check(rc):
diff --git a/metabox_amd/csrc/mbx.hip b/metabox_amd/csrc/mbx.hip
--- a/metabox_amd/csrc/mbx.hip
+++ b/metabox_amd/csrc/mbx.hip
@@ -84,6 +84,12 @@
     bool lde_run_kinds_ok = false;
     bool lde_run_kinds_two = false;
     bool rollout_per_generation = false;
+    bool rollout_no_split = false;
+    uint32_t* d_split = nullptr;
+    uint32_t epoch = 0;
+    int run_slots = 0;
+    bool plan_forced = false;
+    int forced_S = 0, forced_tail_max = 0, forced_tail_min = 0, forced_defer = 0;
     int64_t state_stride = 0;
     const double* d_tape = nullptr;
     size_t lds_bytes = 0;
@@ -451,7 +457,7 @@
     if (c->algo == MBX_ALGO_RLEPSO && (c->n_group < 1 || c->n_group > 16 || c->np / c->n_group < 1))
         return fail(MBX_E_ARG, "bad n_group %d", c->n_group);
     if (c->max_fes <= 0 || c->log_interval <= 0 || c->n_logpoint <= 0) return fail(MBX_E_ARG, "bad budget/log settings");
-    if (c->flags & ~(MBX_F_FDR_FAST | MBX_F_GENERIC_GEOMETRY | MBX_F_ROLLOUT_PER_GENERATION)) return fail(MBX_E_ARG, "unknown bits in cfg.flags 0x%x", c->flags);
+    if (c->flags & ~(MBX_F_FDR_FAST | MBX_F_GENERIC_GEOMETRY | MBX_F_ROLLOUT_PER_GENERATION | MBX_F_ROLLOUT_NO_SPLIT)) return fail(MBX_E_ARG, "unknown bits in cfg.flags 0x%x", c->flags);
     return MBX_OK;
 }
 
@@ -526,7 +532,7 @@
 {
     auto on = [](const char* name) { const char* v = getenv(name); return v && v[0] == '1'; };
     return (on("MBX_FDR_FAST") ? MBX_F_FDR_FAST : 0u) | (on("MBX_GENERIC_GEOMETRY") ? MBX_F_GENERIC_GEOMETRY : 0u) |
-           (on("MBX_ROLLOUT_PER_GENERATION") ? MBX_F_ROLLOUT_PER_GENERATION : 0u);
+           (on("MBX_ROLLOUT_PER_GENERATION") ? MBX_F_ROLLOUT_PER_GENERATION : 0u) | (on("MBX_ROLLOUT_NO_SPLIT") ? MBX_F_ROLLOUT_NO_SPLIT : 0u);
 }
 
 extern "C" int mbx_batch_create(mbx_suite* s, const mbx_algo_cfg* cfg_in, const int32_t* problem_idx, const uint64_t* seeds,
@@ -566,6 +572,7 @@
         if (cfg->algo == MBX_ALGO_DEDDQN && cfg->np == 100 && cfg->dim == 12 && !generic) b->fixed_geometry = 4;
         if (cfg->algo == MBX_ALGO_GLEET && cfg->np == 100 && cfg->dim == 10 && !generic) b->fixed_geometry = 5;
         b->rollout_per_generation = (cfg->flags & MBX_F_ROLLOUT_PER_GENERATION) != 0;
+        b->rollout_no_split = (cfg->flags & MBX_F_ROLLOUT_NO_SPLIT) != 0;
     }
 #ifdef MBX_LDS_PAD_EXPERIMENT
     if (const char* e = getenv("MBX_LDS_PAD")) b->lds_bytes += (size_t)atoi(e);
@@ -602,6 +609,17 @@
         MBX_RL_LDS(k_rlepso_run<1024, 128, 40, 5, true>); MBX_RL_LDS(k_rlepso_run<1024, 128, 40, 5, false>);
         MBX_RL_LDS(k_rlepso_run<512, 100, 30, 5, true>); MBX_RL_LDS(k_rlepso_run<256, 100, 12, 5, true>); MBX_RL_LDS(k_rlepso_run<1024, 100, 40, 5, true>);
 #undef MBX_RL_LDS
+        if (b->fixed_geometry == 1) {
+            HIP_TRY(hipMalloc(&b->d_split, (size_t)2 * n_instances * sizeof(uint32_t)));
+            HIP_TRY(hipMemset(b->d_split, 0, (size_t)2 * n_instances * sizeof(uint32_t)));
+            int dev = 0, per_cu = 0;
+            hipDeviceProp_t prop;
+            HIP_TRY(hipGetDevice(&dev));
+            HIP_TRY(hipGetDeviceProperties(&prop, dev));
+            if (b->fdr_fast) HIP_TRY(hipOccupancyMaxActiveBlocksPerMultiprocessor(&per_cu, (const void*)k_rlepso_run<MBX_RUN10_THREADS, 100, 10, 5, false>, MBX_RUN10_THREADS, lds));
+            else HIP_TRY(hipOccupancyMaxActiveBlocksPerMultiprocessor(&per_cu, (const void*)k_rlepso_run<MBX_RUN10_THREADS, 100, 10, 5, true>, MBX_RUN10_THREADS, lds));
+            b->run_slots = prop.multiProcessorCount * per_cu;
+        }
     } else if (cfg->algo == MBX_ALGO_LDE) {
         {
             HIP_TRY(hipMalloc(&b->d_scratch, (size_t)n_instances * (sizeof(double) + (size_t)g.action_dim * sizeof(float))));
@@ -661,6 +679,7 @@
 {
     if (!b) return MBX_OK;
     (void)hipFree(b->d_problem_idx); (void)hipFree(b->d_seeds); (void)hipFree(b->d_state); (void)hipFree(b->d_order); (void)hipFree(b->d_pci); (void)hipFree(b->d_scratch); (void)hipFree(b->d_lstm_pack);
+    (void)hipFree(b->d_split);
     delete b;
     return MBX_OK;
 }
@@ -973,17 +992,66 @@
     if (i < n) acc[i] = first ? r[i] : acc[i] + r[i];
 }
 
+static RunPlan rlepso_run_plan(const mbx_batch* b, int n_gens, bool capturing)
+{
+    if (b->fixed_geometry != 1 || b->rollout_no_split || !b->d_split || capturing) return RunPlan{0, 1, 0, 0};
+    if (b->plan_forced) return run_plan_make(b->B, n_gens, b->forced_S, b->forced_tail_max, b->forced_tail_min);
+    return run_plan_default(b->B, n_gens, b->run_slots);
+}
+
 static int launch_rlepso_run(mbx_batch* b, const float* d_table, int rows, int n_gens, const RunOut& out, hipStream_t stream)
 {
-#define MBX_RUN_LAUNCH(T, ...) hipLaunchKernelGGL((k_rlepso_run<T, __VA_ARGS__>), dim3(b->B), dim3(T), b->lds_bytes, stream, make_params(b), d_table, rows, n_gens, out)
-    if (b->fixed_geometry == 1) { if (b->fdr_fast) MBX_RUN_LAUNCH(MBX_RUN10_THREADS, 100, 10, 5, false); else MBX_RUN_LAUNCH(MBX_RUN10_THREADS, 100, 10, 5, true); }
-    else if (b->fixed_geometry == 2) { if (b->fdr_fast) MBX_RUN_LAUNCH(1024, 128, 40, 5, false); else MBX_RUN_LAUNCH(1024, 128, 40, 5, true); }
-    else if (b->fixed_geometry == 7) MBX_RUN_LAUNCH(512, 100, 30, 5, true);
-    else if (b->fixed_geometry == 8) MBX_RUN_LAUNCH(256, 100, 12, 5, true);
-    else if (b->fixed_geometry == 10) MBX_RUN_LAUNCH(1024, 100, 40, 5, true);
-    else return fail(MBX_E_UNSUPPORTED, "k_rlepso_run: no instantiation for this geometry");
+    hipStreamCaptureStatus cap = hipStreamCaptureStatusNone;
+    if (hipStreamIsCapturing(stream, &cap) != hipSuccess) { (void)hipGetLastError(); cap = hipStreamCaptureStatusActive; }
+    RunSplit sp{};
+    sp.plan = rlepso_run_plan(b, n_gens, cap != hipStreamCaptureStatusNone);
+    if (sp.plan.S > 0) {
+        b->epoch += 1;
+        if (b->epoch == 0) b->epoch = 1;
+        sp.flag = b->d_split; sp.tail_done = b->d_split + b->B; sp.epoch = b->epoch;
+    }
+    for (int phase = 0; phase < (sp.plan.S > 0 ? 2 : 1); ++phase) {
+        const int grid = phase == 0 ? run_plan_grid(b->B, sp.plan) : sp.plan.S;
+        sp.phase = phase | (phase == 0 && b->plan_forced && b->forced_defer ? 2 : 0);
+#define MBX_RUN_LAUNCH(T, ...) hipLaunchKernelGGL((k_rlepso_run<T, __VA_ARGS__>), dim3(grid), dim3(T), b->lds_bytes, stream, make_params(b), d_table, rows, n_gens, out, sp)
+        if (b->fixed_geometry == 1) { if (b->fdr_fast) MBX_RUN_LAUNCH(MBX_RUN10_THREADS, 100, 10, 5, false); else MBX_RUN_LAUNCH(MBX_RUN10_THREADS, 100, 10, 5, true); }
+        else if (b->fixed_geometry == 2) { if (b->fdr_fast) MBX_RUN_LAUNCH(1024, 128, 40, 5, false); else MBX_RUN_LAUNCH(1024, 128, 40, 5, true); }
+        else if (b->fixed_geometry == 7) MBX_RUN_LAUNCH(512, 100, 30, 5, true);
+        else if (b->fixed_geometry == 8) MBX_RUN_LAUNCH(256, 100, 12, 5, true);
+        else if (b->fixed_geometry == 10) MBX_RUN_LAUNCH(1024, 100, 40, 5, true);
+        else return fail(MBX_E_UNSUPPORTED, "k_rlepso_run: no instantiation for this geometry");
 #undef MBX_RUN_LAUNCH
-    HIP_TRY(hipGetLastError());
+    }
+    HIP_TRY(hipGetLastError());
+    return MBX_OK;
+}
+
+extern "C" int mbx_debug_run_split(mbx_batch* b, int S, int tail_max, int tail_min, int defer_all)
+{
+    if (!b) return fail(MBX_E_ARG, "mbx_debug_run_split: null batch");
+    b->plan_forced = S >= 0;
+    b->forced_S = S; b->forced_tail_max = tail_max; b->forced_tail_min = tail_min; b->forced_defer = defer_all;
+    return MBX_OK;
+}
+
+extern "C" int mbx_batch_run_plan(const mbx_batch* b, int n_gens, int32_t out[6])
+{
+    if (!b || !out || n_gens < 1) return fail(MBX_E_ARG, "mbx_batch_run_plan: bad arguments");
+    const RunPlan p = b->cfg.algo == MBX_ALGO_RLEPSO ? rlepso_run_plan(b, n_gens, false) : RunPlan{0, 1, 0, 0};
+    out[0] = p.S; out[1] = p.stripe; out[2] = p.tail_max; out[3] = p.tail_min; out[4] = run_plan_grid(b->B, p); out[5] = b->run_slots;
+    return MBX_OK;
+}
+
+extern "C" int mbx_debug_run_plan(int n_instances, int n_gens, int slots, const int32_t* forced3, int32_t plan_out[4], int32_t* units_out)
+{
+    if (n_instances < 1 || n_gens < 1 || !plan_out) return fail(MBX_E_ARG, "mbx_debug_run_plan: bad arguments");
+    const RunPlan p = forced3 ? run_plan_make(n_instances, n_gens, forced3[0], forced3[1], forced3[2]) : run_plan_default(n_instances, n_gens, slots);
+    plan_out[0] = p.S; plan_out[1] = p.stripe; plan_out[2] = p.tail_max; plan_out[3] = p.tail_min;
+    if (units_out)
+        for (int idx = 0; idx < run_plan_grid(n_instances, p); ++idx) {
+            const RunUnit u = run_plan_decode(idx, n_instances, n_gens, p);
+            units_out[4 * idx] = u.pos; units_out[4 * idx + 1] = u.g0; units_out[4 * idx + 2] = u.g1; units_out[4 * idx + 3] = u.role;
+        }
     return MBX_OK;
 }
 
diff --git a/metabox_amd/csrc/mbx_rlepso.hpp b/metabox_amd/csrc/mbx_rlepso.hpp
--- a/metabox_amd/csrc/mbx_rlepso.hpp
+++ b/metabox_amd/csrc/mbx_rlepso.hpp
@@ -1,5 +1,6 @@
 #pragma once
 #include "mbx_device.hpp"
+#include "mbx_run_plan.hpp"
 
 namespace mbx {
 
@@ -815,33 +816,89 @@
     uint8_t* done_out;
 };
 
+struct RunSplit {
+    uint32_t* flag;
+    uint32_t* tail_done;
+    RunPlan plan;
+    uint32_t epoch;
+    int32_t phase;
+};
+
 #ifndef MBX_RUN_WAVES
 #define MBX_RUN_WAVES MBX_RL_WAVES
 #endif
+__host__ __device__ constexpr bool rl_run_splits(int DC) { return DC == 10; }
+template <int DC, class ARGS>
+__device__ __forceinline__ RunUnit rl_run_unit(ARGS ar)
+{
+    if constexpr (!rl_run_splits(DC)) return RunUnit{(int32_t)blockIdx.x, 0, ar().n_gens, MBX_UNIT_WHOLE};
+    else {
+        const RunPlan p{ar().sp.plan.S, ar().sp.plan.stripe, ar().sp.plan.tail_max, ar().sp.plan.tail_min};
+        const int32_t B = ar().bp.B;
+        return run_plan_decode((int32_t)blockIdx.x + ((ar().sp.phase & 1) ? B : 0), B, ar().n_gens, p);
+    }
+}
 template <int THREADS, int NPC, int DC, int GC, int KIND, int NOISE, bool TIE, class ARGS>
 __device__ __forceinline__ void rl_run_body(ARGS ar)
 {
-    const int n_gens = ar().n_gens;
     static_assert(NPC > 0 && DC > 0 && GC > 0 && (DC & 1) == 0 && NPC <= THREADS, "k_rlepso_run: compile-time geometry, even D, NP <= THREADS");
     constexpr int NP = NPC, D = DC, G = GC, HD = D / 2, NI = NP * HD, IT = (NI + THREADS - 1) / THREADS, A = 7 * G;
     extern __shared__ __attribute__((aligned(16))) double smem[];
-    const int b = ar().bp.order[blockIdx.x], tid0 = threadIdx.x, tid = tid0;
+    const RunUnit unit = rl_run_unit<DC>(ar);
+    const int g0 = unit.g0, g1 = unit.g1, role = unit.role;
+    const int b = ar().bp.order[unit.pos], tid0 = threadIdx.x, tid = tid0;
     double* S = ar().bp.state + (int64_t)b * ar().bp.state_stride;
     double* sc = S + MBX_RLEPSO_ST_SCALARS(NP, D);
     const int64_t B = ar().bp.B;
 
+    if constexpr (rl_run_splits(DC)) {
+        if (role == MBX_UNIT_TAIL) {
+            if (ar().sp.phase & 1) {
+                if (__hip_atomic_load(ar().sp.tail_done + b, __ATOMIC_RELAXED, __HIP_MEMORY_SCOPE_AGENT) == ar().sp.epoch) return;
+            } else {
+                if (ar().sp.phase & 2) return;
+                uint32_t* seen = (uint32_t*)smem;
+                if (tid0 == 0) *seen = __hip_atomic_load(ar().sp.flag + b, __ATOMIC_RELAXED, __HIP_MEMORY_SCOPE_AGENT);
+                __syncthreads();
+                if (*seen != ar().sp.epoch) return;
+                if (tid0 == 0) {
+                    __builtin_amdgcn_fence(__ATOMIC_ACQUIRE, "agent");
+                    asm volatile("s_waitcnt vmcnt(0)" ::: "memory");
+                }
+                __syncthreads();
+            }
+        }
+    }
+    auto publish = [&]() {
+        if constexpr (rl_run_splits(DC)) {
+            if (role == MBX_UNIT_HEAD) {
+                asm volatile("s_waitcnt vmcnt(0)" ::: "memory");
+                __syncthreads();
+                if (tid0 == 0) {
+                    __builtin_amdgcn_fence(__ATOMIC_RELEASE, "agent");
+                    asm volatile("s_waitcnt vmcnt(0)" ::: "memory");
+                    __hip_atomic_store(ar().sp.flag + b, ar().sp.epoch, __ATOMIC_RELAXED, __HIP_MEMORY_SCOPE_AGENT);
+                }
+            }
+        }
+    };
+
     if (sc[MBX_SC_DONE] != 0.) {
         const double st = sc[MBX_SC_FES] / ar().bp.max_fes;
-        for (int g = tid; g < n_gens; g += THREADS) {
+        for (int g = g0 + tid; g < g1; g += THREADS) {
             if (ar().out.traj_state) ar().out.traj_state[g * B + b] = st;
             if (ar().out.traj_reward) ar().out.traj_reward[g * B + b] = 0.;
             if (ar().out.traj_done) ar().out.traj_done[g * B + b] = 1;
         }
         if (tid == 0) {
             if (ar().out.state_out) ar().out.state_out[b] = st;
-            if (ar().out.reward_out) ar().out.reward_out[b] = 0.;
+            if (ar().out.reward_out && role != MBX_UNIT_TAIL) ar().out.reward_out[b] = 0.;
             if (ar().out.done_out) ar().out.done_out[b] = 1;
-        }
+            if constexpr (rl_run_splits(DC)) {
+                if (role == MBX_UNIT_TAIL) __hip_atomic_store(ar().sp.tail_done + b, ar().sp.epoch, __ATOMIC_RELAXED, __HIP_MEMORY_SCOPE_AGENT);
+            }
+        }
+        publish();
         return;
     }
     unsigned long long clk_c0 = 0, clk_r0 = 0;
@@ -913,9 +970,9 @@
     };
 
     bool done = false;
-    int g = 0;
+    int g = g0;
     __syncthreads();
-    for (; g < n_gens && !done; ++g) {
+    for (; g < g1 && !done; ++g) {
         int tid = tid0;
         asm volatile("" : "+v"(tid));
         gen += 1;
@@ -1079,7 +1136,7 @@
     }
     if (tid < D) S[MBX_RLEPSO_ST_GBPOS(NP, D) + tid] = L.GB[tid];
     const double st = fes / ar().bp.max_fes;
-    for (int t = g + tid; t < n_gens; t += THREADS) {
+    for (int t = g + tid; t < g1; t += THREADS) {
         if (ar().out.traj_state) ar().out.traj_state[t * B + b] = st;
         if (ar().out.traj_reward) ar().out.traj_reward[t * B + b] = 0.;
         if (ar().out.traj_done) ar().out.traj_done[t * B + b] = 1;
@@ -1088,14 +1145,18 @@
         sc[MBX_SC_GBEST] = gbest; sc[MBX_SC_FES] = fes; sc[MBX_SC_LOG_INDEX] = log_index; sc[MBX_SC_COST_LEN] = cost_len;
         sc[MBX_SC_DONE] = done ? 1. : 0.; sc[MBX_SC_RETURN] += ret; sc[MBX_SC_GEN] = gen;
         sc[MBX_SC_GBEST_IDX] = gbest_idx; sc[MBX_SC_REINIT] = n_reinit > 0 ? 1. : 0.;
-        if (ar().out.state_out) ar().out.state_out[b] = st;
-        if (ar().out.reward_out) ar().out.reward_out[b] = ret;
-        if (ar().out.done_out) ar().out.done_out[b] = done ? 1 : 0;
+        if (ar().out.state_out && role != MBX_UNIT_HEAD) ar().out.state_out[b] = st;
+        if (ar().out.reward_out) ar().out.reward_out[b] = role == MBX_UNIT_TAIL ? ar().out.reward_out[b] + ret : ret;
+        if (ar().out.done_out && role != MBX_UNIT_HEAD) ar().out.done_out[b] = done ? 1 : 0;
+        if constexpr (rl_run_splits(DC)) {
+            if (role == MBX_UNIT_TAIL) __hip_atomic_store(ar().sp.tail_done + b, ar().sp.epoch, __ATOMIC_RELAXED, __HIP_MEMORY_SCOPE_AGENT);
+        }
         if (clocked) {
             atomicAdd(ar().bp.clk, (unsigned long long)__builtin_amdgcn_s_memtime() - clk_c0);
             atomicAdd(ar().bp.clk + 1, (unsigned long long)__builtin_amdgcn_s_memrealtime() - clk_r0);
         }
     }
+    publish();
 }
 
 
@@ -1104,6 +1165,7 @@
     const float* policy_table;
     int32_t table_rows, n_gens;
     RunOut out;
+    RunSplit sp;
 };
 
 template <int THREADS, int NPC, int DC, int GC, int KIND, int NOISE, bool TIE>
@@ -1128,13 +1190,15 @@
 
 template <int THREADS, int NPC, int DC, int GC, bool TIE = true>
 __global__ __launch_bounds__(THREADS) MBX_RUN_WAVES void k_rlepso_run(BatchParams bp, const float* __restrict__ policy_table, int table_rows,
-                                                                     int n_gens, RunOut out)
+                                                                     int n_gens, RunOut out, RunSplit sp)
 {
     if constexpr (rl_run_per_kind(DC)) {
-        static_assert(sizeof(RlRunArgs) == sizeof(BatchParams) + 8 + 8 + sizeof(RunOut), "RlRunArgs mirrors the kernel's parameter list");
+        static_assert(sizeof(RlRunArgs) == sizeof(BatchParams) + 8 + 8 + sizeof(RunOut) + sizeof(RunSplit), "RlRunArgs mirrors the kernel's parameter list");
         const uint64_t karg = (uint64_t)(uintptr_t)__builtin_amdgcn_kernarg_segment_ptr();
         const uint32_t klo = (uint32_t)karg, khi = (uint32_t)(karg >> 32);
-        const DevProblem* pr = bp.problems + bp.problem_idx[bp.order[blockIdx.x]];
+        typedef const RlRunArgs __attribute__((address_space(4))) CArgs;
+        const int pos = rl_run_unit<DC>([]() -> CArgs& { return *(CArgs*)(uintptr_t)__builtin_amdgcn_kernarg_segment_ptr(); }).pos;
+        const DevProblem* pr = bp.problems + bp.problem_idx[bp.order[pos]];
         const int kind = __builtin_amdgcn_readfirstlane(pr->kind);
         const bool noisy = __builtin_amdgcn_readfirstlane(pr->noise_kind) != MBX_NOISE_NONE;
 #define MBX_RL_KIND(K) case K: rl_run_body_of_kind<THREADS, NPC, DC, GC, K, 0, TIE>(klo, khi); break;
diff --git a/metabox_amd/csrc/mbx_run_kernels.hpp b/metabox_amd/csrc/mbx_run_kernels.hpp
--- a/metabox_amd/csrc/mbx_run_kernels.hpp
+++ b/metabox_amd/csrc/mbx_run_kernels.hpp
@@ -3,14 +3,14 @@
 #define MBX_RUN10_THREADS 256
 #endif
 #define MBX_RUN_RLEPSO_EXACT(X)                                                                          \
-    X template __global__ void k_rlepso_run<MBX_RUN10_THREADS, 100, 10, 5, true>(BatchParams, const float*, int, int, RunOut); \
-    X template __global__ void k_rlepso_run<512, 100, 30, 5, true>(BatchParams, const float*, int, int, RunOut);                \
-    X template __global__ void k_rlepso_run<256, 100, 12, 5, true>(BatchParams, const float*, int, int, RunOut);
-#define MBX_RUN_RLEPSO_C5(X) X template __global__ void k_rlepso_run<1024, 128, 40, 5, true>(BatchParams, const float*, int, int, RunOut);
-#define MBX_RUN_RLEPSO_D40(X) X template __global__ void k_rlepso_run<1024, 100, 40, 5, true>(BatchParams, const float*, int, int, RunOut);
+    X template __global__ void k_rlepso_run<MBX_RUN10_THREADS, 100, 10, 5, true>(BatchParams, const float*, int, int, RunOut, RunSplit); \
+    X template __global__ void k_rlepso_run<512, 100, 30, 5, true>(BatchParams, const float*, int, int, RunOut, RunSplit);                \
+    X template __global__ void k_rlepso_run<256, 100, 12, 5, true>(BatchParams, const float*, int, int, RunOut, RunSplit);
+#define MBX_RUN_RLEPSO_C5(X) X template __global__ void k_rlepso_run<1024, 128, 40, 5, true>(BatchParams, const float*, int, int, RunOut, RunSplit);
+#define MBX_RUN_RLEPSO_D40(X) X template __global__ void k_rlepso_run<1024, 100, 40, 5, true>(BatchParams, const float*, int, int, RunOut, RunSplit);
 #define MBX_RUN_RLEPSO_FAST(X)                                                                           \
-    X template __global__ void k_rlepso_run<MBX_RUN10_THREADS, 100, 10, 5, false>(BatchParams, const float*, int, int, RunOut); \
-    X template __global__ void k_rlepso_run<1024, 128, 40, 5, false>(BatchParams, const float*, int, int, RunOut);
+    X template __global__ void k_rlepso_run<MBX_RUN10_THREADS, 100, 10, 5, false>(BatchParams, const float*, int, int, RunOut, RunSplit); \
+    X template __global__ void k_rlepso_run<1024, 128, 40, 5, false>(BatchParams, const float*, int, int, RunOut, RunSplit);
 #ifdef MBX_RUN_KERNELS_EXTERN
 namespace mbx {
 MBX_RUN_RLEPSO_EXACT(extern)
diff --git a/metabox_amd/csrc/mbx_run_plan.hpp b/metabox_amd/csrc/mbx_run_plan.hpp
--- /dev/null
+++ b/metabox_amd/csrc/mbx_run_plan.hpp
@@ -0,0 +1,67 @@
+#pragma once
+#include <cstdint>
+
+#if defined(__HIPCC__) || defined(__CUDACC__)
+#define MBX_PLAN_FN __host__ __device__ inline
+#else
+#define MBX_PLAN_FN inline
+#endif
+
+namespace mbx {
+
+enum : int32_t { MBX_UNIT_WHOLE = 0, MBX_UNIT_HEAD = 1, MBX_UNIT_TAIL = 2 };
+
+struct RunPlan { int32_t S, stripe, tail_max, tail_min; };
+struct RunUnit { int32_t pos, g0, g1, role; };
+
+MBX_PLAN_FN int32_t run_plan_grid(int32_t B, const RunPlan& p) { return B + p.S; }
+
+MBX_PLAN_FN int32_t run_plan_tail_len(const RunPlan& p, int32_t t)
+{
+    return p.tail_max - (int32_t)(((uint32_t)t * (uint32_t)(p.tail_max - p.tail_min + 1)) / (uint32_t)p.S);
+}
+
+MBX_PLAN_FN RunUnit run_plan_decode(int32_t idx, int32_t B, int32_t n_gens, const RunPlan& p)
+{
+    if (p.S <= 0) return RunUnit{idx, 0, n_gens, MBX_UNIT_WHOLE};
+    if (idx < p.S) return RunUnit{idx * p.stripe, 0, n_gens - run_plan_tail_len(p, idx), MBX_UNIT_HEAD};
+    if (idx >= B) { const int32_t t = idx - B; return RunUnit{t * p.stripe, n_gens - run_plan_tail_len(p, t), n_gens, MBX_UNIT_TAIL}; }
+    const int32_t j = idx - p.S, between = p.S * (p.stripe - 1);
+    if (j >= between) return RunUnit{p.S * p.stripe + (j - between), 0, n_gens, MBX_UNIT_WHOLE};
+    const uint32_t q = (uint32_t)j / (uint32_t)(p.stripe - 1), r = (uint32_t)j - q * (uint32_t)(p.stripe - 1);
+    return RunUnit{(int32_t)(q * (uint32_t)p.stripe + r + 1), 0, n_gens, MBX_UNIT_WHOLE};
+}
+
+MBX_PLAN_FN RunPlan run_plan_make(int32_t B, int32_t n_gens, int32_t S, int32_t tail_max, int32_t tail_min)
+{
+    if (S <= 0 || n_gens < 2 || B < 1) return RunPlan{0, 1, 0, 0};
+    if (S > B) S = B;
+    if (tail_max > n_gens - 1) tail_max = n_gens - 1;
+    if (tail_max < 1) tail_max = 1;
+    if (tail_min < 1) tail_min = 1;
+    if (tail_min > tail_max) tail_min = tail_max;
+    return RunPlan{S, B / S, tail_max, tail_min};
+}
+
+#ifndef MBX_PLAN_SPLIT_NUM
+#define MBX_PLAN_SPLIT_NUM 3
+#endif
+#ifndef MBX_PLAN_SPLIT_DEN
+#define MBX_PLAN_SPLIT_DEN 8
+#endif
+#ifndef MBX_PLAN_TAIL_MAX_PCT
+#define MBX_PLAN_TAIL_MAX_PCT 40
+#endif
+#ifndef MBX_PLAN_TAIL_MIN_DIV
+#define MBX_PLAN_TAIL_MIN_DIV 20
+#endif
+
+MBX_PLAN_FN RunPlan run_plan_default(int32_t B, int32_t n_gens, int32_t slots)
+{
+    if (slots < 1 || B < 2 * slots || n_gens < 8) return RunPlan{0, 1, 0, 0};
+    const int32_t S = (int32_t)((int64_t)B * MBX_PLAN_SPLIT_NUM / MBX_PLAN_SPLIT_DEN);
+    const int32_t tmin = n_gens / MBX_PLAN_TAIL_MIN_DIV;
+    return run_plan_make(B, n_gens, S, (int32_t)((int64_t)n_gens * MBX_PLAN_TAIL_MAX_PCT / 100), tmin < 1 ? 1 : tmin);
+}
+
+}
diff --git a/metabox_amd/suite.py b/metabox_amd/suite.py
--- a/metabox_amd/suite.py
+++ b/metabox_amd/suite.py
@@ -309,7 +309,18 @@
         import ctypes as C
         out = (C.c_int32 * 4)()
         _abi.check(self.lib.mbx_batch_launch_info(self._h, out))
-        return {'threads': out[0], 'lds_bytes': out[1], 'fixed_geometry': out[2], 'state_doubles': out[3]}
+        info = {'threads': out[0], 'lds_bytes': out[1], 'fixed_geometry': out[2], 'state_doubles': out[3]}
+        if self.cfg.algo == _abi.ALGO_RLEPSO:
+            info['run_plan_20'] = self.run_plan(20)
+        return info
+
+    def run_plan(self, n_gens):
+        out = (C.c_int32 * 6)()
+        _abi.check(self.lib.mbx_batch_run_plan(self._h, int(n_gens), out))
+        return dict(zip(('S', 'stripe', 'tail_max', 'tail_min', 'grid', 'slots'), (int(x) for x in out)))
+
+    def debug_run_split(self, S, tail_max=0, tail_min=0, defer_all=False):
+        _abi.check(self.lib.mbx_debug_run_split(self._h, int(S), int(tail_max), int(tail_min), int(bool(defer_all))))
 
     def close(self):
         if getattr(self, '_h', None):
```
